# everpeace/kube-throttler

Hardware: AMD Instinct MI355X
Metric: pod_throttle_decisions_per_sec (higher is better)
Workload: dtype int64; 1 GPU; configs[2]: 1M pods x 1k Throttle+ClusterThrottle, D=8; pods_total=1000000, pods_per_gpu=1000000, throttles=1000, dims=8, labels_per_pod=8, namespaces=64, step=reconcile(aggregate+allreduce+finalize,apply)+check(all pods), streams=one, kernel_variant=indexed, parallelism=pods row-sharded x1, throttles replicated, exchange=none

## Files before the change

### include/kt_engine.h

```cpp
#ifndef KT_ENGINE_H
#define KT_ENGINE_H

#include <stdint.h>
#include "kt_snapshot.h"

#ifdef __cplusplus
extern "C" {
#endif

#define KT_OK 0
#define KT_ERR_INVALID_ARGUMENT (-1)
#define KT_ERR_OUT_OF_RANGE (-2)
#define KT_ERR_DEVICE (-3)
#define KT_ERR_OVERFLOW_RISK (-4)
#define KT_ERR_NOT_READY (-5)
#define KT_ERR_NO_DEVICE (-6)
#define KT_ERR_UNSUPPORTED (-7)

#define KT_STATUS_NOT_AFFECTED 0
#define KT_STATUS_NOT_THROTTLED 1
#define KT_STATUS_ACTIVE 2
#define KT_STATUS_INSUFFICIENT 3
#define KT_STATUS_POD_REQUESTS_EXCEEDS_THRESHOLD 4
#define KT_STATUS_ERROR 255
// ... 1 lines not shown
#define KT_VERDICT_SUCCESS 0
#define KT_VERDICT_UNSCHEDULABLE 1
#define KT_VERDICT_ERROR 2
#define KT_SUMMARY_VERDICT(w) ((uint32_t)((w) & 3u))
#define KT_SUMMARY_EXCEEDS(w) ((uint32_t)(((w) >> 4) & 0xFFFFFu))
#define KT_SUMMARY_ACTIVE(w) ((uint32_t)(((w) >> 24) & 0xFFFFFu))
#define KT_SUMMARY_INSUFFICIENT(w) ((uint32_t)(((w) >> 44) & 0xFFFFFu))

typedef struct kt_engine kt_engine;

typedef struct kt_config {
  int32_t n_dims;
  int32_t max_labels;
  int64_t pod_capacity;
  int32_t throttle_capacity;
  int32_t namespace_capacity;
  int32_t device;
  int32_t kernel_variant;
} kt_config;
#define KT_VARIANT_INCREMENTAL 0x100

const char* kt_version(void);

int32_t kt_engine_create(const kt_config* cfg, kt_engine** out);
int32_t kt_engine_destroy(kt_engine* e);
const char* kt_last_error(kt_engine* e);

int32_t kt_upsert_namespaces(kt_engine* e, const kt_snapshot* batch, const int32_t* ns_rows);
int32_t kt_upsert_pods(kt_engine* e, const kt_snapshot* batch, const int64_t* pod_rows);
int32_t kt_upsert_throttles(kt_engine* e, const kt_snapshot* batch, const int32_t* thr_rows);
int32_t kt_delete_namespaces(kt_engine* e, int32_t n, const int32_t* ns_rows);
int32_t kt_delete_pods(kt_engine* e, int64_t n, const int64_t* pod_rows);
int32_t kt_delete_throttles(kt_engine* e, int32_t n, const int32_t* thr_rows);
int32_t kt_load_snapshot(kt_engine* e, const kt_snapshot* s);

int32_t kt_upsert_namespace(kt_engine* e, int32_t ns_row, int32_t exists, int32_t n_labels, const uint32_t* label_keys,
                            const uint32_t* label_pairs);
int32_t kt_upsert_pod(kt_engine* e, int64_t pod_row, uint32_t ns, uint32_t flags, int32_t n_labels, const uint32_t* label_keys,
                      const uint32_t* label_pairs, int32_t n_ctr, const uint8_t* ctr_init, const uint32_t* ctr_present,
                      const int64_t* ctr_req, uint32_t ovh_present, const int64_t* ovh);
int32_t kt_upsert_throttle(kt_engine* e, int32_t thr_row, uint32_t flags, uint32_t ns, const int64_t* amt_v,
                           const uint32_t* amt_present, const int64_t* amt_count, const uint8_t* amt_has_count,
                           uint32_t thrl_flag, uint32_t thrl_has, uint64_t status_msgs_fp, uint64_t spec_msgs_fp, int32_t n_ovr,
                           const int64_t* ovr_begin_s, const int32_t* ovr_begin_ns, const int64_t* ovr_end_s,
                           const int32_t* ovr_end_ns, const uint8_t* ovr_flags, const int64_t* ovr_v, const uint32_t* ovr_present,
                           const int64_t* ovr_count, const uint8_t* ovr_has_count, int32_t n_terms, const uint8_t* term_flags,
                           const uint32_t* term_preq_off, const uint32_t* term_nreq_off, uint32_t n_preq, const uint8_t* preq_op,
                           const uint32_t* preq_key, const uint32_t* preq_val_off, const uint32_t* preq_val, uint32_t n_nreq,
                           const uint8_t* nreq_op, const uint32_t* nreq_key, const uint32_t* nreq_val_off, const uint32_t* nreq_val);

int32_t kt_set_reserved(kt_engine* e, int32_t n, const int32_t* thr_rows, const kt_amounts* reserved);
typedef struct kt_status {
  kt_amounts used;
  kt_amounts calc;
  uint8_t* calc_at_nonzero;
  uint32_t* thrl_flag;
  uint32_t* thrl_has;
  uint8_t* thrl_pod;
  uint64_t* msgs_fp;
  uint8_t* error;
} kt_status;
int32_t kt_set_status(kt_engine* e, int32_t n, const int32_t* thr_rows, const kt_status* status);

#define KT_RECONCILE_APPLY 0x1u
int32_t kt_reconcile_launch(kt_engine* e, int64_t now_s, int32_t now_ns, uint32_t flags, void* stream);
int32_t kt_reconcile_rows_launch(kt_engine* e, int64_t now_s, int32_t now_ns, uint32_t flags, int32_t n,
                                 const int32_t* throttle_rows, void* stream);
int32_t kt_aggregate_launch(kt_engine* e, void* stream);
int32_t kt_partial_used_buffer(kt_engine* e, void** device_ptr, int64_t* n_int64);
int32_t kt_use_partial_buffer(kt_engine* e, void* device_ptr, int64_t n_int64);
int32_t kt_finalize_launch(kt_engine* e, int64_t now_s, int32_t now_ns, uint32_t flags, void* stream);
#define KT_COMM_ID_BYTES 128
int32_t kt_comm_unique_id(void* out_id128);
int32_t kt_comm_init(kt_engine* e, int32_t rank, int32_t world, const void* id128);
int32_t kt_comm_allreduce_partial(kt_engine* e, void* stream);
int32_t kt_set_exchange_world(kt_engine* e, int32_t world);
int32_t kt_set_wide_sums(kt_engine* e, int32_t mode);
int32_t kt_partial_words(kt_engine* e, int64_t* n_int64, int32_t* wide);
int32_t kt_partial_layout(int32_t n_dims, int32_t* stride, int32_t* off_values, int32_t* off_presence, int32_t* off_pods,
                          int32_t* off_errors);
int32_t kt_comm_destroy(kt_engine* e);

int32_t kt_reconcile_fetch(kt_engine* e, int32_t n, const kt_status* out);
int32_t kt_reconcile_fetch_used_hi(kt_engine* e, int32_t n, int64_t* out_hi, int32_t* out_any_wide);
int32_t kt_reconcile_fetch_next_override(kt_engine* e, int32_t n, int64_t* next_s, int32_t* next_ns, uint8_t* has);

#define KT_CHECK_STATUS_MATRIX 0x1u
int32_t kt_check_launch(kt_engine* e, int64_t n, const int64_t* pod_rows, int32_t on_equal, uint32_t flags,
                        void* stream);
int32_t kt_sweep_launch(kt_engine* e, int64_t now_s, int32_t now_ns, uint32_t flags, int32_t on_equal, void* stream);
int32_t kt_check_fetch(kt_engine* e, int64_t n, uint64_t* out_summary, uint8_t* out_status);
int32_t kt_check(kt_engine* e, int64_t n, const int64_t* pod_rows, int32_t on_equal, uint64_t* out_summary,
                 uint8_t* out_status);
int32_t kt_affected_pods(kt_engine* e, int64_t n, const int64_t* pod_rows, int32_t m, const int32_t* throttle_rows, uint8_t* out);
#define KT_ADMIT_COMMIT 0x1u
int32_t kt_admit_launch(kt_engine* e, int64_t n, const int64_t* pod_rows, int32_t on_equal, uint32_t flags,
                        void* stream);
int32_t kt_admit_gangs_launch(kt_engine* e, int64_t n, const int64_t* pod_rows, int64_t n_gangs, const int64_t* gang_off,
                              int32_t on_equal, uint32_t flags, void* stream);
int32_t kt_admit_gangs_fetch(kt_engine* e, int64_t n_gangs, uint8_t* out_admitted);
#define KT_HEADROOM_MAX_CAP 0x7FFFFFFF
int32_t kt_headroom_launch(kt_engine* e, int64_t n, const int64_t* pod_rows, int32_t on_equal, int64_t cap, void* stream);
int32_t kt_headroom_fetch(kt_engine* e, int64_t n, int64_t* out_copies, int32_t* out_limiting );
#define KT_PREEMPT_NONE (-1)
int32_t kt_preempt_launch(kt_engine* e, int64_t n, const int64_t* pod_rows, int64_t n_cand, const int64_t* cand_rows, int64_t now_s,
                          int32_t now_ns, int32_t on_equal, void* stream);
int32_t kt_preempt_fetch(kt_engine* e, int64_t n, int64_t* out_prefix, uint8_t* out_victims );
int32_t kt_preempt_reprieve_launch(kt_engine* e, int64_t n, const int64_t* pod_rows, int64_t n_cand, const int64_t* cand_rows, int64_t now_s,
                                   int32_t now_ns, int32_t on_equal, void* stream);
int32_t kt_preempt_gangs_launch(kt_engine* e, int64_t n, const int64_t* pod_rows, int64_t n_gangs, const int64_t* gang_off, int64_t n_cand,
                                const int64_t* cand_rows, int64_t now_s, int32_t now_ns, int32_t on_equal, void* stream);
int32_t kt_preempt_gangs_fetch(kt_engine* e, int64_t n_gangs, int64_t* out_prefix ,
                               uint8_t* out_victims , int64_t* out_blocker );
int32_t kt_preempt_gangs_reprieve_launch(kt_engine* e, int64_t n, const int64_t* pod_rows, int64_t n_gangs, const int64_t* gang_off, int64_t n_cand,
                                         const int64_t* cand_rows, int64_t now_s, int32_t now_ns, int32_t on_equal, void* stream);
#define KT_FORECAST_NONE (-1)
int32_t kt_forecast_launch(kt_engine* e, int64_t n, const int64_t* pod_rows, int64_t n_inst, const int64_t* inst_s, const int32_t* inst_ns,
                           int32_t on_equal, void* stream);
int32_t kt_forecast_fetch(kt_engine* e, int64_t n, int64_t* out_first, uint8_t* out_verdicts );
int32_t kt_override_instants(kt_engine* e, int64_t from_s, int32_t from_ns, int64_t until_s, int32_t until_ns, int64_t cap, int64_t* out_s,
                             int32_t* out_ns, int64_t* out_total);
int32_t kt_fetch_reserved(kt_engine* e, int32_t n, const int32_t* throttle_rows, const kt_amounts* out);
int32_t kt_throttle_rows(kt_engine* e, int32_t* out_rows);
int32_t kt_check_device_summary(kt_engine* e, void** device_ptr);

int32_t kt_fetch_pod_requests(kt_engine* e, int64_t n, const int64_t* pod_rows, int64_t* out_v, uint32_t* out_present);

#define KT_KERNEL_CHECK 0
#define KT_KERNEL_AGGREGATE 1
#define KT_KERNEL_FINALIZE 2
#define KT_KERNEL_PREPARE 3
#define KT_KERNEL_REDUCE 4
#define KT_KERNEL_COUNT 5
int32_t kt_timing_enable(kt_engine* e, int32_t on);
int32_t kt_timing_read(kt_engine* e, int32_t kernel, double* total_ms, int64_t* launches);
int32_t kt_timing_reset(kt_engine* e);
int32_t kt_synchronize(kt_engine* e, void* stream);
const char* kt_kernel_name(kt_engine* e, int32_t kernel);
#define KT_COUNTER_FEW_CHECKS 0
#define KT_COUNTER_COMPILES 1
#define KT_COUNTER_INDEX_CHUNKS 2
#define KT_COUNTER_INDEX_WORDS 3
#define KT_COUNTER_NS_WORD_VISITS 4
#define KT_COUNTER_NS_ROWS 5
#define KT_COUNTER_NS_CHUNK_VISITS 6
#define KT_COUNTER_INDEX_IMAGE_WORDS 7
#define KT_COUNTER_SLOW_THROTTLES 8
#define KT_COUNTER_PACKED_WORDS 9
#define KT_COUNTER_VIEW_BUILDS 10
#define KT_COUNTER_AGG_WORKGROUPS 11
#define KT_COUNTER_MATCH_CACHE_BUILDS 12
#define KT_COUNTER_MATCH_CACHE_SCANS 13
#define KT_COUNTER_MATCH_CACHE_PLANES 14
int64_t kt_counter(kt_engine* e, int32_t which);
int32_t kt_paged_check(kt_engine* const* pages, int32_t n_pages, int64_t n, const int64_t* pod_rows, int32_t on_equal,
                       uint64_t* out_summary, uint8_t* out_status);
int32_t kt_paged_reconcile(kt_engine* const* pages, int32_t n_pages, int64_t now_s, int32_t now_ns, uint32_t flags, int32_t n,
                           const kt_status* page_out, uint8_t* replaced_any, uint8_t* error_any);
int32_t kt_paged_admit(kt_engine* const* pages, int32_t n_pages, int64_t n, const int64_t* pod_rows, int32_t on_equal, uint32_t flags,
                       uint64_t* out_summary, uint8_t* out_status);
int32_t kt_paged_admit_gangs(kt_engine* const* pages, int32_t n_pages, int64_t n, const int64_t* pod_rows, int64_t n_gangs,
                             const int64_t* gang_off, int32_t on_equal, uint32_t flags, uint64_t* out_summary, uint8_t* out_status,
                             uint8_t* out_gang_admitted);
int32_t kt_paged_headroom(kt_engine* const* pages, int32_t n_pages, int64_t n, const int64_t* pod_rows, int32_t on_equal,
                          int64_t cap, int64_t* out_copies, int32_t* out_limiting);
#define KT_PREEMPT_REPRIEVE 0x1u
int32_t kt_paged_preempt(kt_engine* const* pages, int32_t n_pages, int64_t n, const int64_t* pod_rows, int64_t n_cand,
                         const int64_t* cand_rows, int64_t now_s, int32_t now_ns, int32_t on_equal, uint32_t flags,
                         int64_t* out_prefix , uint8_t* out_victims );

int32_t kt_debug_reload_env(kt_engine* e);

#ifdef __cplusplus
}
#endif
#endif
```

### kube_throttler_amd/csrc/kt_engine.cpp

```cpp
#include "kt_engine_impl.h"

thread_local std::string g_create_error;

static bool getenv_flag(const char* name) {
  const char* v = getenv(name);
  return v && *v && *v != '0';
}
static void load_env_switches(kt_engine* e) {
  for (int k = 0; k < kSwCount; ++k) e->sw[k] = getenv_flag(kEnvSwitchName[k]);
  const char* cap = getenv("KT_REPRIEVE_LDS_CAP");
  const long cap_n = cap ? strtol(cap, nullptr, 10) : 0;
  e->reprieve_lds_cap_limit = cap_n > 0 && cap_n <= 0x7FFFFFFFl ? (uint32_t)cap_n : 0u;
}

void recs_invalidate_and_drain(kt_engine* e) {
  {
    std::lock_guard<std::mutex> g(e->recs_mu);
    e->recs_valid = false;
  }
  if (e->few_ready) std::lock_guard<std::mutex> drain(e->small_mu);
}

hipStream_t pick_stream(kt_engine* e, void* s) {
  hipStream_t st = s ? (hipStream_t)s : e->own_stream;
// ... 330 lines not shown
  if (e->h_small) (void)hipHostFree(e->h_small);
  if (e->h_few) (void)hipHostFree(e->h_few);
  e->d_few_acc.release();
  e->d_few_ticket.release();
  for (auto& ev : e->recs_ev)
    if (ev) (void)hipEventDestroy(ev);
  if (e->admit_pages_ev) (void)hipEventDestroy(e->admit_pages_ev);
  if (e->preempt_pages_ev) (void)hipEventDestroy(e->preempt_pages_ev);
  if (e->small_stream) (void)hipStreamDestroy(e->small_stream);
  if (e->h_stage) (void)hipHostFree(e->h_stage);
  for (auto& sl : e->ev_slots) {
    if (sl.ev) (void)hipEventDestroy(sl.ev);
    if (sl.h) (void)hipHostFree(sl.h);
  }
  if (e->h_overflow) (void)hipHostFree(e->h_overflow);
  DevBuf<uint32_t>* u32s[] = {&e->d_thr_term_off, &e->d_term_thr, &e->d_term_req_off, &e->d_req_key, &e->d_req_val_off,
                              &e->d_req_val, &e->d_ns_term_ok, &e->d_thr_flags, &e->d_thrl_flag, &e->d_thrl_has,
                              &e->d_ovr_off, &e->d_out_thrl_flag, &e->d_out_thrl_has};
  for (auto* b : u32s) b->release();
  DevBuf<uint8_t>* u8s[] = {&e->d_term_flags, &e->d_req_op, &e->d_ns_valid, &e->d_ovr_flags, &e->d_out_calc_updated,
                            &e->d_out_thrl_pod, &e->d_out_error, &e->d_recs2[0], &e->d_recs2[1], &e->d_wvimg[0], &e->d_wvimg[1], &e->d_status, &e->d_stage, &e->d_ev_stage, &e->d_slab, &e->d_admit, &e->d_admit_pages, &e->d_preempt_pages, &e->d_gang_out};
  for (auto* b : u8s) b->release();
  e->d_status_fp.release(); e->d_spec_fp.release(); e->d_summary.release(); e->d_rows.release(); e->d_gang_off.release();
  e->d_headroom_copies.release(); e->d_headroom_limiting.release();
  e->d_preempt_prefix.release(); e->d_preempt_victims.release(); e->d_preempt_partial.release(); e->d_preempt_gang_off.release(); e->d_preempt_blocker.release(); e->d_reprieve_ws.release();
  e->d_forecast_first.release(); e->d_forecast_verdicts.release(); e->d_forecast_inst_s.release(); e->d_forecast_inst_ns.release();
  e->d_used_hi.release(); e->d_out_used_hi.release();
  e->d_ovr_begin_s.release(); e->d_ovr_end_s.release(); e->d_ovr_begin_ns.release(); e->d_ovr_end_ns.release();
  e->d_partial.release();
  e->d_out_next_s.release();
  e->d_agg.release();
  e->d_out_next_ns.release();
  e->d_sp.release();
  AmountDev* ams[] = {&e->d_spec, &e->d_calc, &e->d_used, &e->d_reserved, &e->d_ovr_thr, &e->d_out_used, &e->d_out_calc};
  for (auto* a : ams) a->release();
  kt::release_index(e->dindex);
  for (auto& f : e->fam)
    for (auto& pr : f.pool) {
      (void)hipEventDestroy(pr.first);
      (void)hipEventDestroy(pr.second);
    }
  if (e->own_stream) (void)hipStreamDestroy(e->own_stream);
  delete e;
  return KT_OK;
}


int32_t kt_throttle_rows(kt_engine* e, int32_t* out_rows) {
  if (!e || !out_rows) return KT_ERR_INVALID_ARGUMENT;
  LaunchLock lk(e);
  *out_rows = e->thr_rows_hi;
  return KT_OK;
}

int32_t kt_check_device_summary(kt_engine* e, void** device_ptr) {
  if (!e || !device_ptr) return KT_ERR_INVALID_ARGUMENT;
  LaunchLock lk(e);
  if (!e->check_ready) return e->fail(KT_ERR_NOT_READY, "no check launched yet");
  *device_ptr = e->d_summary.p;
  return KT_OK;
}

int32_t kt_fetch_pod_requests(kt_engine* e, int64_t n, const int64_t* pod_rows, int64_t* out_v, uint32_t* out_present) {
  if (!e || n < 0 || !out_v || !out_present) return KT_ERR_INVALID_ARGUMENT;
  LaunchLock lk(e);
  KT_HIP(e, hipSetDevice(e->device));
  if (n == 0) return KT_OK;
  if (!pod_rows && n > e->cfg.pod_capacity) return e->fail(KT_ERR_OUT_OF_RANGE, "n > pod_capacity");
  if (pod_rows)
    for (int64_t i = 0; i < n; ++i)
      if (pod_rows[i] < 0 || pod_rows[i] >= e->cfg.pod_capacity) return e->fail(KT_ERR_OUT_OF_RANGE, "pod row");
  hipStream_t s = e->own_stream;
  if (e->last_stream) KT_HIP(e, hipStreamSynchronize(e->last_stream));
  const int D = e->D;
  size_t bytes = (size_t)n * 8 * D + (size_t)n * 4 + (pod_rows ? (size_t)n * 8 : 0) + 64;
  KT_HIP(e, e->d_stage.reserve(bytes));
  int64_t* dv = (int64_t*)e->d_stage.p;
  int64_t* drows = dv + (size_t)n * D;
  uint32_t* dp = (uint32_t*)(drows + (pod_rows ? n : 0));
  if (pod_rows) KT_HIP(e, hipMemcpyAsync(drows, pod_rows, (size_t)n * 8, hipMemcpyHostToDevice, s));
  kt::launch_gather_pod_requests(e->pods, n, pod_rows ? drows : nullptr, dv, dp, s);
  KT_HIP(e, hipMemcpyAsync(out_v, dv, (size_t)n * 8 * D, hipMemcpyDeviceToHost, s));
  KT_HIP(e, hipMemcpyAsync(out_present, dp, (size_t)n * 4, hipMemcpyDeviceToHost, s));
  KT_HIP(e, hipStreamSynchronize(s));
  return KT_OK;
}

int32_t kt_timing_enable(kt_engine* e, int32_t on) {
  if (!e) return KT_ERR_INVALID_ARGUMENT;
  LaunchLock lk(e);
  e->timing = on != 0;
  return KT_OK;
}

int32_t kt_timing_reset(kt_engine* e) {
  if (!e) return KT_ERR_INVALID_ARGUMENT;
  LaunchLock lk(e);
  KT_HIP(e, hipSetDevice(e->device));
  if (e->last_stream) KT_HIP(e, hipStreamSynchronize(e->last_stream));
  for (auto& f : e->fam) f.used = 0;
  return KT_OK;
}

int32_t kt_timing_read(kt_engine* e, int32_t kernel, double* total_ms, int64_t* launches) {
  if (!e || kernel < 0 || kernel >= KT_KERNEL_COUNT || !total_ms || !launches) return KT_ERR_INVALID_ARGUMENT;
  LaunchLock lk(e);
  KT_HIP(e, hipSetDevice(e->device));
  if (e->last_stream) KT_HIP(e, hipStreamSynchronize(e->last_stream));
  double tot = 0;
  TimingFamily& f = e->fam[kernel];
  for (size_t i = 0; i < f.used; ++i) {
    float ms = 0;
    KT_HIP(e, hipEventElapsedTime(&ms, f.pool[i].first, f.pool[i].second));
    tot += ms;
  }
  *total_ms = tot;
  *launches = (int64_t)f.used;
  return KT_OK;
}

int32_t kt_synchronize(kt_engine* e, void* stream) {
  if (!e) return KT_ERR_INVALID_ARGUMENT;
  LaunchLock lk(e);
  KT_HIP(e, hipSetDevice(e->device));
  KT_HIP(e, hipStreamSynchronize(pick_stream(e, stream)));
  return KT_OK;
}

int32_t kt_debug_reload_env(kt_engine* e) {
  if (!e) return KT_ERR_INVALID_ARGUMENT;
  StateLock lk(e);
  load_env_switches(e);
  return KT_OK;
}

int64_t kt_counter(kt_engine* e, int32_t which) {
  if (!e) return -1;
  switch (which) {
    case KT_COUNTER_FEW_CHECKS: return e->few_served.load(std::memory_order_relaxed);
    case KT_COUNTER_COMPILES: return e->n_compiles.load(std::memory_order_relaxed);
    case KT_COUNTER_INDEX_CHUNKS: return e->ctr_index_chunks.load(std::memory_order_relaxed);
    case KT_COUNTER_INDEX_WORDS: return e->ctr_index_words.load(std::memory_order_relaxed);
    case KT_COUNTER_NS_ROWS: return e->ctr_ns_rows.load(std::memory_order_relaxed);
    case KT_COUNTER_NS_WORD_VISITS: return e->ctr_ns_word_visits.load(std::memory_order_relaxed);
    case KT_COUNTER_NS_CHUNK_VISITS: return e->ctr_ns_chunk_visits.load(std::memory_order_relaxed);
    case KT_COUNTER_INDEX_IMAGE_WORDS: return e->ctr_index_image_words.load(std::memory_order_relaxed);
    case KT_COUNTER_SLOW_THROTTLES: return e->ctr_slow_throttles.load(std::memory_order_relaxed);
    case KT_COUNTER_PACKED_WORDS: return e->ctr_packed_words.load(std::memory_order_relaxed);
    case KT_COUNTER_AGG_WORKGROUPS: return e->ctr_agg_workgroups.load(std::memory_order_relaxed);
    case KT_COUNTER_VIEW_BUILDS: return e->ctr_view_builds.load(std::memory_order_relaxed);
    case KT_COUNTER_MATCH_CACHE_BUILDS: return e->ctr_mc_builds.load(std::memory_order_relaxed);
    case KT_COUNTER_MATCH_CACHE_SCANS: return e->ctr_mc_scans.load(std::memory_order_relaxed);
    case KT_COUNTER_MATCH_CACHE_PLANES: return e->ctr_mc_planes.load(std::memory_order_relaxed);
    default: return -1;
  }
}

int32_t kt_partial_layout(int32_t n_dims, int32_t* stride, int32_t* off_values, int32_t* off_presence, int32_t* off_pods,
                          int32_t* off_errors) {
  if (n_dims < 1 || n_dims > KT_MAX_DIMS) return KT_ERR_INVALID_ARGUMENT;
  if (stride) *stride = kt::partial_stride(n_dims);
  if (off_values) *off_values = 0;
  if (off_presence) *off_presence = kt::partial_off_presence(n_dims);
  if (off_pods) *off_pods = kt::partial_off_pods(n_dims);
  if (off_errors) *off_errors = kt::partial_off_errors(n_dims);
  return KT_OK;
}

const char* kt_kernel_name(kt_engine* e, int32_t kernel) {
  if (!e || kernel < 0 || kernel >= KT_KERNEL_COUNT) return "";
  return e->last_kernel[kernel];
}
```

### kube_throttler_amd/csrc/kt_engine_check.cpp

```cpp
#include "kt_engine_impl.h"

static int32_t ensure_check_recs(kt_engine* e, int32_t on_equal, int DT, hipStream_t s) {
  if (e->recs_valid && e->recs_eq == (on_equal != 0) && e->recs_DT == DT) return KT_OK;
  recs_invalidate_and_drain(e);
  {
    TimedLaunch tl(e, KT_KERNEL_PREPARE, s);
    kt::launch_prepare_check(e->tt, e->thr_rows_hi, e->D, DT, on_equal != 0, e->recs_ptr(), req_bound(e), s);
  }
  if (e->few_ready) KT_HIP(e, hipEventRecord(e->recs_ev[e->recs_cur], s));
  std::lock_guard<std::mutex> g(e->recs_mu);
  e->recs_ev_pending[e->recs_cur] = e->few_ready;
  e->recs_prev_valid = false;
  ++e->recs_seq[e->recs_cur];
  e->recs_valid = true;
  e->recs_eq = on_equal != 0;
  e->recs_DT = DT;
  return KT_OK;
}

int32_t match_cache_for_scan(kt_engine* e, hipStream_t s, kt::MatchCacheArgs& mc) {
  mc = kt::MatchCacheArgs();
  if (e->sw[kSw_NO_MATCH_CACHE] || e->cfg.kernel_variant != 0 || e->incremental || e->program_dirty || e->pod_rows_hi <= 0) return KT_OK;
  if (!kt::match_cache_fits(e->dindex) || e->hindex.has_slow || e->n_overflow != 0 || e->pods.LA > 8 || !e->pods.latom) return KT_OK;
  if (e->mc_planes_gen != e->program_gen) {
    const kt::BmChunk& ch = e->dindex.h_chunks[0];
    const uint32_t* rng = (const uint32_t*)(e->hindex.bm_images.data() + ch.img_off + ch.off_nsl_rng);
    uint32_t longest = 0;
    for (uint32_t n = 0; n < e->hindex.n_ns; ++n) longest = std::max(longest, rng[2 * n + 1] - rng[2 * n]);
    e->mc_planes = longest, e->mc_planes_gen = e->program_gen;
    e->ctr_mc_planes.store((int64_t)longest, std::memory_order_relaxed);
  }
  const uint32_t planes = e->mc_planes;
  if (!kt::check_replays_match_cache(e->pods, e->sp, e->dindex, planes, e->n_overflow != 0, e->sw[kSw_CHECK_ONE_PER_CU])) return KT_OK;
  const uint64_t stride = (uint64_t)e->cfg.pod_capacity;
  if (!e->mc_valid || e->mc_gen != e->program_gen) {
    if (e->d_mc.cap < (size_t)planes * stride) {
      if (e->last_stream) KT_HIP(e, hipStreamSynchronize(e->last_stream));
      KT_HIP(e, e->d_mc.reserve((size_t)planes * stride));
    }
    order_behind_ingest(e, s);
    if (!kt::launch_build_match_cache(e->pods, e->pod_rows_hi, nullptr, e->dindex, e->d_mc.p, stride, planes, s)) return KT_OK;
    KT_HIP(e, hipGetLastError());
    e->mc_valid = true, e->mc_gen = e->program_gen;
    e->mc_pending.clear();
    e->ctr_mc_builds.fetch_add(1, std::memory_order_relaxed);
  } else if (!e->mc_pending.empty()) {
    const size_t n = e->mc_pending.size();
    if (!e->h_mc_rows) {
      KT_HIP(e, hipHostMalloc((void**)&e->h_mc_rows, (size_t)kPatchBatchMax * 8, hipHostMallocDefault));
      KT_HIP(e, hipEventCreateWithFlags(&e->mc_rows_ev, hipEventDisableTiming));
    } else if (e->mc_rows_ev_used) {
      KT_HIP(e, hipEventSynchronize(e->mc_rows_ev));
    }
    memcpy(e->h_mc_rows, e->mc_pending.data(), n * 8);
    order_behind_ingest(e, s);
    if (!kt::launch_build_match_cache(e->pods, (int64_t)n, e->h_mc_rows, e->dindex, e->d_mc.p, stride, planes, s)) {
      e->mc_valid = false;
      e->mc_pending.clear();
      return KT_OK;
    }
    KT_HIP(e, hipGetLastError());
    KT_HIP(e, hipEventRecord(e->mc_rows_ev, s));
    e->mc_rows_ev_used = true;
    e->mc_pending.clear();
  }
  mc.mw = e->d_mc.p, mc.stride = stride, mc.planes = planes;
  return KT_OK;
}

static int32_t check_launch_locked(kt_engine* e, int64_t n, const int64_t* pod_rows, int32_t on_equal, uint32_t flags,
                                   hipStream_t s, bool allow_small = true) {
  e->headroom_ready = false;
  e->preempt_ready = false;
  e->forecast_ready = false;
  if (pod_rows) {
    for (int64_t i = 0; i < n; ++i)
      if (pod_rows[i] < 0 || pod_rows[i] >= e->cfg.pod_capacity)
        return e->fail(KT_ERR_OUT_OF_RANGE, "pod row %lld", (long long)pod_rows[i]);
  } else if (n > e->cfg.pod_capacity) {
    return e->fail(KT_ERR_OUT_OF_RANGE, "n=%lld > pod_capacity", (long long)n);
  }
  int32_t rc = ensure_ready(e, s);
  if (rc != KT_OK) return rc;
  const bool want_status = (flags & KT_CHECK_STATUS_MATRIX) != 0;
  const size_t T = (size_t)e->thr_rows_hi;
  if (e->d_summary.cap < (size_t)n + 1 || (want_status && e->d_status.cap < (size_t)n * T + 64) ||
      (pod_rows && e->d_rows.cap < (size_t)n + 1)) {
    if (e->last_stream) KT_HIP(e, hipStreamSynchronize(e->last_stream));
    KT_HIP(e, e->d_summary.reserve((size_t)n + 1));
    if (want_status) KT_HIP(e, e->d_status.reserve((size_t)n * T + 64));
    if (pod_rows) KT_HIP(e, e->d_rows.reserve((size_t)n + 1));
  }
  const bool small = allow_small && e->cfg.kernel_variant != 1 && n > 0 && n <= kt::kCheckSmallMax;
  kt::CheckSmall sm{};
  if (small) {
    if (!e->h_small) {
      KT_HIP(e, hipHostMalloc((void**)&e->h_small, (size_t)kt::kCheckSmallMax * 8, hipHostMallocMapped));
      KT_HIP(e, e->d_ticket.reserve(16));
      KT_HIP(e, hipMemsetAsync(e->d_ticket.p, 0, 16 * 4, s));
    }
    sm.ticket = e->d_ticket.p;
    sm.host_summary = e->h_small;
    if (pod_rows && n <= 8) {
      sm.n_inline = (uint32_t)n;
      for (int64_t k = 0; k < 8; ++k) sm.inline_rows[k] = pod_rows[k < n ? k : n - 1];
    }
  }
  if (pod_rows && n && !sm.n_inline) {
    KT_HIP(e, hipMemcpyAsync(e->d_rows.p, pod_rows, (size_t)n * 8, hipMemcpyHostToDevice, s));
    KT_HIP(e, hipStreamSynchronize(s));
  }
  const int DT = e->cfg.kernel_variant == 1 ? kt::dt_bucket(e->D) : kt::dt_bucket_ix(e->D);
  if ((rc = ensure_check_recs(e, on_equal, DT, s)) != KT_OK) return rc;
  kt::MatchCacheArgs mc;
  if (e->cfg.kernel_variant != 1 && !pod_rows && !small && !want_status && n > 0 && n <= e->cfg.pod_capacity && e->dindex.n_chunks == 1 &&
      !e->sw[kSw_FORCE_NS_ORDER] && !e->sw[kSw_CHECK_ONE_PER_CU]) {
    if ((rc = match_cache_for_scan(e, s, mc)) != KT_OK) return rc;
  }
  {
    TimedLaunch tl(e, KT_KERNEL_CHECK, s);
    if (e->cfg.kernel_variant == 1)
      kt::launch_check_dense(e->pods, n, pod_rows ? e->d_rows.p : nullptr, e->sp, e->uses_keys, e->recs_ptr(),
                             e->d_summary.p, want_status ? e->d_status.p : nullptr, s),
          e->last_kernel[KT_KERNEL_CHECK] = "kt_check_dense";
    else {
      const bool by_ns = !pod_rows && !small && n == e->pod_rows_hi && (e->dindex.n_chunks > 1 || e->sw[kSw_FORCE_NS_ORDER]) && !e->sw[kSw_NO_NS_ORDER];
      if (by_ns && (rc = settle_view_patches(e, s)) != KT_OK) return rc;
      ScanView& av = e->views.all_rows;
      if (by_ns && (!av.valid || (int64_t)av.n != e->pod_rows_hi)) {
        const ViewSpec spec{false, true, kt::check_sweep_blocks, e->pod_rows_hi, false};
        KT_HIP(e, e->d_carry.reserve((size_t)e->pod_rows_hi + 1));
        if ((rc = list_view_rows(e, av, spec, s)) != KT_OK) return rc;
        if ((rc = copy_view_records(e, av, spec, 0, s)) != KT_OK) return rc;
        av.valid = true;
      }
      kt::CheckByNs view{av.meta.p, av.latom.p, e->d_carry.p};
      if (by_ns && av.range_G) view.wg_range = av.range.p, view.wg_range_G = av.range_G;
      if (by_ns && !want_status && e->dindex.n_slow == 0 && e->n_overflow == 0 && e->dindex.n_chunks > 1 && !e->sw[kSw_NO_VERDICT_IMAGES]) {
        const int b = e->recs_cur;
        if (e->wvimg_seq[b] != e->recs_seq[b] || e->wvimg_gen[b] != e->program_gen || e->wvimg_DT[b] != DT) {
          KT_HIP(e, e->d_wvimg[b].reserve(kt::verdict_images_bytes(e->dindex.bm_words, e->D)));
          TimedLaunch tl2(e, KT_KERNEL_PREPARE, s);
          kt::launch_build_verdict_images(e->dindex, e->dindex.bm_words, e->recs_ptr(), e->thr_rows_hi, e->D, e->d_wvimg[b].p, s);
          e->wvimg_seq[b] = e->recs_seq[b], e->wvimg_gen[b] = e->program_gen, e->wvimg_DT[b] = DT;
        }
        view.wv_img = e->d_wvimg[b].p, view.wv_total_words = e->dindex.bm_words;
      }
      const char* k = kt::launch_check_indexed(e->pods, n, by_ns ? av.rows.p : pod_rows ? e->d_rows.p : nullptr, e->sp, e->d_sp.p, e->dindex,
                                               e->recs_ptr(), e->d_summary.p, want_status ? e->d_status.p : nullptr, s,
                                               small ? &sm : nullptr, e->n_overflow != 0, by_ns ? &view : nullptr, e->sw[kSw_CHECK_ONE_PER_CU],
                                               mc.mw ? &mc : nullptr);
      if (mc.used) e->ctr_mc_scans.fetch_add(1, std::memory_order_relaxed);
      if (!k) return e->fail(KT_ERR_UNSUPPORTED, "%d throttle rows exceed the indexed check kernel's LDS budget (use kernel_variant 1)", e->thr_rows_hi);
      e->last_kernel[KT_KERNEL_CHECK] = k;
    }
  }
  KT_HIP(e, hipGetLastError());
  e->check_n = n;
  e->check_in_h_small = small;
  e->check_T = e->thr_rows_hi;
  e->check_has_status = want_status;
  e->check_ready = true;
  e->last_stream = s;
  return KT_OK;
}

int32_t kt_check_launch(kt_engine* e, int64_t n, const int64_t* pod_rows, int32_t on_equal, uint32_t flags, void* stream) {
  if (!e || n < 0) return KT_ERR_INVALID_ARGUMENT;
  LaunchLock lk(e);
  KT_HIP(e, hipSetDevice(e->device));
  return check_launch_locked(e, n, pod_rows, on_equal, flags, pick_stream(e, stream));
}

int32_t kt_sweep_launch(kt_engine* e, int64_t now_s, int32_t now_ns, uint32_t flags, int32_t on_equal, void* stream) {
  if (!e) return KT_ERR_INVALID_ARGUMENT;
  LaunchLock lk(e);
  KT_HIP(e, hipSetDevice(e->device));
  hipStream_t s = pick_stream(e, stream);
  int32_t rc = ensure_ready(e, s);
  if (rc != KT_OK) return rc;
  const int64_t n = e->pod_rows_hi;
  auto one_after_the_other = [&]() -> int32_t {
    int32_t r = check_launch_locked(e, n, nullptr, on_equal, 0u, s);
    if (r != KT_OK) return r;
    if ((r = aggregate_locked(e, s, true)) != KT_OK) return r;
    return finalize_locked(e, now_s, now_ns, flags, s, !e->incremental);
  };
  bool fused = e->cfg.kernel_variant != 1 && !e->incremental && e->dindex.n_chunks == 1 && e->dindex.n_slow == 0 && !e->hindex.has_slow && !e->dindex.has_long &&
               e->n_overflow == 0 && e->thr_rows_hi > 0 && n > 0 && kt::dt_bucket_ix(e->D) == 8 && !e->sw[kSw_NO_SWEEP] &&
               !e->sw[kSw_NO_FUSED] && !e->sw[kSw_NO_PACK];
  if (!fused) return one_after_the_other();
  if ((rc = request_sums_in_range(e, s)) != KT_OK) return rc;
  if (e->wide) return one_after_the_other();
  const int nb = kt::aggregate_blocks(n);
  kt::PackPlan plan = kt::make_pack_plan(e->D, e->max_abs, e->or_abs, e->neg_seen, kt::aggregate_slab_pods(n, nb), true, 4);
  if (!plan.nw || plan.rec_bytes > kt::agg_rec_bytes(e->D, false)) return one_after_the_other();
  const size_t words = (size_t)e->thr_rows_hi * kt::partial_stride(e->D);
  if (e->ext_partial && (int64_t)words > e->ext_partial_words)
    return e->fail(KT_ERR_OUT_OF_RANGE, "caller partial buffer holds %lld words, %lld needed", (long long)e->ext_partial_words, (long long)words);
  if (e->d_summary.cap < (size_t)n + 1) {
    if (e->last_stream) KT_HIP(e, hipStreamSynchronize(e->last_stream));
    KT_HIP(e, e->d_summary.reserve((size_t)n + 1));
  }
  const int DT = kt::dt_bucket_ix(e->D);
  if ((rc = ensure_check_recs(e, on_equal, DT, s)) != KT_OK) return rc;
  e->fused_pending = false;
  e->agg_wide = false;
  if (words && e->clean_partial != (const void*)e->partial()) KT_HIP(e, hipMemsetAsync(e->partial(), 0, words * 8, s));
  e->clean_partial = nullptr;
  kt::AggScan sc;
// ... 947 lines not shown
```

### kube_throttler_amd/csrc/kt_engine_impl.h

```cpp
#pragma once
#include <hip/hip_runtime.h>
#include <dlfcn.h>

#include <algorithm>
#include <cstdarg>
#include <cstdio>
#include <cstring>
#include <memory>
#include <atomic>
#include <chrono>
#include <mutex>
#include <shared_mutex>
#include <string>
#include <unordered_set>
#include <vector>

#include "../../include/kt_engine.h"
#include "kt_index.h"
#include "kt_launch.h"


#define KT_INTERNAL __attribute__((visibility("hidden")))

namespace kte {


struct Req {
  uint8_t op;
  uint32_t key;
  std::vector<uint32_t> vals;
};
struct Term {
  uint8_t flags = 0;
  std::vector<Req> preq, nreq;
};
struct HostAmount {
  int64_t v[KT_MAX_DIMS] = {0};
  int64_t v_hi[KT_MAX_DIMS] = {0};
  uint32_t present = 0;
  int64_t count = 0;
  uint8_t has_count = 0;
};
struct Override {
  int64_t begin_s, end_s;
  int32_t begin_ns, end_ns;
  uint8_t flags;
  HostAmount thr;
};
struct HostThrottle {
  uint32_t flags = 0;
  uint32_t ns = 0;
  HostAmount spec, calc, used, reserved;
  uint32_t thrl_flag = 0, thrl_has = 0;
  uint64_t status_fp = 0, spec_fp = 0;
  std::vector<Override> ovr;
  std::vector<Term> terms;
  std::vector<uint32_t> adm;
  uint64_t adm_gen = 0;
  uint32_t adm_ns = 0;
};
static bool same_reqs(const std::vector<Req>& a, const std::vector<Req>& b) {
  if (a.size() != b.size()) return false;
  for (size_t i = 0; i < a.size(); ++i)
    if (a[i].op != b[i].op || a[i].key != b[i].key || a[i].vals != b[i].vals) return false;
  return true;
}
static bool same_selector(const HostThrottle& a, const HostThrottle& b) {
  const uint32_t sel = KT_THR_VALID | KT_THR_RESPONSIBLE | KT_THR_CLUSTER;
  if ((a.flags & sel) != (b.flags & sel) || a.ns != b.ns || a.terms.size() != b.terms.size()) return false;
  for (size_t k = 0; k < a.terms.size(); ++k)
    if (a.terms[k].flags != b.terms[k].flags || !same_reqs(a.terms[k].preq, b.terms[k].preq) || !same_reqs(a.terms[k].nreq, b.terms[k].nreq))
      return false;
  return true;
}
struct HostNamespace {
  bool valid = false;
  std::vector<std::pair<uint32_t, uint32_t>> labels;
};

template <class T>
struct DevBuf {
  T* p = nullptr;
  size_t cap = 0;
  hipError_t reserve(size_t n) {
    if (n <= cap && p) return hipSuccess;
    if (p) (void)hipFree(p);
    p = nullptr;
    cap = 0;
    size_t want = std::max<size_t>(n, 16);
    hipError_t e = kt::kt_alloc_device((void**)&p, want * sizeof(T));
    if (e == hipSuccess) cap = want;
    return e;
  }
  void release() {
    if (p) (void)hipFree(p);
    p = nullptr;
    cap = 0;
  }
};

struct AmountDev {
  DevBuf<int64_t> v;
  DevBuf<uint32_t> present;
  DevBuf<int64_t> count;
  DevBuf<uint8_t> has_count;
  hipError_t reserve(size_t n, int D) {
    hipError_t e;
    if ((e = v.reserve(n * D)) != hipSuccess) return e;
    if ((e = present.reserve(n)) != hipSuccess) return e;
    if ((e = count.reserve(n)) != hipSuccess) return e;
    return has_count.reserve(n);
  }
  kt::AmountTab tab() const { return kt::AmountTab{v.p, present.p, count.p, has_count.p}; }
  void release() { v.release(); present.release(); count.release(); has_count.release(); }
};

struct ScanView {
  DevBuf<int64_t> rows;
  DevBuf<unsigned long long> d_n;
  unsigned long long n = 0;
  DevBuf<uint64_t> meta;
  DevBuf<uint16_t> latom;
  DevBuf<int64_t> req;
  DevBuf<uint64_t> pk;
  kt::PackPlan pack;
  DevBuf<int32_t> pos;
  DevBuf<uint32_t> range;
  int range_G = 0;
  int64_t cap = 0;
  int64_t extra = 0;
  bool by_ns = false;
  bool valid = false;
  void release() { rows.release(); d_n.release(); meta.release(); latom.release(); req.release(); pk.release(); pos.release(); range.release(); }
};
struct ViewSpec {
  bool countable_only;
  bool by_ns;
  int (*grid)(int64_t);
  int64_t rows_cap;
  bool requests;
};
struct ScanViews {
  ScanView countable;
  ScanView all_rows;
  DevBuf<unsigned long long> d_ns_cursor;
  std::vector<unsigned long long> h_ns_end;
  std::vector<uint32_t> h_range;
  DevBuf<uint32_t> d_dirty;
  bool check_dirty = false;
  void invalidate() { countable.valid = false, all_rows.valid = false; }
  void release() { countable.release(); all_rows.release(); d_ns_cursor.release(); d_dirty.release(); }
};

struct AmountHostFlat {
  std::vector<int64_t> v;
  std::vector<uint32_t> present;
  std::vector<int64_t> count;
  std::vector<uint8_t> has_count;
  void resize(size_t n, int D) {
    v.assign(n * D, 0);
    present.assign(n, 0);
    count.assign(n, 0);
    has_count.assign(n, 0);
  }
  void set(size_t i, int D, const HostAmount& a) {
    for (int d = 0; d < D; ++d) v[i * D + d] = (a.present >> d) & 1u ? a.v[d] : 0;
    present[i] = a.present;
    count[i] = a.has_count ? a.count : 0;
    has_count[i] = a.has_count;
  }
  void get(size_t i, int D, HostAmount& a) const {
    for (int d = 0; d < D; ++d) a.v[d] = v[i * D + d];
    a.present = present[i];
    a.count = count[i];
    a.has_count = has_count[i];
  }
};

struct TimingFamily {
  std::vector<std::pair<hipEvent_t, hipEvent_t>> pool;
  size_t used = 0;
};

}
using namespace kte;

extern thread_local std::string g_create_error;


enum EnvSwitch { kSw_FEED_NO_STAGE, kSw_FORCE_NS_ORDER, kSw_INGEST_EVENT_WAIT, kSw_NO_FEED_FEW, kSw_NO_FEED_FUSION, kSw_NO_FUSED, kSw_NO_NS_ORDER, kSw_NO_PACK, kSw_NO_SCAN_VIEW, kSw_NO_SWEEP, kSw_NO_VERDICT_IMAGES, kSw_NO_WG_RANGES, kSw_SYNC_INGEST, kSw_INGEST_TRUST_FENCE, kSw_NO_VIEW_PATCH, kSw_CHECK_ONE_PER_CU, kSw_AGG_SMALL_WINDOW, kSw_AGG_ONE_PER_CU, kSw_NO_MATCH_CACHE, kSwCount };
static const char* const kEnvSwitchName[kSwCount] = {"KT_FEED_NO_STAGE", "KT_FORCE_NS_ORDER", "KT_INGEST_EVENT_WAIT", "KT_NO_FEED_FEW", "KT_NO_FEED_FUSION", "KT_NO_FUSED", "KT_NO_NS_ORDER", "KT_NO_PACK", "KT_NO_SCAN_VIEW", "KT_NO_SWEEP", "KT_NO_VERDICT_IMAGES", "KT_NO_WG_RANGES", "KT_SYNC_INGEST", "KT_INGEST_TRUST_FENCE", "KT_NO_VIEW_PATCH", "KT_CHECK_ONE_PER_CU", "KT_AGG_SMALL_WINDOW", "KT_AGG_ONE_PER_CU", "KT_NO_MATCH_CACHE"};
struct kt_engine {
  bool sw[kSwCount] = {};
  uint32_t reprieve_lds_cap_limit = 0;
  kt_config cfg{};
  std::shared_mutex mu;
  std::mutex small_mu;
  std::mutex ingest_mu;
  std::mutex op_mu;
  std::mutex recs_mu;
  std::mutex err_mu;
  std::string err;
  int device = 0;
  hipStream_t own_stream = nullptr;
  int D = 0, L = 0;

  kt::PodTable pods{};
  int64_t pod_rows_hi = 0;
  unsigned __int128 max_abs[KT_MAX_DIMS] = {0};
  uint64_t or_abs[KT_MAX_DIMS] = {0};
  ScanViews views;
  bool cut_plain = false;
  void* cur_launch_lock = nullptr;
  std::atomic<int64_t> ctr_index_chunks{0}, ctr_index_words{0}, ctr_index_image_words{0}, ctr_ns_rows{0}, ctr_ns_word_visits{0}, ctr_ns_chunk_visits{0}, ctr_slow_throttles{0}, ctr_packed_words{0}, ctr_agg_workgroups{0}, ctr_view_builds{0}, ctr_mc_builds{0}, ctr_mc_scans{0}, ctr_mc_planes{0};
  DevBuf<uint16_t> d_latom;
  DevBuf<uint64_t> d_mc;
  int64_t* h_mc_rows = nullptr;
  hipEvent_t mc_rows_ev = nullptr;
  bool mc_rows_ev_used = false;
  std::vector<int64_t> mc_pending;
  bool mc_valid = false;
  uint64_t mc_gen = ~0ull;
  uint64_t mc_planes_gen = ~0ull;
  uint32_t mc_planes = 0;
  DevBuf<unsigned long long> d_overflow;
  unsigned long long n_overflow = 0;
  static constexpr int kEvSlots = 8;
  static constexpr size_t kEvSlotBytes = 64 * 1024;
  struct EvSlot {
    uint8_t* h = nullptr;
    hipEvent_t ev = nullptr;
    bool used = false;
  } ev_slots[kEvSlots];
  int ev_next = 0;
  std::atomic<bool> ingest_pending{false};
  hipEvent_t ingest_ev = nullptr;
  std::atomic<hipEvent_t> ingest_unretired{nullptr};
  hipStream_t ingest_stream = nullptr;
  unsigned long long* h_overflow = nullptr;
  bool overflow_in_flight = false;
  unsigned long long ingest_seq = 0;
  unsigned long long ingest_spin_seq = 0;
  bool req_sums_valid = true;
  unsigned __int128 req_sum_bound[KT_MAX_DIMS] = {0};
  DevBuf<unsigned long long> d_req_sums;
  DevBuf<uint8_t> d_row_mask;
  DevBuf<uint32_t> d_slab_tag;
  uint32_t slab_epoch = 0;
  bool neg_seen = false;

  std::vector<HostNamespace> ns;
  uint64_t ns_gen = 1;
  int32_t ns_rows_hi = 0;
  int64_t pod_ns_hi = 0;
  size_t ns_compiled = 0;
  std::vector<HostThrottle> thr;
  int32_t thr_rows_hi = 0;
  bool program_dirty = true;
  bool spec_dirty = false;
  bool status_host_dirty = true;
  bool reserved_dev_newer = false;
  bool incremental = false;
  bool agg_valid = false;
  DevBuf<unsigned long long> d_agg;
  bool recs_valid = false;
  bool recs_eq = false;
  int recs_DT = 0;
  bool status_dev_newer = false;

  DevBuf<uint32_t> d_thr_term_off, d_term_thr, d_term_req_off, d_req_key, d_req_val_off, d_req_val, d_ns_term_ok;
  DevBuf<uint8_t> d_term_flags, d_req_op, d_ns_valid;
  kt::SelProgram sp{};
  DevBuf<kt::SelProgram> d_sp;
  bool uses_keys = false;
  kt::HostIndex hindex;
  kt::IndexDev dindex;

  DevBuf<uint32_t> d_thr_flags, d_thrl_flag, d_thrl_has, d_ovr_off;
  DevBuf<uint64_t> d_status_fp, d_spec_fp;
  AmountDev d_spec, d_calc, d_used, d_reserved, d_ovr_thr;
  DevBuf<int64_t> d_ovr_begin_s, d_ovr_end_s;
  DevBuf<int32_t> d_ovr_begin_ns, d_ovr_end_ns;
  DevBuf<uint8_t> d_ovr_flags;
  kt::ThrTables tt{};

  DevBuf<unsigned long long> d_partial;
  DevBuf<uint8_t> d_admit;
  DevBuf<uint8_t> d_admit_pages;
  std::vector<kt::AdmitPage> h_admit_pages;
  hipEvent_t admit_pages_ev = nullptr;
  DevBuf<int64_t> d_gang_off;
  DevBuf<uint8_t> d_gang_out;
  std::vector<int64_t> h_gang_off;
  bool gang_ready = false, gang_on_device = false;
  int64_t gang_n = 0;
  DevBuf<int64_t> d_headroom_copies;
  DevBuf<int32_t> d_headroom_limiting;
  bool headroom_ready = false;
  int64_t headroom_n = 0;
  DevBuf<int64_t> d_preempt_prefix;
  DevBuf<uint8_t> d_preempt_victims;
  DevBuf<unsigned long long> d_preempt_partial;
  DevBuf<unsigned char> d_reprieve_ws;
  bool preempt_ready = false;
  int64_t preempt_n = 0, preempt_m = 0;
  DevBuf<uint8_t> d_preempt_pages;
  std::vector<kt::PreemptPage> h_preempt_pages;
  hipEvent_t preempt_pages_ev = nullptr;
  bool preempt_gangs = false;
  DevBuf<int64_t> d_preempt_gang_off, d_preempt_blocker;
  DevBuf<int64_t> d_forecast_first, d_forecast_inst_s;
  DevBuf<int32_t> d_forecast_inst_ns;
  DevBuf<uint8_t> d_forecast_verdicts;
  bool forecast_ready = false;
  int64_t forecast_n = 0, forecast_m = 0;
  DevBuf<uint8_t> d_slab;
  unsigned long long* ext_partial = nullptr;
  int64_t ext_partial_words = 0;
  unsigned long long* partial() { return ext_partial ? ext_partial : d_partial.p; }
  const void* clean_partial = nullptr;
  AmountDev d_out_used, d_out_calc;
  bool wide = false;
  bool agg_wide = false;
  DevBuf<int64_t> d_used_hi, d_out_used_hi;
  DevBuf<uint8_t> d_out_calc_updated, d_out_thrl_pod, d_out_error;
  DevBuf<int64_t> d_out_next_s;
  DevBuf<int32_t> d_out_next_ns;
  DevBuf<uint32_t> d_out_thrl_flag, d_out_thrl_has;
  bool reconcile_ready = false;
  bool agg_pending = false;
  bool fused_pending = false;
  int fused_nb = 0;
  uint32_t fused_epoch = 0;
  kt::PackPlan fused_pack;
  size_t agg_words = 0;
  uint64_t program_gen = 0, agg_gen = 0;
  int32_t exchange_world = 1;

  DevBuf<uint8_t> d_recs2[2];
  int recs_cur = 0;
  uint64_t recs_seq[2] = {0, 0};
  DevBuf<uint8_t> d_wvimg[2];
  uint64_t wvimg_seq[2] = {~0ull, ~0ull}, wvimg_gen[2] = {~0ull, ~0ull};
  int wvimg_DT[2] = {0, 0};
  hipEvent_t recs_ev[2] = {nullptr, nullptr};
  bool recs_ev_pending[2] = {false, false};
  int32_t wide_mode = 0;
  bool recs_prev_valid = false;
  uint8_t* recs_ptr() { return d_recs2[recs_cur].p; }
  hipStream_t small_stream = nullptr;
  DevBuf<unsigned long long> d_few_acc;
  DevBuf<uint32_t> d_few_ticket;
  uint64_t* h_few = nullptr;
  uint64_t few_seq = 0;
  std::atomic<bool> few_ready{false};
  std::atomic<int64_t> few_served{0};
  std::atomic<int64_t> n_compiles{0};
  DevBuf<uint64_t> d_summary;
  DevBuf<uint64_t> d_carry;
  DevBuf<uint8_t> d_status;
  DevBuf<int64_t> d_rows;
  int64_t check_n = 0;
  DevBuf<uint32_t> d_ticket;
  uint64_t* h_small = nullptr;
  bool check_in_h_small = false;
  int32_t check_T = 0, reconcile_T = 0;
  bool check_has_status = false;
// ... 183 lines not shown
```

### kube_throttler_amd/csrc/kt_engine_reconcile.cpp

```cpp
#include "kt_engine_impl.h"

Rccl* rccl() {
  static Rccl r;
  static std::once_flag once;
  std::call_once(once, [] {
    for (const char* name : {"librccl.so.1", "librccl.so", "/opt/rocm/lib/librccl.so.1"}) {
      r.lib = dlopen(name, RTLD_NOW | RTLD_LOCAL);
      if (r.lib) break;
    }
    if (!r.lib) {
      r.err = std::string("cannot load librccl.so: ") + (dlerror() ? dlerror() : "?");
      return;
    }
    r.GetUniqueId = (decltype(r.GetUniqueId))dlsym(r.lib, "ncclGetUniqueId");
    r.CommInitRank = (decltype(r.CommInitRank))dlsym(r.lib, "ncclCommInitRank");
    r.AllReduce = (decltype(r.AllReduce))dlsym(r.lib, "ncclAllReduce");
    r.CommDestroy = (decltype(r.CommDestroy))dlsym(r.lib, "ncclCommDestroy");
    r.GetErrorString = (decltype(r.GetErrorString))dlsym(r.lib, "ncclGetErrorString");
    if (!r.GetUniqueId || !r.CommInitRank || !r.AllReduce || !r.CommDestroy) r.err = "librccl.so lacks the nccl* entry points";
  });
  return &r;
}
static constexpr int kNcclInt64 = 4, kNcclSum = 0;

// ... 30 lines not shown
  if (world > e->exchange_world) {
    e->exchange_world = world;
    if (world > 4) e->req_sums_valid = false;
  }
  return KT_OK;
}

int32_t kt_set_exchange_world(kt_engine* e, int32_t world) {
  if (!e || world < 1) return KT_ERR_INVALID_ARGUMENT;
  StateLock lk(e);
  if (world != e->exchange_world && (world > 4 || e->exchange_world > 4 || e->wide)) e->req_sums_valid = false;
  e->exchange_world = world;
  return KT_OK;
}

int32_t kt_set_wide_sums(kt_engine* e, int32_t mode) {
  if (!e || (mode != 0 && mode != 1)) return KT_ERR_INVALID_ARGUMENT;
  StateLock lk(e);
  if (mode == 1 && e->incremental) return e->fail(KT_ERR_UNSUPPORTED, "kt_set_wide_sums(1): an incremental engine keeps int64 partials");
  if (mode != e->wide_mode) e->req_sums_valid = false;
  e->wide_mode = mode;
  return KT_OK;
}

int32_t kt_partial_words(kt_engine* e, int64_t* n_int64, int32_t* wide) {
  if (!e || !n_int64) return KT_ERR_INVALID_ARGUMENT;
  LaunchLock lk(e);
  if (!e->agg_pending) return e->fail(KT_ERR_NOT_READY, "kt_partial_words: no partials pending (kt_aggregate_launch first)");
  *n_int64 = (int64_t)e->agg_words;
  if (wide) *wide = e->agg_wide ? 1 : 0;
  return KT_OK;
}

int32_t kt_comm_allreduce_partial(kt_engine* e, void* stream) {
  if (!e) return KT_ERR_INVALID_ARGUMENT;
  LaunchLock lk(e);
  KT_HIP(e, hipSetDevice(e->device));
  if (!e->comm) return e->fail(KT_ERR_NOT_READY, "kt_comm_allreduce_partial before kt_comm_init");
  hipStream_t s = pick_stream(e, stream);
  if (!e->agg_pending) return e->fail(KT_ERR_NOT_READY, "kt_comm_allreduce_partial: no partials pending (kt_aggregate_launch first)");
  KT_CHECK_PARTIALS_CURRENT(e, "kt_comm_allreduce_partial");
  const size_t words = e->agg_words;
  if (!words) return KT_OK;
  if (!e->partial()) return e->fail(KT_ERR_NOT_READY, "no partial buffer yet: kt_aggregate_launch first");
  if (e->ext_partial && (int64_t)words > e->ext_partial_words)
    return e->fail(KT_ERR_OUT_OF_RANGE, "caller partial buffer holds %lld words, %lld needed", (long long)e->ext_partial_words,
                   (long long)words);
  Rccl* r = rccl();
  const int rc = r->AllReduce(e->partial(), e->partial(), words, kNcclInt64, kNcclSum, e->comm, s);
  if (rc != 0) return e->fail(KT_ERR_DEVICE, "ncclAllReduce: %s", r->GetErrorString ? r->GetErrorString(rc) : "error");
  e->last_stream = s;
  return KT_OK;
}

int32_t kt_comm_destroy(kt_engine* e) {
  if (!e) return KT_ERR_INVALID_ARGUMENT;
  StateLock lk(e);
  KT_HIP(e, hipSetDevice(e->device));
  if (!e->comm) return KT_OK;
  if (e->last_stream) KT_HIP(e, hipStreamSynchronize(e->last_stream));
  (void)rccl()->CommDestroy(e->comm);
  e->comm = nullptr;
  e->comm_world = 1, e->comm_rank = 0;
  return KT_OK;
}



int32_t slab_tags(kt_engine* e, kt::AggScan& sc, hipStream_t s) {
  const size_t need = (size_t)e->dindex.n_chunks * kt::kSlabTagStride + 1;
  if (e->d_slab_tag.cap < need) {
    if (e->last_stream) KT_HIP(e, hipStreamSynchronize(e->last_stream));
    KT_HIP(e, e->d_slab_tag.reserve(need));
    KT_HIP(e, hipMemsetAsync(e->d_slab_tag.p, 0, e->d_slab_tag.cap * 4, s));
    e->slab_epoch = 0;
  }
  if (++e->slab_epoch == 0u) {
    KT_HIP(e, hipMemsetAsync(e->d_slab_tag.p, 0, e->d_slab_tag.cap * 4, s));
    e->slab_epoch = 1;
  }
  sc.slab_tag = e->d_slab_tag.p, sc.epoch = e->slab_epoch;
  return KT_OK;
}

int32_t request_sums_in_range(kt_engine* e, hipStream_t s) {
  if (e->req_sums_valid && !(e->wide_mode == 1 && !e->wide)) return KT_OK;
  KT_HIP(e, e->d_req_sums.reserve(32));
  kt::launch_sum_abs_requests(e->pods, e->pod_rows_hi, e->d_req_sums.p, s);
  KT_HIP(e, hipGetLastError());
  unsigned long long h[32];
  KT_HIP(e, hipMemcpyAsync(h, e->d_req_sums.p, sizeof(h), hipMemcpyDeviceToHost, s));
  KT_HIP(e, hipStreamSynchronize(s));
  bool wide = false;
  for (int d = 0; d < e->D; ++d) {
    const unsigned __int128 total = (unsigned __int128)h[2 * d] + ((unsigned __int128)h[2 * d + 1] << 32);
    e->req_sum_bound[d] = total;
    if (total > rank_sum_bound(e->exchange_world)) {
      if (e->incremental)
        return e->fail(KT_ERR_OVERFLOW_RISK,
                       "dimension %d: the requests of the pods held here add up beyond 2^60 at this scale (the reference would "
                       "promote to big decimals); an incremental engine needs a coarser scale for it", d);
      if ((unsigned __int128)e->pod_rows_hi * (unsigned __int128)e->exchange_world > ((unsigned __int128)1 << 30))
        return e->fail(KT_ERR_OVERFLOW_RISK, "dimension %d: wide sums hold for up to 2^30 pods over all ranks", d);
      if (e->exchange_world > 1 && e->wide_mode != 1)
        return e->fail(KT_ERR_OVERFLOW_RISK,
                       "dimension %d: the requests of this rank's pods add up beyond the exact range of one int64 block; with %d ranks "
                       "the two-block form must be agreed: call kt_set_wide_sums(e, 1) on every rank", d, e->exchange_world);
      wide = true;
    }
  }
  if (e->wide_mode == 1 && !wide) {
    if (e->incremental) return e->fail(KT_ERR_UNSUPPORTED, "kt_set_wide_sums(1): an incremental engine keeps int64 partials");
    if ((unsigned __int128)e->pod_rows_hi * (unsigned __int128)e->exchange_world > ((unsigned __int128)1 << 30))
      return e->fail(KT_ERR_OVERFLOW_RISK, "wide sums hold for up to 2^30 pods over all ranks");
    wide = true;
  }
  if (wide != e->wide) e->views.countable.valid = false;
  e->wide = wide;
  e->req_sums_valid = true;
  return KT_OK;
}

static void upgrade_launch_lock(kt_engine* e) {
  if (e->cur_launch_lock) ((LaunchLock*)e->cur_launch_lock)->upgrade();
}

int32_t aggregate_locked(kt_engine* e, hipStream_t s, bool allow_fused) {
  e->fused_pending = false;
  int32_t rc = ensure_ready(e, s);
  if (rc != KT_OK) return rc;
  if ((rc = request_sums_in_range(e, s)) != KT_OK) return rc;
  const size_t block_words = (size_t)e->thr_rows_hi * kt::partial_stride(e->D);
  const size_t words = block_words * (e->wide ? 2 : 1);
  e->agg_wide = e->wide;
  if (e->ext_partial && (int64_t)words > e->ext_partial_words)
    return e->fail(KT_ERR_OUT_OF_RANGE, "caller partial buffer holds %lld words, %lld needed",
                   (long long)e->ext_partial_words, (long long)words);
  if (e->incremental && e->agg_valid) {
    if (words) KT_HIP(e, hipMemcpyAsync(e->partial(), e->d_agg.p, words * 8, hipMemcpyDeviceToDevice, s));
    e->last_kernel[KT_KERNEL_AGGREGATE] = "(incremental: no scan)";
    e->last_stream = s;
    e->agg_pending = true, e->agg_words = words, e->agg_gen = e->program_gen;
    return KT_OK;
  }
  const bool by_ns = (e->dindex.n_chunks > 1 || e->sw[kSw_FORCE_NS_ORDER]) && !e->sw[kSw_NO_NS_ORDER];
  if ((rc = settle_view_patches(e, s)) != KT_OK) return rc;
  ScanView& cv = e->views.countable;
  if (cv.valid && cv.extra && !(!e->sw[kSw_NO_SCAN_VIEW] && (by_ns || e->dindex.n_chunks == 1))) cv.valid = false;
  const bool two_view = !e->sw[kSw_NO_SCAN_VIEW] && !e->sw[kSw_NO_PACK] && e->cfg.kernel_variant != 1 && !by_ns && !e->incremental && !e->wide &&
                        e->dindex.n_chunks == 1;
  const kt::AggTwoLaunch two_launch{!e->sw[kSw_AGG_ONE_PER_CU], e->sw[kSw_AGG_SMALL_WINDOW], e->n_overflow != 0, e->pods.LA};
  if (cv.valid && cv.pack.headroom >= (uint32_t)kt::kPackHeadroomBitsTwo && !(two_view && kt::aggregate_two_per_cu_fits(e->dindex, cv.pack, two_launch)))
    cv.valid = false;
  if (e->cfg.kernel_variant != 1 && (!cv.valid || cv.by_ns != by_ns)) {
    if (e->last_stream && e->last_stream != s) KT_HIP(e, hipStreamSynchronize(e->last_stream));
    const ViewSpec spec{true, by_ns, kt::aggregate_blocks, e->cfg.pod_capacity, true};
    if ((rc = list_view_rows(e, cv, spec, s)) != KT_OK) return rc;
    const int64_t headroom = std::min<int64_t>(std::max<int64_t>(65536, (int64_t)cv.n / 16), e->cfg.pod_capacity - (int64_t)cv.n);
    const bool view_scan = !e->sw[kSw_NO_SCAN_VIEW] && (cv.by_ns || e->dindex.n_chunks == 1);
    cv.pack = kt::PackPlan();
    if (view_scan && !e->incremental && !e->wide && !e->sw[kSw_NO_PACK] && !e->dindex.has_long) {
      const int64_t cap = (int64_t)cv.n + headroom;
      uint64_t slab_pods = kt::aggregate_slab_pods(cap, kt::aggregate_blocks(cap));
      if (cv.range_G) slab_pods = std::max<uint64_t>(slab_pods, (uint64_t)kt::wg_range_cap((int64_t)cv.n, cv.range_G) + 64u);
      cv.pack = kt::make_pack_plan(e->D, e->max_abs, e->or_abs, e->neg_seen, slab_pods, true, kt::pack_max_words(e->D));
      if (cv.pack.nw && cv.pack.rec_bytes > e->dindex.cut_thr_bytes) cv.pack = kt::PackPlan();
      if (two_view && cv.pack.nw) {
        const uint64_t slab_pods2 = kt::aggregate_slab_pods(cap, kt::aggregate_blocks(cap, kt::kAggWorkgroupsTwo));
        const kt::PackPlan two = kt::make_pack_plan(e->D, e->max_abs, e->or_abs, e->neg_seen, slab_pods2, false, 3,
                                                    kt::kPackHeadroomBitsTwo);
        if (two.nw && kt::aggregate_two_per_cu_fits(e->dindex, two, two_launch)) cv.pack = two;
      }
    }
    if (!cv.pack.nw && kt::agg_rec_bytes(e->D, e->incremental) > e->dindex.cut_thr_bytes) {
      upgrade_launch_lock(e);
      e->cut_plain = true, e->program_dirty = true;
      return aggregate_locked(e, s, allow_fused);
    }
    if (!e->sw[kSw_NO_SCAN_VIEW] && (rc = copy_view_records(e, cv, spec, headroom, s)) != KT_OK) return rc;
    cv.valid = true;
  }
  if (words && e->clean_partial != (const void*)e->partial()) KT_HIP(e, hipMemsetAsync(e->partial(), 0, words * 8, s));
  e->clean_partial = nullptr;
  {
    TimedLaunch tl(e, KT_KERNEL_AGGREGATE, s);
    std::unique_ptr<TimedLaunch> tr;
    const bool defer = allow_fused && !e->incremental && !e->wide && e->dindex.n_chunks == 1 && !e->sw[kSw_NO_FUSED];
    auto after_scan = [&]() {
      tl.stop_now();
      if (!(defer && cv.pack.nw)) tr.reset(new TimedLaunch(e, KT_KERNEL_REDUCE, s));
    };
    const int n_pass = e->wide ? 2 : 1;
    for (int pass = 0; pass < n_pass; ++pass) {
      const int limb = e->wide ? pass + 1 : 0;
      unsigned long long* target = e->partial() + (size_t)pass * block_words;
      if (e->cfg.kernel_variant == 1) {
        kt::launch_aggregate_dense(e->pods, e->pod_rows_hi, e->sp, e->uses_keys, target, s, limb);
        e->last_kernel[KT_KERNEL_AGGREGATE] = "kt_aggregate_dense";
      } else {
        kt::AggScan sc;
        sc.n = (int64_t)cv.n, sc.rows = cv.rows.p, sc.counts = e->incremental, sc.nonneg = !e->neg_seen;
        sc.overflow_pods = two_launch.overflow_pods;
        sc.small_window = two_launch.small_window;
        sc.one_per_cu = !two_launch.enabled;
        sc.limb = limb;
        sc.by_ns = !e->sw[kSw_NO_SCAN_VIEW] && (cv.by_ns || e->dindex.n_chunks == 1);
        if (sc.by_ns) sc.n += cv.extra;
        if (sc.by_ns) sc.v_meta = cv.meta.p, sc.v_latom = cv.latom.p, sc.v_req = cv.pack.nw ? nullptr : cv.req.p;
        if (sc.by_ns && cv.pack.nw) sc.pk = &cv.pack, sc.v_pk = cv.pk.p;
        if (sc.by_ns && cv.by_ns && cv.range_G) sc.wg_range = cv.range.p, sc.wg_range_G = cv.range_G;
        if ((rc = slab_tags(e, sc, s)) != KT_OK) return rc;
        sc.defer_reduce = defer && sc.pk != nullptr;
        const char* k = kt::launch_aggregate_indexed(e->pods, sc, e->sp, e->d_sp.p, e->dindex, target, e->d_slab.p, s,
                                                     pass == 0 ? std::function<void()>(after_scan) : std::function<void()>());
        if (!k && sc.refused) return e->fail(KT_ERR_OUT_OF_RANGE, "aggregate launch refused: %s", sc.refused);
        if (!k) return e->fail(KT_ERR_UNSUPPORTED, "a chunk of the selector index exceeds the aggregate kernel's LDS budget (use kernel_variant 1)");
        e->last_kernel[KT_KERNEL_AGGREGATE] = k;
        e->ctr_agg_workgroups.store((int64_t)sc.launched_blocks, std::memory_order_relaxed);
        e->ctr_packed_words.store(sc.launched_packed ? (int64_t)cv.pack.nw : 0, std::memory_order_relaxed);
        if (sc.defer_reduce && sc.launched_packed) e->fused_pending = true, e->fused_nb = sc.launched_blocks, e->fused_epoch = sc.epoch, e->fused_pack = cv.pack;
        e->last_kernel[KT_KERNEL_REDUCE] = e->fused_pending ? "(in kt_reduce_finalize_packed)" : sc.launched_packed ? "kt_reduce_packed_slabs" : "kt_reduce_bitmap_slabs";
      }
    }
  }
  KT_HIP(e, hipGetLastError());
  if (e->incremental) {
    KT_HIP(e, e->d_agg.reserve(words + 1));
    if (words) KT_HIP(e, hipMemcpyAsync(e->d_agg.p, e->partial(), words * 8, hipMemcpyDeviceToDevice, s));
    e->agg_valid = true;
  }
  e->last_stream = s;
  e->agg_pending = true, e->agg_words = words, e->agg_gen = e->program_gen;
  return KT_OK;
}

int32_t delta_scan(kt_engine* e, int64_t n, const int64_t* rows_dev, int64_t row0, int sign, hipStream_t s) {
  if (!e->incremental || !e->agg_valid || n <= 0 || e->thr_rows_hi == 0) return KT_OK;
  kt::AggScan sc;
  sc.n = n, sc.rows = rows_dev, sc.row0 = row0, sc.counts = true, sc.sign = sign, sc.overflow_pods = e->n_overflow != 0;
  sc.small_window = e->sw[kSw_AGG_SMALL_WINDOW];
  int32_t rc = slab_tags(e, sc, s);
  if (rc != KT_OK) return rc;
  const char* k = kt::launch_aggregate_indexed(e->pods, sc, e->sp, e->d_sp.p, e->dindex, e->d_agg.p, e->d_slab.p, s, nullptr);
  if (!k && sc.refused) return e->fail(KT_ERR_OUT_OF_RANGE, "aggregate launch refused: %s", sc.refused);
  if (!k) return e->fail(KT_ERR_UNSUPPORTED, "a chunk of the selector index exceeds the aggregate kernel's LDS budget");
  KT_HIP(e, hipGetLastError());
  return KT_OK;
}

int32_t finalize_locked(kt_engine* e, int64_t now_s, int32_t now_ns, uint32_t flags, hipStream_t s, bool consume,
                               const uint8_t* row_mask) {
  KT_CHECK_PARTIALS_CURRENT(e, "kt_finalize_launch");
  int32_t rc = ensure_ready(e, s);
  if (rc != KT_OK) return rc;
  if (!e->agg_pending) e->agg_wide = e->wide;
  e->agg_pending = false;
  kt::ReconcileOut out{e->d_out_used.tab(), e->d_out_calc.tab(), e->d_out_used_hi.p, e->d_out_calc_updated.p, e->d_out_thrl_flag.p,
                       e->d_out_thrl_has.p, e->d_out_thrl_pod.p, e->d_out_error.p, e->d_out_next_s.p, e->d_out_next_ns.p};
  const bool apply = (flags & KT_RECONCILE_APPLY) != 0;
  const int rec_DT = e->cfg.kernel_variant == 1 ? kt::dt_bucket(e->D) : kt::dt_bucket_ix(e->D);
  bool keep_prev;
  int wbuf;
  {
    std::lock_guard<std::mutex> g(e->recs_mu);
    keep_prev = apply && e->recs_valid && e->recs_DT == rec_DT && e->few_ready;
    wbuf = keep_prev ? 1 - e->recs_cur : e->recs_cur;
  }
  if (apply && !keep_prev) recs_invalidate_and_drain(e);
  if (apply && keep_prev) {
    {
      std::lock_guard<std::mutex> g(e->recs_mu);
      e->recs_prev_valid = false;
    }
    if (e->few_ready) std::lock_guard<std::mutex> drain(e->small_mu);
  }
  {
    TimedLaunch tl(e, KT_KERNEL_FINALIZE, s);
    if (e->fused_pending) {
      kt::launch_reduce_finalize_packed(e->tt, e->sp, e->D, e->dindex, e->fused_pack, e->d_slab.p, e->fused_nb, e->d_slab_tag.p, e->fused_epoch, e->partial(),
                                        consume, now_s, now_ns, apply, out, apply ? e->d_recs2[wbuf].p : nullptr, rec_DT, e->recs_eq, req_bound(e), s,
                                        row_mask, e->dindex.n_slow != 0 || e->n_overflow != 0);
      e->last_kernel[KT_KERNEL_FINALIZE] = "kt_reduce_finalize_packed";
    } else {
      kt::launch_finalize(e->tt, e->sp, e->D, e->partial(), consume, now_s, now_ns, apply, out, apply ? e->d_recs2[wbuf].p : nullptr, rec_DT,
                          e->recs_eq, req_bound(e), s, row_mask,
                          e->agg_wide ? e->partial() + (size_t)e->thr_rows_hi * kt::partial_stride(e->D) : nullptr);
      e->last_kernel[KT_KERNEL_FINALIZE] = "kt_finalize";
    }
    e->fused_pending = false;
  }
  if (apply) {
    if (e->few_ready) KT_HIP(e, hipEventRecord(e->recs_ev[wbuf], s));
    std::lock_guard<std::mutex> g(e->recs_mu);
    e->recs_ev_pending[wbuf] = e->few_ready;
    e->recs_prev_valid = keep_prev;
    e->recs_cur = wbuf;
    ++e->recs_seq[wbuf];
    e->recs_valid = true;
    e->recs_DT = rec_DT;
  }
  e->clean_partial = consume ? (const void*)e->partial() : nullptr;
  KT_HIP(e, hipGetLastError());
  if (apply) e->status_dev_newer = true;
  e->reconcile_ready = true;
  e->reconcile_T = e->thr_rows_hi;
  e->last_stream = s;
  return KT_OK;
}

int32_t preempt_reconcile_locked(kt_engine* e, int64_t now_s, int32_t now_ns, hipStream_t s) {
  int32_t rc = request_sums_in_range(e, s);
  if (rc != KT_OK) return rc;
  if (e->wide) return e->fail(KT_ERR_UNSUPPORTED, "preempt: `used` is wider than int64 (kt_preempt reads int64 sums)");
  const size_t words = (size_t)e->thr_rows_hi * kt::partial_stride(e->D);
  if (e->d_preempt_partial.cap < words + 1) {
    if (e->last_stream) KT_HIP(e, hipStreamSynchronize(e->last_stream));
    KT_HIP(e, e->d_preempt_partial.reserve(words + 1));
  }
  e->reconcile_ready = false;
  if (!words) return KT_OK;
  KT_HIP(e, hipMemsetAsync(e->d_preempt_partial.p, 0, words * 8, s));
  kt::launch_aggregate_dense(e->pods, e->pod_rows_hi, e->sp, e->uses_keys, e->d_preempt_partial.p, s, 0);
  kt::ReconcileOut out{e->d_out_used.tab(), e->d_out_calc.tab(), e->d_out_used_hi.p, e->d_out_calc_updated.p, e->d_out_thrl_flag.p,
                       e->d_out_thrl_has.p, e->d_out_thrl_pod.p, e->d_out_error.p, e->d_out_next_s.p, e->d_out_next_ns.p};
  kt::launch_finalize(e->tt, e->sp, e->D, e->d_preempt_partial.p, false, now_s, now_ns, false, out, nullptr, 0, false,
                      req_bound(e), s);
  KT_HIP(e, hipGetLastError());
  e->last_stream = s;
  return KT_OK;
}

int32_t kt_aggregate_launch(kt_engine* e, void* stream) {
  if (!e) return KT_ERR_INVALID_ARGUMENT;
  LaunchLock lk(e);
  KT_HIP(e, hipSetDevice(e->device));
  return aggregate_locked(e, pick_stream(e, stream));
}

int32_t kt_partial_used_buffer(kt_engine* e, void** device_ptr, int64_t* n_int64) {
  if (!e || !device_ptr || !n_int64) return KT_ERR_INVALID_ARGUMENT;
  LaunchLock lk(e);
  KT_HIP(e, hipSetDevice(e->device));
  int32_t rc = ensure_ready(e, e->own_stream);
  if (rc != KT_OK) return rc;
  *device_ptr = e->partial();
  *n_int64 = e->agg_pending ? (int64_t)e->agg_words : (int64_t)e->thr_rows_hi * kt::partial_stride(e->D) * ((e->wide || e->wide_mode == 1) ? 2 : 1);
  return KT_OK;
}

int32_t kt_use_partial_buffer(kt_engine* e, void* device_ptr, int64_t n_int64) {
  if (!e || (device_ptr && n_int64 <= 0)) return KT_ERR_INVALID_ARGUMENT;
  StateLock lk(e);
  KT_HIP(e, hipSetDevice(e->device));
  if (e->last_stream) KT_HIP(e, hipStreamSynchronize(e->last_stream));
  e->ext_partial = (unsigned long long*)device_ptr;
  e->ext_partial_words = device_ptr ? n_int64 : 0;
  e->clean_partial = nullptr;
  return KT_OK;
}

int32_t kt_finalize_launch(kt_engine* e, int64_t now_s, int32_t now_ns, uint32_t flags, void* stream) {
  if (!e) return KT_ERR_INVALID_ARGUMENT;
  LaunchLock lk(e);
  KT_HIP(e, hipSetDevice(e->device));
  e->fused_pending = false;
  return finalize_locked(e, now_s, now_ns, flags, pick_stream(e, stream));
}
// ... 107 lines not shown
```

### kube_throttler_amd/csrc/kt_engine_views.cpp

```cpp
#include "kt_engine_impl.h"

int32_t list_view_rows(kt_engine* e, ScanView& v, const ViewSpec& spec, hipStream_t s) {
  ScanViews& vs = e->views;
  const uint32_t n_ns = (uint32_t)e->sp.n_ns;
  e->ctr_view_builds.fetch_add(1, std::memory_order_relaxed);
  v.valid = false;
  v.by_ns = spec.by_ns;
  KT_HIP(e, v.rows.reserve((size_t)spec.rows_cap + 1));
  KT_HIP(e, v.d_n.reserve(1));
  if (spec.by_ns) {
    KT_HIP(e, vs.d_ns_cursor.reserve((size_t)n_ns + 1));
    kt::launch_order_rows_by_ns(e->pods, e->pod_rows_hi, spec.countable_only, n_ns, vs.d_ns_cursor.p, v.rows.p, v.d_n.p, s);
  } else {
    KT_HIP(e, hipMemsetAsync(v.d_n.p, 0, 8, s));
    kt::launch_compact_countable(e->pods, e->pod_rows_hi, v.rows.p, v.d_n.p, s);
  }
  KT_HIP(e, hipGetLastError());
  const bool plan_ranges = spec.by_ns && !e->sw[kSw_NO_WG_RANGES];
  if (spec.countable_only) KT_HIP(e, hipMemcpyAsync(&v.n, v.d_n.p, 8, hipMemcpyDeviceToHost, s));
  else v.n = (unsigned long long)e->pod_rows_hi;
  if (plan_ranges) {
    vs.h_ns_end.resize((size_t)n_ns + 1);
    KT_HIP(e, hipMemcpyAsync(vs.h_ns_end.data(), vs.d_ns_cursor.p, (size_t)n_ns * 8, hipMemcpyDeviceToHost, s));
  }
  if (spec.countable_only || plan_ranges) KT_HIP(e, hipStreamSynchronize(s));
  v.range_G = 0;
  if (plan_ranges && v.n > 0) {
    v.range_G = spec.grid((int64_t)v.n);
    KT_HIP(e, v.range.reserve((size_t)v.range_G + 2));
    vs.h_range.resize((size_t)v.range_G + 2);
    kt::plan_wg_ranges(vs.h_ns_end.data(), n_ns, (int64_t)v.n, v.range_G, vs.h_range.data());
    KT_HIP(e, hipMemcpyAsync(v.range.p, vs.h_range.data(), vs.h_range.size() * 4, hipMemcpyHostToDevice, s));
    KT_HIP(e, hipStreamSynchronize(s));
  }
  return KT_OK;
}

int32_t copy_view_records(kt_engine* e, ScanView& v, const ViewSpec& spec, int64_t headroom, hipStream_t s) {
  ScanViews& vs = e->views;
  v.cap = (int64_t)v.n + headroom;
  v.extra = 0;
  const size_t nc = (size_t)v.cap + 1, np = (size_t)spec.rows_cap + 1;
  KT_HIP(e, v.meta.reserve(nc));
  KT_HIP(e, v.latom.reserve(nc * (size_t)e->pods.LA));
  if (spec.requests) KT_HIP(e, v.pack.nw ? v.pk.reserve(nc * (size_t)v.pack.stride) : v.req.reserve(nc * (size_t)e->pods.DS));
  KT_HIP(e, v.pos.reserve(np));
  KT_HIP(e, vs.d_dirty.reserve(4));
  KT_HIP(e, hipMemsetAsync(v.pos.p, 0xFF, np * 4, s));
  if (spec.countable_only) {
    KT_HIP(e, hipMemsetAsync(v.meta.p + v.n, 0, (size_t)(headroom + 1) * 8, s));
    KT_HIP(e, hipMemsetAsync(v.rows.p + v.n, 0, (size_t)(headroom + 1) * 8, s));
  }
  if (!vs.check_dirty) KT_HIP(e, hipMemsetAsync(vs.d_dirty.p, 0, 4, s));
  kt::launch_build_scan_view(e->pods, (int64_t)v.n, v.rows.p, v.meta.p, v.latom.p, spec.requests && !v.pack.nw ? v.req.p : nullptr, s,
                             v.pack.nw ? &v.pack : nullptr, v.pk.p, v.pos.p);
  KT_HIP(e, hipGetLastError());
  return KT_OK;
}

bool views_patchable(const kt_engine* e, int64_t n, const unsigned __int128* batch_max, const uint64_t* batch_or, bool batch_neg) {
  const ScanView& c = e->views.countable;
  if (e->incremental || e->cfg.kernel_variant != 0 || e->program_dirty || n > kPatchBatchMax) return false;
  if (!c.valid && !e->views.all_rows.valid) return false;
  if (e->sw[kSw_NO_VIEW_PATCH]) return false;
  if (c.valid) {
    if (c.meta.p == nullptr || c.pos.p == nullptr) return false;
    if (c.extra + n > c.cap - (int64_t)c.n) return false;
    if (c.pack.nw) {
      if (batch_neg) return false;
      for (int d = 0; d < e->D; ++d) {
        if (batch_max[d] > e->max_abs[d]) return false;
        if (c.pack.shift[d] && (batch_or[d] & ((1ull << c.pack.shift[d]) - 1ull))) return false;
      }
    }
  }
  return true;
}
kt::ViewPatch view_patch_of(kt_engine* e, int64_t n) {
  ScanView& c = e->views.countable;
  const ScanView& a = e->views.all_rows;
  kt::ViewPatch v{};
  if (c.valid) {
    v.vc_meta = c.meta.p, v.vc_latom = c.latom.p, v.vc_req = c.pack.nw ? nullptr : c.req.p, v.vc_pk = c.pack.nw ? c.pk.p : nullptr;
    v.vc_rows = c.rows.p, v.pos_c = c.pos.p, v.n_c = c.d_n.p, v.cap_c = c.cap;
    v.by_ns = c.by_ns ? 1u : 0u;
    v.pk = c.pack;
    if (!c.by_ns) c.extra += n;
  }
  if (a.valid) v.va_meta = a.meta.p, v.va_latom = a.latom.p, v.pos_a = a.pos.p, v.rows_a = (int64_t)a.n;
  v.dirty = e->views.d_dirty.p;
  if ((c.valid && c.by_ns) || a.valid) e->views.check_dirty = true;
  return v;
}
int32_t patch_views(kt_engine* e, int64_t n, const int64_t* rows_dev, int64_t row0, hipStream_t s) {
  const kt::ViewPatch v = view_patch_of(e, n);
  kt::launch_patch_scan_views(e->pods, n, rows_dev, row0, v, s);
  KT_HIP(e, hipGetLastError());
  return KT_OK;
}
int32_t settle_view_patches(kt_engine* e, hipStream_t s) {
  ScanViews& vs = e->views;
  if (!vs.check_dirty) return KT_OK;
  uint32_t dirty = 0;
  KT_HIP(e, hipMemcpyAsync(&dirty, vs.d_dirty.p, 4, hipMemcpyDeviceToHost, s));
  KT_HIP(e, hipStreamSynchronize(s));
  if (dirty) {
    vs.invalidate();
    KT_HIP(e, hipMemsetAsync(vs.d_dirty.p, 0, 4, s));
  }
  vs.check_dirty = false;
  return KT_OK;
}
```

### kube_throttler_amd/csrc/kt_index.h

```cpp
#pragma once
#include <hip/hip_runtime.h>
#include <stdint.h>

#include <algorithm>
#include <functional>
#include <vector>

#include "kt_device.h"

namespace kt {

constexpr uint32_t kKeyAtom = 0x80000000u;
constexpr uint32_t kMaxIndexedTerms = 512;
constexpr uint32_t kCheckWordLds = 64u * 8u + 560u;

constexpr uint32_t kTermAdj = 0x80000000u;
constexpr uint32_t kTermReal = 0x40000000u;
constexpr uint32_t kTermRowMask = 0x000FFFFFu;
constexpr uint16_t kRankAdj = 0x8000u;

struct ThrInfo {
  bool live;
  bool cluster;
  uint32_t ns;
// ... 38 lines not shown
struct AtomId {
  uint32_t atom, id;
  uint32_t home;
};
constexpr int kAtomHomeShift = 48;
constexpr uint32_t kAtomIdMask = 0xFFFFu;

struct HostIndex {
  std::vector<uint32_t> slow_thr;
  uint32_t bm_words = 0;
  uint32_t bm_rows = 0;
  bool has_veto = false;
  uint32_t max_need = 0;
  uint32_t n_pair_keys = 0, n_key_atoms = 0;
  uint32_t n_keys = 0;
  bool has_slow = false;
  bool has_long = false;
  uint32_t la = 8;
  bool rich = false;
  std::vector<AtomId> atoms;
  std::vector<uint32_t> atom_key;
  std::vector<uint64_t> atom_table;
  std::vector<BmChunk> bm_chunks;
  std::vector<unsigned char> bm_images;
  std::vector<uint32_t> bm_rank_t;
  std::vector<uint32_t> thr_ngrp;
  std::vector<uint32_t> nogroup;
  std::vector<uint32_t> bm_chunk_ns;
  uint32_t ns_words = 0;
  uint32_t bm_max_lds = 0, bm_max_thr = 0, bm_max_words = 0;
  uint64_t bm_slab_bytes = 0;
  uint32_t cut_chk_budget = 0;
  uint32_t cut_thr_bytes = 0;
  bool agg_windowed = false;
  bool cut_grouped = false;
  uint32_t img_words = 0;
  int64_t ns_word_visits = 0;
  int64_t ns_chunk_visits = 0;
  uint32_t n_ns = 0;
  std::vector<uint64_t> full_any, full_veto, full_nsrows;
  std::vector<WordHdr> full_hdr;
  std::vector<uint32_t> full_term_t, full_term_g, full_term_rank;
  std::vector<uint8_t> full_real;
};

__host__ __device__ inline uint32_t agg_rec_bytes(int D, bool counts) {
  return (uint32_t)(((size_t)D * 8 + (counts ? (size_t)D * 4 + 4 : 8) + 15) & ~(size_t)15);
}

struct PackPlan {
  uint32_t nw = 0;
  uint32_t stride = 0;
  uint32_t rec_bytes = 0;
  uint8_t word[16] = {0}, pos[16] = {0}, width[16] = {0}, shift[16] = {0};
  uint8_t cnt_width = 0;
  uint64_t even[8] = {0, 0, 0, 0, 0, 0, 0, 0};
  uint8_t top_pos[8] = {0, 0, 0, 0, 0, 0, 0, 0};
  uint32_t desc[16] = {0};
  uint32_t cnt_desc = 0;
  uint32_t headroom = 0;
};
constexpr int kPackHeadroomBits = 8;
constexpr int kPackHeadroomBitsTwo = 9;
constexpr uint32_t kPackMaxWords = 8;
__host__ __device__ inline uint32_t pack_max_words(int D) { return D <= 8 ? 4u : kPackMaxWords; }
__host__ __device__ inline uint32_t packed_rec_max(int D) { return (pack_max_words(D) + 1u) * 8u; }
constexpr int kPackClasses = 3;
__host__ __device__ inline uint32_t pack_desc(uint32_t word, uint32_t cls, uint32_t pos, uint32_t wext, uint32_t shift) {
  return (word * 4u + cls) | pos << 8 | wext << 16 | shift << 24;
}
PackPlan make_pack_plan(int D, const unsigned __int128* max_abs, const uint64_t* or_abs, bool neg_seen, uint64_t n_slab_pods, bool pad_odd,
                        uint32_t max_words = kPackMaxWords, int headroom_bits = kPackHeadroomBits);

struct ViewPatch {
  uint64_t* vc_meta;
  uint16_t* vc_latom;
  int64_t* vc_req;
  uint64_t* vc_pk;
  int64_t* vc_rows;
  int32_t* pos_c;
  unsigned long long* n_c;
  int64_t cap_c;
  uint64_t* va_meta;
  uint16_t* va_latom;
  int32_t* pos_a;
  int64_t rows_a;
  uint32_t by_ns;
  uint32_t* dirty;
  PackPlan pk;
};

__host__ __device__ inline uint32_t atom_slot(uint32_t atom, uint32_t mask) { return ((atom * 0x9E3779B1u) >> 7) & mask; }

struct IndexDev {
  uint32_t* slow_thr = nullptr;
  uint32_t n_slow = 0;
  unsigned char* bm_blob = nullptr;
  BmChunk* bm_chunks = nullptr;
  uint32_t* bm_rank_t = nullptr;
  uint32_t* thr_ngrp = nullptr;
  uint32_t* nogroup = nullptr;
  uint32_t* grp_arrive = nullptr;
  uint32_t n_nogroup = 0;
  size_t cap_thr_ngrp = 0, cap_nogroup = 0, cap_grp_arrive = 0;
  uint32_t* bm_chunk_ns = nullptr;
  uint32_t ns_words = 0;
  uint64_t* atom_table = nullptr;
  uint32_t atom_mask = 0;
  std::vector<BmChunk> h_chunks;
  uint32_t n_chunks = 0, bm_max_lds = 0, bm_max_thr = 0, bm_max_words = 0, bm_rows = 0;
  uint64_t bm_slab_bytes = 0;
  uint32_t has_veto = 0, max_need = 0, n_atoms = 0, has_key_atoms = 0, la = 8;
  uint32_t bm_words = 0;
  uint32_t cut_thr_bytes = 0;
  bool has_long = false;
  bool rich = false;
  size_t cap_bm_blob = 0, cap_bm_chunks = 0, cap_bm_rank_t = 0, cap_bm_chunk_ns = 0, cap_atom_table = 0, cap_slow = 0;
};

void build_index(HostIndex& out, const std::vector<uint32_t>& thr_term_off, const std::vector<uint32_t>& term_thr,
                 const std::vector<uint8_t>& term_flags, const std::vector<uint32_t>& term_req_off,
                 const std::vector<uint8_t>& req_op, const std::vector<uint32_t>& req_key,
                 const std::vector<uint32_t>& req_val_off, const std::vector<uint32_t>& req_val,
                 const std::function<ThrInfo(uint32_t)>& thr_info, uint32_t n_ns,
                 const std::vector<uint32_t>& ns_term_ok, uint32_t gw, uint32_t agg_budget, uint32_t chk_budget, uint32_t thr_bytes,
                 int max_labels, const std::vector<uint32_t>* adm_in = nullptr, uint32_t chk_budget_full = 0,
                 uint32_t chk_word = kCheckWordLds, const HostIndex* atoms_from = nullptr, uint32_t thr_bytes_packed = 0);
void transpose_term_ns_bits(const std::vector<uint32_t>& in, size_t G, uint32_t nsw, uint32_t n_ns, uint32_t gw, std::vector<uint32_t>& out);
void parallel_for(size_t n, size_t min_per_part, const std::function<void(size_t, size_t, size_t)>& f, size_t* parts_out);
void cut_chunks(HostIndex& out, uint32_t agg_budget, uint32_t chk_budget, uint32_t thr_bytes, uint32_t chk_word = kCheckWordLds,
                uint32_t thr_bytes_packed = 0);
void index_group_counts(HostIndex& h, uint32_t T);
hipError_t upload_index(const HostIndex& h, IndexDev& d, hipStream_t s);
void release_index(IndexDev& d);

inline uint32_t atom_slots(uint32_t n_keys, int L) {
  const uint32_t ub = std::min<uint32_t>((uint32_t)L, n_keys);
  return ub <= 8 ? 8u : ub <= 16 ? 16u : 32u;
}

struct PodTable;
struct SelProgram;
uint32_t aggregate_fixed_lds();
uint32_t check_fixed_lds();
uint32_t check_word_lds(int D);
constexpr int kMatchPlanes = 8;
constexpr int kMatchReplay = 4;
struct MatchCacheArgs {
  const uint64_t* mw = nullptr;
  uint64_t stride = 0;
  uint32_t planes = 0;
  mutable bool used = false;
};
struct AggScan {
  int64_t n = 0;
  const int64_t* rows = nullptr;
  int64_t row0 = 0;
  bool counts = false;
  int sign = 1;
  bool nonneg = false;
  bool overflow_pods = false;
  bool by_ns = false;
  const uint64_t* v_meta = nullptr;
  const uint16_t* v_latom = nullptr;
  const int64_t* v_req = nullptr;
  uint32_t* slab_tag = nullptr;
  uint32_t epoch = 0;
  const uint32_t* wg_range = nullptr;
  int wg_range_G = 0;
  const PackPlan* pk = nullptr;
  const uint64_t* v_pk = nullptr;
  int limb = 0;
  bool small_window = false;
  bool defer_reduce = false;
  bool one_per_cu = false;
  mutable int launched_blocks = 0;
  mutable bool launched_packed = false;
  mutable const char* refused = nullptr;
};
constexpr int kAggWorkgroups = 256, kAggWorkgroupsTwo = 512;
constexpr uint32_t kSlabTagStride = kAggWorkgroupsTwo;
inline uint64_t agg_slab_area_bytes(uint32_t n_thr, uint32_t thr_bytes) {
  return (uint64_t)kAggWorkgroups * (((uint64_t)n_thr * thr_bytes + 15) & ~15ull) + 8192ull;
}
int aggregate_blocks(int64_t n_rows);
int aggregate_blocks(int64_t n_rows, int max_wg);
uint64_t aggregate_slab_pods(int64_t n_rows, int blocks);
struct AggTwoLaunch {
  bool enabled;
  bool small_window;
  bool overflow_pods;
  int pod_LA;
};
bool aggregate_two_per_cu_fits(const IndexDev& ix, const PackPlan& pk, const AggTwoLaunch& launch);
const char* launch_aggregate_indexed(const PodTable& pods, const AggScan& scan, const SelProgram& sp, const SelProgram* sp_dev,
                              const IndexDev& ix, unsigned long long* partial, void* slab, hipStream_t s,
                              const std::function<void()>& after_scan = nullptr);
struct ThrTables;
struct ReconcileOut;
struct ReqBound;
void launch_reduce_finalize_packed(const ThrTables& tt, const SelProgram& sp, int D, const IndexDev& ix, const PackPlan& pk, const void* slab,
                                   int n_slabs, const uint32_t* slab_tag, uint32_t epoch, unsigned long long* partial, bool consume, int64_t now_s,
                                   int32_t now_ns, bool apply, const ReconcileOut& out, void* recs, int rec_DT, bool rec_eq, const ReqBound& vmax,
                                   hipStream_t s, const uint8_t* row_mask, bool scan_adds_rows);
constexpr int64_t kCheckSmallMax = 256;
struct CheckSmall {
  uint32_t* ticket;
  uint64_t* host_summary;
  uint32_t n_inline;
  int64_t inline_rows[8];
};
struct CheckByNs {
  const uint64_t* v_meta;
  const uint16_t* v_latom;
  uint64_t* carry;
  const unsigned char* wv_img = nullptr;
  uint32_t wv_total_words = 0;
  const uint32_t* wg_range = nullptr;
  int wg_range_G = 0;
};
bool match_cache_fits(const IndexDev& ix);
bool check_replays_match_cache(const PodTable& pods, const SelProgram& sp, const IndexDev& ix, uint32_t planes, bool overflow_pods, bool one_per_cu);
bool launch_build_match_cache(const PodTable& pods, int64_t n, const int64_t* rows_dev, const IndexDev& ix, uint64_t* mw, uint64_t stride,
                              uint32_t planes, hipStream_t s);
int check_sweep_blocks(int64_t n);
size_t verdict_images_bytes(uint32_t total_words, int D);
void launch_build_verdict_images(const IndexDev& ix, uint32_t total_words, const void* recs, int T, int D, void* out, hipStream_t s);
const char* launch_check_indexed(const PodTable& pods, int64_t n, const int64_t* rows_dev, const SelProgram& sp,
                          const SelProgram* sp_dev, const IndexDev& ix, const void* recs, uint64_t* summary,
                          uint8_t* status, hipStream_t s, const CheckSmall* small = nullptr, bool overflow_pods = false,
                          const CheckByNs* by_ns = nullptr, bool one_per_cu = false, const MatchCacheArgs* mc = nullptr);
const char* launch_sweep_indexed(const PodTable& pods, int64_t n, const SelProgram& sp, const SelProgram* sp_dev, const IndexDev& ix,
                                 const void* recs, uint64_t* summary, const PackPlan& pk, void* slab, uint32_t* slab_tag, uint32_t epoch,
                                 int* launched_blocks, hipStream_t s);
bool launch_check_few(const PodTable& pods, int n, const int64_t* rows_host, const SelProgram& sp, const IndexDev& ix, const void* recs,
                      unsigned long long* acc, uint32_t* ticket, uint64_t* host_summary, uint64_t* host_seq, uint64_t seq, hipStream_t s);
void launch_translate_pods(const PodTable& pods, int64_t n, const int64_t* rows_dev, int64_t row0, const IndexDev& ix,
                           unsigned long long* n_overflow, hipStream_t s);

}
```

### kube_throttler_amd/csrc/kt_kernels_aggregate.hip

```cpp
#include <cstdio>
#include <type_traits>

#include "kt_scan.h"

namespace kt {

__host__ __device__ inline uint32_t agg_tab_bytes(uint32_t n_thr, int D, bool counts) { return n_thr * agg_rec_bytes(D, counts); }

template <int DT, bool PK>
constexpr int pk_words() { return PK ? (DT > 8 ? 8 : 4) : 1; }
template <int DT, int LA, bool PK>
struct TileRecAgg {
  uint32_t p;
  uint64_t meta;
  u32x4 raw[LA / 8];
  int64_t v[PK ? 1 : DT];
  unsigned long long pw[pk_words<DT, PK>()];
};

struct BmAggArgs {
  const uint64_t* meta;
  const uint16_t* latom;
  const int64_t* req;
  const uint32_t* lpair;
// ... 218 lines not shown
#pragma unroll
          for (int d = 0; d < DT; ++d) v[d] = limb_of(cur.v[d], a.limb);
        } else {
#pragma unroll
          for (int k = 0; k < NW; ++k) pw[k] = cur.pw[k];
        }
        const uint32_t zero_keys = present & ~(uint32_t)(meta >> kMetaNzShift) & 0xFFFFu;
        uint32_t ro[LA];
        atom_row_offsets<LA>(raw, ro);

        const bool overflow = a.has_overflow && countable && (meta & kMetaOverflow) != 0;
        const bool scan_counted = counted && !overflow;
        if (ci == first_ci && r0 == 0u && (a.n_slow || a.has_overflow))
          agg_walk_without_rank(a.sp, a.slow_thr, a.n_slow, a.T, a.lpair, a.lkey, a.LS, a.req, D, DS, a.partial, a.sign, a.limb, p, ns, countable,
                                counted, overflow, present);

        uint32_t last_r = 0xFFFFFFFFu;
        const uint32_t pk_nw = __builtin_amdgcn_readfirstlane(a.pk.nw);
        auto add_words = [&](lds_u64wp tv) {
          if constexpr (NW > 4) {
#pragma unroll
            for (int k = 0; k < 5; ++k) lds_add64(tv + k, pw[k]);
            if (pk_nw > 5u) lds_add64(tv + 5, pw[5]);
            if (pk_nw > 6u) lds_add64(tv + 6, pw[6]);
            if (pk_nw > 7u) lds_add64(tv + 7, pw[7]);
          } else {
            lds_add64(tv, pw[0]);
            if (pk_nw > 1u) lds_add64(tv + 1, pw[1]);
            if (pk_nw > 2u) lds_add64(tv + 2, pw[2]);
            if (pk_nw > 3u) lds_add64(tv + 3, pw[3]);
          }
        };
        auto add_match = [&](bool has, uint32_t tr) {
              const uint32_t r = tr & 0x7FFFu;
              const bool ok = has && !((tr & kRankAdj) && r == last_r);
              if (ok) last_r = r;
              if (ok && (!WIN || r - r0 < nrec)) {
                KT_LDS unsigned char* rp = tab + __umul24(WIN ? r - r0 : r, rec);
                lds_u64wp tv = (lds_u64wp)rp;
                if constexpr (PK) {
                  add_words(tv);
                  if (zero_keys) (void)__hip_atomic_fetch_or((lds_u32wp)(rp + a.pk.nw * 8u), zero_keys, __ATOMIC_RELAXED, __HIP_MEMORY_SCOPE_WORKGROUP);
                  return;
                }
                lds_u32wp tu = (lds_u32wp)(rp + (uint32_t)D * 8);
#pragma unroll
                for (int d = 0; d < DT; ++d)
                  if (v[d] != 0) lds_add64(tv + d, (unsigned long long)v[d]);
                if (counts) {
#pragma unroll
                  for (int d = 0; d < DT; ++d)
                    if ((present >> d) & 1u) lds_add(tu + d, 1u);
                  lds_add(tu + D, 1u);
                } else {
                  if (need_pres) (void)__hip_atomic_fetch_or(tu, present, __ATOMIC_RELAXED, __HIP_MEMORY_SCOPE_WORKGROUP);
                  lds_add(tu + 1, 1u);
                }
              }
        };
        auto confirm_slow = [&](uint32_t c) {
          return term_match_mem(*a.sp, bm.term_g[c], a.lpair + (uint64_t)p * (uint32_t)a.LS, a.lkey + (uint64_t)p * (uint32_t)a.LS, a.LS);
        };
        if constexpr (kFoldQueue) {
          constexpr int kWq = 4;
          uint64_t qx[kWq];
          typedef typename std::conditional<(kWq > 3), uint64_t, uint32_t>::type qw_t;
          static_assert(kWq * 10 <= 64, "ten bits per queued word number");
          qw_t qw = 0;
          uint32_t qn = 0u;
#pragma unroll
          for (int k = 0; k < kWq; ++k) qx[k] = 0ull;
          auto add_rank = [&](bool has, uint32_t r) {
            if (has && (!WIN || r - r0 < nrec)) {
              KT_LDS unsigned char* rp = tab + __umul24(WIN ? r - r0 : r, rec);
              lds_u64wp tv = (lds_u64wp)rp;
              add_words(tv);
              if (zero_keys) (void)__hip_atomic_fetch_or((lds_u32wp)(rp + a.pk.nw * 8u), zero_keys, __ATOMIC_RELAXED, __HIP_MEMORY_SCOPE_WORKGROUP);
            }
          };
          auto flush = [&]() {
            while (__ballot(qn != 0u) != 0ull) {
              const bool has = qn != 0u;
              const uint32_t cw = ((uint32_t)qw & 1023u) * 64u;
              const uint32_t c = cw + (uint32_t)__ffsll((unsigned long long)qx[0]) - 1u;
              qx[0] &= qx[0] - 1ull;
              const uint32_t r = trank[has ? c : 0u] & 0x7FFFu;
              if (has && qx[0] == 0ull) {
#pragma unroll
                for (int k = 0; k + 1 < kWq; ++k) qx[k] = qx[k + 1];
                qx[kWq - 1] = 0ull;
                qw >>= 10;
                qn -= 1u;
              }
              add_rank(has, r);
            }
          };
          const bool seg_on = ch.has_adj != 0u;
          KT_LDS const u64x2* segp = (KT_LDS const u64x2*)(lds + a.off_seg);
          scan_tile<LA, VETO, NEED, VETO>(
              bm, scan_counted, ns, ro, [&](bool, uint32_t) {}, confirm_slow,
              [&](uint32_t w, uint64_t x, const u64x2& seg) -> uint64_t {
                if (seg_on) {
                  const uint64_t v = x | seg.y;
                  x = andn_64(x, v - seg.x);
                }
                if (__ballot(x != 0ull && qn >= (uint32_t)kWq) != 0ull) flush();
                if (x != 0ull) {
#pragma unroll
                  for (int k = kWq - 1; k > 0; --k) qx[k] = qx[k - 1];
                  qx[0] = x;
                  qw = (qw_t)(qw << 10) | (qw_t)w;
                  qn += 1u;
                }
                return 0ull;
              },
              [&](uint32_t w) -> u64x2 { return seg_on ? segp[w] : u64x2{0ull, 0ull}; });
          flush();
        } else if constexpr (PK) {
          scan_tile<LA, VETO, NEED, VETO>(
              bm, scan_counted, ns, ro, [&](bool, uint32_t) {}, confirm_slow,
              [&](uint32_t w, uint64_t x, int) -> uint64_t {
                uint64_t xf = x;
                while (__ballot(xf != 0ull) != 0ull) {
                  const bool h1 = xf != 0ull;
                  const uint32_t c1 = h1 ? w * 64u + (uint32_t)__ffsll((unsigned long long)xf) - 1u : 0u;
                  xf &= xf - 1ull;
                  const bool h2 = xf != 0ull;
                  const uint32_t c2 = h2 ? w * 64u + (uint32_t)__ffsll((unsigned long long)xf) - 1u : 0u;
                  xf &= xf - 1ull;
                  const uint32_t tr1 = trank[c1], tr2 = trank[c2];
                  add_match(h1, tr1);
                  add_match(h2, tr2);
                }
                return 0ull;
              });
        } else {
          scan_tile<LA, VETO, NEED, VETO>(
              bm, scan_counted, ns, ro, [&](bool has, uint32_t c) { add_match(has, trank[c]); }, confirm_slow);
        }
      }
      __syncthreads();
      u32x4* dst = (u32x4*)(a.slab + (size_t)ch.slab_off * 16 + (size_t)blockIdx.x * slab_pitch + (size_t)r0 * rec);
      lds_u4p src = (lds_u4p)(lds + a.off_tab);
      for (uint32_t i = threadIdx.x; i < tab_bytes / 16; i += kBlockIx) dst[i] = src[i];
    }
    if (threadIdx.x == 0) a.slab_tag[ci * kSlabTagStride + blockIdx.x] = a.epoch;
  }
}

struct BmAggOneArgs {
  const uint64_t* v_meta;
  const uint16_t* v_latom;
  const uint64_t* v_pk;
  unsigned char* slab;
  BmIndexArgs ix;
  BmChunk ch;
  uint32_t n_rows, tpb;
  uint32_t off_rank, off_tab, off_seg;
  uint32_t tab_bytes;
  uint32_t pk_nw, pk_stride, pk_rec, skew;
};
__device__ __forceinline__ uint32_t agg_one_rec_off(uint32_t r, uint32_t rec, uint32_t skew) { return __umul24(r, rec) + (skew ? (r >> 3) << 3 : 0u); }

template <bool VETO, int NEED>
__global__ __launch_bounds__(kBlockIx, 8) void kt_aggregate_bitmap_one(const BmAggOneArgs a) {
  constexpr int LA = 8, NW = 3, kWq = VETO ? 3 : 4;
  KT_LDS unsigned char* lds = (KT_LDS unsigned char*)kt_smem;
  const uint32_t lane = threadIdx.x & (kWave - 1);
  const uint32_t wave = __builtin_amdgcn_readfirstlane(threadIdx.x / kWave);
  const uint32_t n_rows = a.n_rows;
  const uint32_t n_wtiles = (n_rows + kWave - 1u) / kWave;
  const uint32_t t_lo = min(blockIdx.x * a.tpb, n_wtiles), t_hi = min(t_lo + a.tpb, n_wtiles);
  const BmChunk& ch = a.ch;
  const uint32_t rec = a.pk_rec, skew = a.skew, pk_nw = a.pk_nw;
  KT_LDS const uint16_t* trank = (KT_LDS const uint16_t*)(lds + a.off_rank);
  KT_LDS unsigned char* tab = lds + a.off_tab;
  struct Rec {
    uint64_t meta;
    u32x4 raw;
    unsigned long long pw[NW];
  };
  auto fetch_tile = [&](uint32_t wt) {
    Rec r;
    const uint32_t ic = min(wt * kWave + lane, n_rows - 1u);
    r.meta = a.v_meta[ic];
    r.raw = *(const u32x4*)(a.v_latom + (uint64_t)ic * LA);
    const u64x2* q = (const u64x2*)(a.v_pk + (uint64_t)ic * a.pk_stride);
    const u64x2 q0 = q[0];
    r.pw[0] = q0.x, r.pw[1] = q0.y, r.pw[2] = 0ull;
    if (a.pk_stride > 2u) r.pw[2] = q[1].x;
    return r;
  };
  for (uint32_t i = threadIdx.x; i < a.tab_bytes / 4; i += kBlockIx) ((lds_u32wp)tab)[i] = 0u;
  {
    const StageSeg segs[2] = {chunk_image_segment(a.ix, ch),
                              StageSeg{a.off_rank, (const u32x4*)(a.ix.blob + ch.img_off + ch.off_term_rank), ch.n_words * 8u}};
    lds_stage_segments<2, 4>(lds, segs);
  }
  if (ch.has_adj) {
    const uint16_t* g_rank = (const uint16_t*)(a.ix.blob + ch.img_off + ch.off_term_rank);
    for (uint32_t w = wave; w < ch.n_words; w += (uint32_t)(kBlockIx / kWave)) {
      const uint32_t tr = g_rank[w * 64u + lane];
      const uint32_t tp = (uint32_t)__shfl_up((int)tr, 1), tn = (uint32_t)__shfl_down((int)tr, 1);
      const bool adj = (tr & kRankAdj) != 0u;
      const bool same_prev = lane > 0u && adj && tp == tr, same_next = lane < 63u && adj && tn == tr;
      const uint64_t m_lo = __ballot(!same_prev), m_hi = __ballot(!same_next);
      if (lane < 2u) ((lds_u64wp)(lds + a.off_seg))[w * 2u + lane] = lane == 0u ? m_lo : m_hi;
    }
  }
  const BmView bm = open_chunk<VETO>(lds, a.ix, ch);
  __syncthreads();
  const bool seg_on = ch.has_adj != 0u;
  KT_LDS const u64x2* segp = (KT_LDS const u64x2*)(lds + a.off_seg);
  for (uint32_t wt = t_lo + wave; wt < t_hi; wt += (uint32_t)(kBlockIx / kWave)) {
    const Rec cur = fetch_tile(wt);
    const bool in = wt * kWave + lane < n_rows;
    const uint64_t meta = cur.meta;
    const uint32_t st = (uint32_t)(meta >> kMetaStateShift) & 0xFu;
    const bool counted = in && (st & (kPodValid | kPodSchedMatch | kPodScheduled | kPodFinished)) == (kPodValid | kPodSchedMatch | kPodScheduled);
    if (__ballot(counted) == 0ull) continue;
    const uint32_t ns = counted ? (uint32_t)(meta & kMetaNsMask) : 0u;
    const uint32_t present = (uint32_t)(meta >> kMetaPresentShift) & 0xFFFFu;
    const uint32_t zero_keys = present & ~(uint32_t)(meta >> kMetaNzShift) & 0xFFFFu;
    unsigned long long pw[NW];
#pragma unroll
    for (int k = 0; k < NW; ++k) pw[k] = cur.pw[k];
    const u32x4 raw[1] = {cur.raw};
    uint32_t ro[LA];
    atom_row_offsets<LA>(raw, ro);
    uint64_t qx[kWq];
    typedef typename std::conditional<(kWq > 3), uint64_t, uint32_t>::type qw_t;
    qw_t qw = 0;
    uint32_t qn = 0u;
#pragma unroll
    for (int k = 0; k < kWq; ++k) qx[k] = 0ull;
    auto flush = [&]() {
      while (__ballot(qn != 0u) != 0ull) {
        const bool has = qn != 0u;
        const uint32_t cw = ((uint32_t)qw & 1023u) * 64u;
        const uint32_t c = cw + (uint32_t)__ffsll((unsigned long long)qx[0]) - 1u;
        qx[0] &= qx[0] - 1ull;
        const uint32_t r = trank[has ? c : 0u] & 0x7FFFu;
        if (has && qx[0] == 0ull) {
#pragma unroll
          for (int k = 0; k + 1 < kWq; ++k) qx[k] = qx[k + 1];
          qx[kWq - 1] = 0ull;
          qw >>= 10;
          qn -= 1u;
        }
        if (has) {
          KT_LDS unsigned char* rp = tab + agg_one_rec_off(r, rec, skew);
          lds_u64wp tv = (lds_u64wp)rp;
          lds_add64(tv, pw[0]);
          if (pk_nw > 1u) lds_add64(tv + 1, pw[1]);
          if (pk_nw > 2u) lds_add64(tv + 2, pw[2]);
          if (zero_keys) (void)__hip_atomic_fetch_or((lds_u32wp)(rp + pk_nw * 8u), zero_keys, __ATOMIC_RELAXED, __HIP_MEMORY_SCOPE_WORKGROUP);
        }
      }
    };
    scan_tile<LA, VETO, NEED, false>(
        bm, counted, ns, ro, [&](bool, uint32_t) {}, [&](uint32_t) { return true; },
        [&](uint32_t w, uint64_t x, const u64x2& seg) -> uint64_t {
          if (seg_on) {
            const uint64_t v = x | seg.y;
            x = andn_64(x, v - seg.x);
          }
          if (__ballot(x != 0ull && qn >= (uint32_t)kWq) != 0ull) flush();
          if (x != 0ull) {
#pragma unroll
            for (int k = kWq - 1; k > 0; --k) qx[k] = qx[k - 1];
            qx[0] = x;
            qw = (qw_t)(qw << 10) | (qw_t)w;
            qn += 1u;
          }
          return 0ull;
        },
        [&](uint32_t w) -> u64x2 { return seg_on ? segp[w] : u64x2{0ull, 0ull}; });
    flush();
  }
  __syncthreads();
  const uint32_t slab_pitch = (ch.n_thr * rec + 15u) & ~15u;
  u32x4* dst = (u32x4*)(a.slab + (size_t)blockIdx.x * slab_pitch);
  for (uint32_t i = threadIdx.x; i < slab_pitch / 16u; i += kBlockIx) {
    KT_LDS const u32x2* src = (KT_LDS const u32x2*)(tab + i * 16u + (skew ? (i >> 4) << 3 : 0u));
    const u32x2 lo = src[0], hi = src[1];
    dst[i] = u32x4{lo.x, lo.y, hi.x, hi.y};
  }
}

static BmAggOneArgs make_bm_agg_one_args(const IndexDev& ix, const PackPlan& pk, uint32_t* total) {
  BmAggOneArgs a{};
  uint32_t o = 0;
  auto take = [&](uint32_t bytes) { uint32_t r = o; o += (bytes + 15u) & ~15u; return r; };
  a.pk_nw = pk.nw, a.pk_stride = pk.stride, a.pk_rec = pk.rec_bytes, a.skew = pk.rec_bytes == 32u ? 1u : 0u;
  a.off_rank = take(ix.bm_max_words * 64u * 2u);
  a.tab_bytes = (ix.bm_max_thr * pk.rec_bytes + (a.skew ? ((ix.bm_max_thr + 7u) >> 3) * 8u : 0u) + 15u) & ~15u;
  a.off_tab = take(a.tab_bytes);
  a.off_seg = take(ix.bm_max_words * 16u);
  plan_bitmap_index(ix, a.ix, take);
  *total = o;
  return a;
}

bool aggregate_two_per_cu_fits(const IndexDev& ix, const PackPlan& pk, const AggTwoLaunch& launch) {
  if (!launch.enabled || launch.small_window || launch.overflow_pods || launch.pod_LA > 8) return false;
  if (ix.n_chunks != 1 || ix.h_chunks.size() != 1 || ix.n_slow != 0 || ix.has_long || ix.la > 8u || ix.max_need > 3u) return false;
  if (!pk.nw || pk.nw > 3u || pk.rec_bytes > 32u || pk.headroom < (uint32_t)kPackHeadroomBitsTwo) return false;
  const BmChunk& ch = ix.h_chunks[0];
  if (ch.has_slow || ch.n_thr == 0u) return false;
  uint32_t total = 0;
  (void)make_bm_agg_one_args(ix, pk, &total);
  if (2u * total > (uint32_t)kMaxLds) return false;
  const uint64_t pitch = ((uint64_t)ch.n_thr * pk.rec_bytes + 15u) & ~15ull;
  return (uint64_t)kAggWorkgroupsTwo * pitch <= agg_slab_area_bytes(ch.n_thr, ix.cut_thr_bytes);
}

constexpr int kSlabSplits = 4;
__global__ __launch_bounds__(256) void kt_reduce_bitmap_slabs(const unsigned char* slab, const BmChunk* chunks,
                                                              const uint32_t* rank_t, int n_slabs, int D, int counts, int sign,
                                                              const uint32_t* slab_tag, uint32_t epoch, unsigned long long* partial) {
  constexpr int G = 4;
  __shared__ unsigned long long part[G][64][4];
  const BmChunk ch = chunks[blockIdx.y];
  const uint32_t rec = agg_rec_bytes(D, counts != 0), ppr = rec / 16u;
  const uint32_t n_pieces = ch.n_thr * ppr;
  if (blockIdx.x * 64u >= n_pieces) return;
  const size_t pitch = (size_t)ch.n_thr * rec;
  const uint32_t wl = threadIdx.x & 63u, g = threadIdx.x >> 6;
  const uint32_t pi = blockIdx.x * 64u + wl;
  const bool in = pi < n_pieces;
  const uint32_t r = in ? pi / ppr : 0u, q = in ? pi - r * ppr : 0u;
  const uint32_t dw0 = q * 4u, n_val = 2u * (uint32_t)D, n_u32 = counts ? (uint32_t)D + 1u : 2u;
  uint32_t kind[4];
#pragma unroll
  for (int k = 0; k < 4; ++k) {
    const uint32_t dw = dw0 + k;
    kind[k] = dw < n_val ? 0u : dw < n_val + n_u32 ? ((!counts && dw == n_val) ? 2u : 1u) : 3u;
  }
  unsigned long long acc[4] = {0, 0, 0, 0};
  const unsigned char* base = slab + (size_t)ch.slab_off * 16 + (size_t)(in ? pi : 0u) * 16;
  const int step = G * kSlabSplits;
  const uint32_t* tag = slab_tag + blockIdx.y * kSlabTagStride;
#pragma unroll 8
  for (int b = (int)(blockIdx.z * G + g); b < n_slabs; b += step) {
    if (tag[b] != epoch) continue;
    const u32x4 x = *(const u32x4*)(base + (size_t)b * pitch);
    const uint32_t w[4] = {x.x, x.y, x.z, x.w};
#pragma unroll
    for (int h = 0; h < 2; ++h) {
      if (kind[2 * h] == 0u) {
        acc[2 * h] += (unsigned long long)w[2 * h] | (unsigned long long)w[2 * h + 1] << 32;
      } else {
        acc[2 * h] = kind[2 * h] == 2u ? (acc[2 * h] | w[2 * h]) : acc[2 * h] + w[2 * h];
        acc[2 * h + 1] = kind[2 * h + 1] == 2u ? (acc[2 * h + 1] | w[2 * h + 1]) : acc[2 * h + 1] + w[2 * h + 1];
      }
    }
  }
#pragma unroll
  for (int k = 0; k < 4; ++k) part[g][wl][k] = acc[k];
  __syncthreads();
  if (g == 0 && in) {
    const int stride = partial_stride(D);
    unsigned long long* prow = partial + (size_t)rank_t[ch.rank0 + r] * stride;
#pragma unroll
    for (int k = 0; k < 4; ++k) {
      if (kind[k] == 3u || (kind[k] == 0u && (k & 1))) continue;
      unsigned long long sum = 0;
#pragma unroll
      for (int gg = 0; gg < G; ++gg) sum = kind[k] == 2u ? (sum | part[gg][wl][k]) : sum + part[gg][wl][k];
      if (sum == 0ull) continue;
      const uint32_t dw = dw0 + k;
      if (kind[k] == 0u) {
        atomicAdd(prow + dw / 2u, (unsigned long long)((long long)sign * (long long)sum));
      } else if (kind[k] == 2u) {
        for (int d = 0; d < D; ++d)
          if ((sum >> d) & 1ull) atomicAdd(prow + partial_off_presence(D) + d, 1ull);
      } else {
        const uint32_t u = dw - n_val;
        const int j = counts ? (u < (uint32_t)D ? partial_off_presence(D) + (int)u : partial_off_pods(D)) : partial_off_pods(D);
        atomicAdd(prow + j, (unsigned long long)((long long)sign * (long long)sum));
      }
    }
  }
}

template <int NL>
__global__ __launch_bounds__(kRecBlock) void kt_reduce_packed_slabs(const unsigned char* slab, const BmChunk* chunks, const uint32_t* rank_t,
                                                                   int n_slabs, int D, const PackPlan pk, const uint32_t* slab_tag, uint32_t epoch,
                                                                   int check_tags, unsigned long long* partial) {
  __shared__ RecSumsLds lds;
  const BmChunk ch = chunks[blockIdx.y];
  const uint32_t units = pk.rec_bytes >> 3, rb = RecSlabLoads<NL>::kTileUnits / units;
  const uint32_t rec0 = blockIdx.x * rb;
  if (rec0 >= ch.n_thr) return;
  const uint32_t nrec = min(rb, ch.n_thr - rec0);
  const uint32_t x = threadIdx.x, g = x >> 4, d = x & 15u;
  const size_t pitch = ((size_t)ch.n_thr * pk.rec_bytes + 15u) & ~(size_t)15u;
  RecSlabLoads<NL> sl;
  record_slabs_live(n_slabs, slab_tag + blockIdx.y * kSlabTagStride, epoch, check_tags, sl);
  uint32_t t = 0;
  if (g < nrec) t = rank_t[ch.rank0 + rec0 + g];
  record_slabs_issue(slab + (size_t)ch.slab_off * 16 + (size_t)rec0 * pk.rec_bytes, pitch, nrec * units, sl);
  block_record_sums(sl, pk, lds);
  if (g >= nrec) return;
  const uint32_t ub = g * units;
  const unsigned long long pods = packed_pods(lds, ub, pk);
  if (pods == 0ull) return;
  unsigned long long* prow = partial + (size_t)t * partial_stride(D);
  if (d == 0u) atomicAdd(prow + partial_off_pods(D), pods);
  if (d < (uint32_t)D) {
    const unsigned long long mine = packed_field(lds, ub, packed_desc_of(pk, (int)d, D));
    if (mine) atomicAdd(prow + d, mine);
    if ((packed_zero_keys(lds, ub, pk) >> d) & 1u) atomicAdd(prow + partial_off_presence(D) + d, 1ull);
  }
}

#define KT_AGG_BM_LAUNCH(DT_, LA_, VETO_, NEED_, PK_, WIN_)                                                    \
  {                                                                                                           \
    auto kfn = kt_aggregate_bitmap<DT_, LA_, VETO_, NEED_, PK_, WIN_>;                                        \
    (void)hipFuncSetAttribute((const void*)kfn, hipFuncAttributeMaxDynamicSharedMemorySize, (int)lds_bm);     \
    hipLaunchKernelGGL(kfn, g_, b_, lds_bm, s, bm_args);                                                      \
  }
#define KT_AGG_BM_CASE(DT_, LA_, VETO_, NEED_)                                                                \
  {                                                                                                           \
    if (!packed && !windowed) KT_AGG_BM_LAUNCH(DT_, LA_, VETO_, NEED_, false, false)                          \
    else if (!packed) KT_AGG_BM_LAUNCH(DT_, LA_, VETO_, NEED_, false, true)                                   \
    else if (!windowed && !wide_pk) KT_AGG_BM_LAUNCH(8, LA_, VETO_, NEED_, true, false)                      \
    else if (!wide_pk) KT_AGG_BM_LAUNCH(8, LA_, VETO_, NEED_, true, true)                                     \
    else if (!windowed) KT_AGG_BM_LAUNCH(16, LA_, VETO_, NEED_, true, false)                                  \
    else KT_AGG_BM_LAUNCH(16, LA_, VETO_, NEED_, true, true)                                                  \
  }

static_assert(kAggWorkgroups == kCUs && kAggWorkgroupsTwo == 2 * kCUs, "one or two workgroups per CU");
static_assert(kAggWorkgroups <= 16 * kRecWaves && kAggWorkgroupsTwo <= 32 * kRecWaves, "the packed reductions take 16 or 32 slabs per wave");
static_assert(kAggWorkgroups <= 1 << kPackHeadroomBits && kAggWorkgroupsTwo <= 1 << kPackHeadroomBitsTwo, "headroom of the packed fields");
int aggregate_blocks(int64_t n_rows, int max_wg) {
  int64_t b = (n_rows + kBlockIx - 1) / kBlockIx;
  return (int)(b < 1 ? 1 : b > max_wg ? max_wg : b);
}
int aggregate_blocks(int64_t n_rows) { return aggregate_blocks(n_rows, kAggWorkgroups); }
uint64_t aggregate_slab_pods(int64_t n_rows, int blocks) {
  const int64_t tiles = (n_rows + kWave - 1) / kWave;
  const int64_t per_wg = (tiles + blocks - 1) / blocks + (kBlockIx / kWave);
  return (uint64_t)per_wg * kWave;
}

const char* launch_aggregate_indexed(const PodTable& pods, const AggScan& sc, const SelProgram& sp, const SelProgram* sp_dev,
                              const IndexDev& ix, unsigned long long* partial, void* slab_, hipStream_t s,
                              const std::function<void()>& after_scan) {
  const int64_t n_rows = sc.n;
  if (n_rows <= 0 || sp.T <= 0) return "";
  const int DT = dt_bucket_ix(pods.D), LA = pods.LA;
  unsigned char* slab = (unsigned char*)slab_;
  uint32_t bm_total = 0;
  BmAggArgs bm_args = make_bm_agg_args(pods, sc, sp, sp_dev, ix, partial, slab, &bm_total);
  if (bm_total > (uint32_t)kMaxLds) return nullptr;
  const bool packed = bm_args.v_pk != nullptr && bm_args.ix.by_ns && !sc.counts && sc.sign == 1 && sc.nonneg &&
                      bm_args.pk.rec_bytes <= ix.cut_thr_bytes && !ix.has_long;
  if (bm_args.v_pk != nullptr && !packed) return nullptr;
  if (!packed && agg_rec_bytes(pods.D, sc.counts) > ix.cut_thr_bytes) return nullptr;
  const bool two_per_cu = packed && aggregate_two_per_cu_fits(ix, bm_args.pk, AggTwoLaunch{!sc.one_per_cu, sc.small_window, sc.overflow_pods, LA});
  if (packed && bm_args.pk.headroom >= (uint32_t)kPackHeadroomBitsTwo && !two_per_cu) {
    sc.refused = "the packed words were planned for two workgroups per CU and this launch cannot run that form";
    return nullptr;
  }
  int nb = aggregate_blocks(n_rows, two_per_cu ? kAggWorkgroupsTwo : kAggWorkgroups);
  if (two_per_cu) bm_args.wg_range = nullptr;
  if (bm_args.ix.by_ns && bm_args.wg_range) {
    if (ix.n_chunks == 1) bm_args.wg_range = nullptr;
  }
  if (bm_args.ix.by_ns && !bm_args.wg_range) {
    const int64_t tiles = (n_rows + kWave - 1) / kWave, tpb = (tiles + nb - 1) / nb;
    nb = (int)((tiles + tpb - 1) / tpb);
  }
  {
    const uint32_t rec_bytes = packed ? bm_args.pk.rec_bytes : agg_rec_bytes(pods.D, sc.counts);
    for (const BmChunk& ch : ix.h_chunks)
      if ((uint64_t)nb * (((uint64_t)ch.n_thr * rec_bytes + 15u) & ~15ull) > agg_slab_area_bytes(ch.n_thr, ix.cut_thr_bytes)) {
        sc.refused = "the slabs of the launch's workgroups do not fit the chunk's slab area";
        return nullptr;
      }
  }
  dim3 g_(nb), b_(kBlockIx);
  const size_t lds_bm = bm_total;
  if (two_per_cu) {
    uint32_t one_total = 0;
    BmAggOneArgs oa = make_bm_agg_one_args(ix, bm_args.pk, &one_total);
    const BmChunk& ch = ix.h_chunks[0];
    oa.v_meta = sc.v_meta, oa.v_latom = sc.v_latom, oa.v_pk = sc.v_pk, oa.ch = ch;
    oa.slab = slab + (size_t)ch.slab_off * 16;
    oa.n_rows = (uint32_t)n_rows;
    oa.tpb = (uint32_t)((((n_rows + kWave - 1) / kWave) + nb - 1) / nb);
    static const bool dbg_one = getenv("KT_DEBUG_LDS") != nullptr;
    if (dbg_one)
      fprintf(stderr, "kt_aggregate_bitmap_one: lds=%u (2 per CU) workgroups=%d tiles per workgroup=%u nw=%u rec=%u skew=%u\n", one_total, nb, oa.tpb,
              oa.pk_nw, oa.pk_rec, oa.skew);
#define KT_AGG_ONE_LAUNCH(VETO_, NEED_)                                                                          \
  {                                                                                                             \
    auto kfn = kt_aggregate_bitmap_one<VETO_, NEED_>;                                                           \
    (void)hipFuncSetAttribute((const void*)kfn, hipFuncAttributeMaxDynamicSharedMemorySize, (int)one_total);    \
    hipLaunchKernelGGL(kfn, g_, b_, one_total, s, oa);                                                          \
  }
#ifdef KT_FAST_BUILD
    KT_AGG_ONE_LAUNCH(false, 2)
#else
    if (!ix.rich) KT_AGG_ONE_LAUNCH(false, 2) else KT_AGG_ONE_LAUNCH(true, 3)
#endif
#undef KT_AGG_ONE_LAUNCH
  } else {
  const bool windowed = bm_args.win_recs != 0u;
  const bool wide_pk = packed && bm_args.pk.nw > 4u;
  static const bool dbg_lds = getenv("KT_DEBUG_LDS") != nullptr;
  if (dbg_lds)
    fprintf(stderr, "kt_aggregate_bitmap: lds=%u chunks=%u largest LDS part=%u max thr=%u T=%d packed=%d nw=%u rec=%u\n", bm_total, ix.n_chunks,
            ix.bm_max_lds, ix.bm_max_thr, sp.T, packed ? 1 : 0, bm_args.pk.nw, bm_args.pk.rec_bytes);
#ifdef KT_FAST_BUILD
  KT_AGG_BM_CASE(8, 8, false, 2)
#else
  if (!ix.rich) { if (DT <= 8) KT_AGG_BM_CASE(8, 8, false, 2) else KT_AGG_BM_CASE(16, 8, false, 2) }
  else if (ix.max_need > 3u) {
    if (LA <= 8) { if (DT <= 8) KT_AGG_BM_CASE(8, 8, true, 5) else KT_AGG_BM_CASE(16, 8, true, 5) }
    else if (LA <= 16) { if (DT <= 8) KT_AGG_BM_CASE(8, 16, true, 5) else KT_AGG_BM_CASE(16, 16, true, 5) }
    else { if (DT <= 8) KT_AGG_BM_CASE(8, 32, true, 5) else KT_AGG_BM_CASE(16, 32, true, 5) }
  }
  else if (LA <= 8) { if (DT <= 8) KT_AGG_BM_CASE(8, 8, true, 3) else KT_AGG_BM_CASE(16, 8, true, 3) }
  else if (LA <= 16) { if (DT <= 8) KT_AGG_BM_CASE(8, 16, true, 3) else KT_AGG_BM_CASE(16, 16, true, 3) }
  else { if (DT <= 8) KT_AGG_BM_CASE(8, 32, true, 3) else KT_AGG_BM_CASE(16, 32, true, 3) }
#endif
  }
  if (after_scan) after_scan();
  sc.launched_blocks = nb, sc.launched_packed = packed;
  if (packed && sc.defer_reduce) {
  } else if (packed) {
    const uint32_t rb_ = (uint32_t)(nb > 16 * kRecWaves ? kRecTileUnits / 2 : kRecTileUnits) / (bm_args.pk.rec_bytes >> 3);
    if (ix.bm_max_thr > 0 && nb > 16 * kRecWaves)
      hipLaunchKernelGGL(kt_reduce_packed_slabs<32>, dim3((ix.bm_max_thr + rb_ - 1u) / rb_, ix.n_chunks), dim3(kRecBlock), 0, s, slab,
                         ix.bm_chunks, ix.bm_rank_t, nb, pods.D, bm_args.pk, sc.slab_tag, sc.epoch, ix.n_chunks > 1 ? 1 : 0, partial);
    else if (ix.bm_max_thr > 0)
      hipLaunchKernelGGL(kt_reduce_packed_slabs<16>, dim3((ix.bm_max_thr + rb_ - 1u) / rb_, ix.n_chunks), dim3(kRecBlock), 0, s, slab,
                         ix.bm_chunks, ix.bm_rank_t, nb, pods.D, bm_args.pk, sc.slab_tag, sc.epoch, ix.n_chunks > 1 ? 1 : 0, partial);
  } else {
    const uint32_t max_pieces = ix.bm_max_thr * (agg_rec_bytes(pods.D, sc.counts) / 16u);
    if (max_pieces > 0)
      hipLaunchKernelGGL(kt_reduce_bitmap_slabs, dim3((max_pieces + 63) / 64, ix.n_chunks, kSlabSplits), dim3(256), 0, s, slab,
                         ix.bm_chunks, ix.bm_rank_t, nb, pods.D, sc.counts ? 1 : 0, sc.sign, sc.slab_tag, sc.epoch, partial);
  }
  return packed ? (ix.n_chunks == 1 ? "kt_aggregate_bitmap_packed" : "kt_aggregate_bitmap_packed_chunked")
                : (ix.n_chunks == 1 ? "kt_aggregate_bitmap" : "kt_aggregate_bitmap_chunked");
}

}
```

### kube_throttler_amd/csrc/kt_kernels_match.hip

```cpp
#include "kt_scan.h"

namespace kt {

struct MatchBuildArgs {
  const uint64_t* meta;
  const uint16_t* latom;
  const int64_t* rows;
  uint64_t* mw;
  uint64_t stride;
  uint32_t planes;
  uint32_t n;
  uint32_t cap;
  BmIndexArgs ix;
  BmChunk ch;
};

template <bool VETO, int NEED>
__global__ __launch_bounds__(kBlockIx) void kt_build_match_cache(const MatchBuildArgs a) {
  constexpr int LA = 8;
  KT_LDS unsigned char* lds = (KT_LDS unsigned char*)kt_smem;
  const uint32_t lane = threadIdx.x & (kWave - 1);
  const uint32_t wave = __builtin_amdgcn_readfirstlane(threadIdx.x / kWave);
  const BmChunk& ch = a.ch;
  {
    const StageSeg segs[1] = {chunk_image_segment(a.ix, ch)};
    lds_stage_segments<1, 4>(lds, segs);
  }
  const BmView bm = open_chunk<VETO>(lds, a.ix, ch);
  __syncthreads();
  const uint32_t n = a.n, planes = a.planes;
  const uint32_t n_wtiles = (n + kWave - 1u) / kWave;
  const uint32_t wstep = gridDim.x * (uint32_t)(kBlockIx / kWave);
  for (uint32_t wt = blockIdx.x * (uint32_t)(kBlockIx / kWave) + wave; wt < n_wtiles; wt += wstep) {
    const uint32_t i = wt * kWave + lane;
    const uint32_t ic = min(i, n - 1u);
    const uint32_t p = a.rows ? (uint32_t)a.rows[ic] : ic;
    const bool in = i < n && p < a.cap;
    const uint32_t pc = min(p, a.cap - 1u);
    const uint64_t meta = a.meta[pc];
    u32x4 raw[1];
    load_atoms<LA>(a.latom, (int64_t)pc, raw);
    const bool on = in && ((meta >> kMetaStateShift) & kPodValid) != 0;
    const uint32_t ns = on ? (uint32_t)(meta & kMetaNsMask) : 0u;
    uint32_t ro[LA];
    atom_row_offsets<LA>(raw, ro);
    uint64_t* q = a.mw + pc;
    uint32_t round = 0u;
    scan_tile<LA, VETO, NEED, false>(
        bm, on, ns, ro, [&](bool, uint32_t) {}, [&](uint32_t) { return true; },
        [&](uint32_t, uint64_t xx, int) -> uint64_t {
          if (in && round < planes) q[(uint64_t)round * a.stride] = xx;
          round += 1u;
          return 0ull;
        });
    for (; round < planes; ++round)
      if (in) q[(uint64_t)round * a.stride] = 0ull;
  }
}

bool match_cache_fits(const IndexDev& ix) {
  if (ix.n_chunks != 1 || ix.h_chunks.size() != 1 || ix.n_slow != 0 || ix.has_long || ix.la > 8u || ix.max_need > 3u) return false;
  const BmChunk& ch = ix.h_chunks[0];
  return !ch.has_slow && ch.n_words != 0u && ix.bm_max_lds <= (uint32_t)kMaxLds;
}

bool launch_build_match_cache(const PodTable& pods, int64_t n, const int64_t* rows_dev, const IndexDev& ix, uint64_t* mw, uint64_t stride,
                              uint32_t planes, hipStream_t s) {
  if (n <= 0) return true;
  if (!match_cache_fits(ix) || pods.LA > 8 || !mw || planes == 0u || planes > (uint32_t)kMatchPlanes || stride == 0u || n > (int64_t)stride)
    return false;
  MatchBuildArgs a{};
  a.meta = pods.meta, a.latom = pods.latom, a.rows = rows_dev, a.mw = mw, a.stride = stride, a.planes = planes;
  a.n = (uint32_t)n, a.cap = (uint32_t)std::min<uint64_t>(stride, 0x80000000ull);
  uint32_t o = 0;
  auto take = [&](uint32_t bytes) { uint32_t r = o; o += (bytes + 15u) & ~15u; return r; };
  plan_bitmap_index(ix, a.ix, take);
  a.ch = ix.h_chunks[0];
  const uint32_t lds_bytes = o;
  const int64_t tiles = (n + kWave - 1) / kWave, per_wg = kBlockIx / kWave;
  const int64_t nb = std::min<int64_t>((tiles + per_wg - 1) / per_wg, 2 * kCUs);
  dim3 g_((unsigned)nb), b_(kBlockIx);
#define KT_MATCH_LAUNCH(VETO_, NEED_)                                                                           \
  {                                                                                                             \
    auto kfn = kt_build_match_cache<VETO_, NEED_>;                                                              \
    (void)hipFuncSetAttribute((const void*)kfn, hipFuncAttributeMaxDynamicSharedMemorySize, (int)lds_bytes);    \
    hipLaunchKernelGGL(kfn, g_, b_, lds_bytes, s, a);                                                           \
  }
#ifdef KT_FAST_BUILD
  KT_MATCH_LAUNCH(false, 2)
#else
  if (!ix.rich) KT_MATCH_LAUNCH(false, 2) else KT_MATCH_LAUNCH(true, 3)
#endif
#undef KT_MATCH_LAUNCH
  return true;
}

}
```

### kube_throttler_amd/engine.py

```python
from __future__ import annotations

import ctypes as C
import os
import subprocess

import numpy as np

from . import snapshot as S

_HERE = os.path.dirname(os.path.abspath(__file__))
_CSRC = os.path.join(_HERE, "csrc")
LIB_PATH = os.path.join(_CSRC, "libkt_engine.so")
if os.environ.get("KT_ENGINE_LIB"):
    LIB_PATH = os.path.abspath(os.environ["KT_ENGINE_LIB"])
_LIB = None

KT_OK = 0
ERR_NAMES = {-1: "KT_ERR_INVALID_ARGUMENT", -2: "KT_ERR_OUT_OF_RANGE", -3: "KT_ERR_DEVICE", -4: "KT_ERR_OVERFLOW_RISK",
             -5: "KT_ERR_NOT_READY", -6: "KT_ERR_NO_DEVICE", -7: "KT_ERR_UNSUPPORTED"}
RECONCILE_APPLY = 0x1
ADMIT_COMMIT = 0x1
VARIANT_INCREMENTAL = 0x100
CHECK_STATUS_MATRIX = 0x1
KERNEL_CHECK, KERNEL_AGGREGATE, KERNEL_FINALIZE, KERNEL_PREPARE, KERNEL_REDUCE = 0, 1, 2, 3, 4
VARIANT_INDEXED, VARIANT_DENSE = 0, 1

EXPORTS = [
    "kt_version", "kt_engine_create", "kt_engine_destroy", "kt_last_error", "kt_upsert_namespaces", "kt_upsert_pods",
    "kt_upsert_throttles", "kt_delete_namespaces", "kt_delete_pods", "kt_delete_throttles", "kt_load_snapshot",
    "kt_set_reserved", "kt_set_status", "kt_reconcile_launch", "kt_aggregate_launch", "kt_partial_used_buffer",
    "kt_use_partial_buffer", "kt_finalize_launch", "kt_reconcile_fetch", "kt_check_launch", "kt_check_fetch", "kt_throttle_rows", "kt_sweep_launch",
    "kt_check_device_summary", "kt_fetch_pod_requests", "kt_timing_enable", "kt_timing_read", "kt_timing_reset",
    "kt_synchronize", "kt_kernel_name", "kt_admit_launch", "kt_fetch_reserved", "kt_reconcile_fetch_next_override",
    "kt_check", "kt_upsert_namespace", "kt_upsert_pod", "kt_upsert_throttle", "kt_comm_unique_id", "kt_comm_init",
    "kt_comm_allreduce_partial", "kt_comm_destroy", "kt_reconcile_rows_launch", "kt_set_exchange_world", "kt_counter", "kt_reconcile_fetch_used_hi",
    "kt_set_wide_sums", "kt_partial_words", "kt_partial_layout", "kt_debug_reload_env", "kt_affected_pods", "kt_paged_check", "kt_paged_reconcile",
    "kt_paged_admit", "kt_admit_gangs_launch", "kt_admit_gangs_fetch", "kt_paged_admit_gangs",
    "kt_headroom_launch", "kt_headroom_fetch", "kt_paged_headroom", "kt_preempt_launch", "kt_preempt_fetch",
    "kt_preempt_reprieve_launch", "kt_preempt_gangs_launch", "kt_preempt_gangs_reprieve_launch", "kt_preempt_gangs_fetch", "kt_forecast_launch", "kt_forecast_fetch", "kt_override_instants",
    "kt_paged_preempt",
]
HEADROOM_MAX_CAP = 0x7FFFFFFF
PREEMPT_NONE = -1
PREEMPT_REPRIEVE = 0x1
FORECAST_NONE = -1
COUNTER_FEW_CHECKS, COUNTER_COMPILES, COUNTER_INDEX_CHUNKS, COUNTER_INDEX_WORDS, COUNTER_NS_WORD_VISITS, COUNTER_NS_ROWS = range(6)
COUNTER_NS_CHUNK_VISITS, COUNTER_INDEX_IMAGE_WORDS, COUNTER_SLOW_THROTTLES, COUNTER_PACKED_WORDS = 6, 7, 8, 9
COUNTER_AGG_WORKGROUPS = 11
COUNTER_VIEW_BUILDS = 10
COUNTER_MATCH_CACHE_BUILDS, COUNTER_MATCH_CACHE_SCANS, COUNTER_MATCH_CACHE_PLANES = 12, 13, 14


def partial_layout(n_dims: int) -> dict:
    v = [C.c_int32() for _ in range(5)]
    rc = lib().kt_partial_layout(int(n_dims), *[C.byref(x) for x in v])
    if rc != KT_OK:
        raise EngineError(rc, f"kt_partial_layout({n_dims})")
    return dict(zip(("stride", "values", "presence", "pods", "errors"), (int(x.value) for x in v)))


def version() -> str:
    return lib().kt_version().decode()


def paged_check(engines, n, rows=None, on_equal=False):
    hs = (C.c_void_p * len(engines))(*[e._h for e in engines])
    T = engines[0].throttle_rows()
    rows_a = None if rows is None else np.ascontiguousarray(rows, dtype=np.int64)
    if rows_a is None:
        rows_a = np.arange(n, dtype=np.int64)
    status = np.zeros((max(n, 1), max(T, 1)), np.uint8)
    summary = np.zeros(max(n, 1), np.uint64)
    rc = lib().kt_paged_check(hs, len(engines), n, rows_a.ctypes.data, int(on_equal), summary.ctypes.data, status.ctypes.data)
    if rc != KT_OK:
        raise EngineError(rc, "kt_paged_check: " + "; ".join(lib().kt_last_error(e._h).decode() for e in engines))
    return status[:n, :T], summary[:n]


def paged_admit(engines, rows, on_equal=False, commit=False):
    hs = (C.c_void_p * len(engines))(*[e._h for e in engines])
    T = engines[0].throttle_rows()
    rows_a = np.ascontiguousarray(rows, dtype=np.int64)
    n = len(rows_a)
    status = np.zeros((max(n, 1), max(T, 1)), np.uint8)
    summary = np.zeros(max(n, 1), np.uint64)
    rc = lib().kt_paged_admit(hs, len(engines), n, rows_a.ctypes.data if n else None, int(on_equal),
                              ADMIT_COMMIT if commit else 0, summary.ctypes.data, status.ctypes.data)
    if rc != KT_OK:
        raise EngineError(rc, "kt_paged_admit: " + "; ".join(lib().kt_last_error(e._h).decode() for e in engines))
    return status[:n, :T], summary[:n]


def _gang_offsets(gang_off):
    g = np.ascontiguousarray(gang_off, dtype=np.int64)
    if g.ndim != 1 or len(g) < 1:
        raise ValueError("gang_off: [n_gangs + 1] offsets, starting at 0 and ending at the queue length")
    return g


def paged_admit_gangs(engines, rows, gang_off, on_equal=False, commit=False):
    hs = (C.c_void_p * len(engines))(*[e._h for e in engines])
    T = engines[0].throttle_rows()
    rows_a = np.ascontiguousarray(rows, dtype=np.int64)
    g = _gang_offsets(gang_off)
    n, ng = len(rows_a), len(g) - 1
    status = np.zeros((max(n, 1), max(T, 1)), np.uint8)
    summary = np.zeros(max(n, 1), np.uint64)
    admitted = np.zeros(max(ng, 1), np.uint8)
    rc = lib().kt_paged_admit_gangs(hs, len(engines), n, rows_a.ctypes.data if n else None, ng, g.ctypes.data, int(on_equal),
                                    ADMIT_COMMIT if commit else 0, summary.ctypes.data, status.ctypes.data, admitted.ctypes.data)
    if rc != KT_OK:
        raise EngineError(rc, "kt_paged_admit_gangs: " + "; ".join(lib().kt_last_error(e._h).decode() for e in engines))
    return status[:n, :T], summary[:n], admitted[:ng]


def paged_headroom(engines, rows, cap, on_equal=False):
    hs = (C.c_void_p * len(engines))(*[e._h for e in engines])
    rows_a = np.ascontiguousarray(rows, dtype=np.int64)
    n = len(rows_a)
    copies = np.zeros(max(n, 1), np.int64)
    limiting = np.zeros(max(n, 1), np.int32)
    rc = lib().kt_paged_headroom(hs, len(engines), n, rows_a.ctypes.data if n else None, int(on_equal), int(cap),
                                 copies.ctypes.data, limiting.ctypes.data)
    if rc != KT_OK:
        raise EngineError(rc, "kt_paged_headroom: " + "; ".join(lib().kt_last_error(e._h).decode() for e in engines))
    return copies[:n], limiting[:n]


def paged_preempt(engines, pod_rows, cand_rows, now, on_equal=False, reprieve=False, want_victims=True):
    hs = (C.c_void_p * len(engines))(*[e._h for e in engines])
    a = np.ascontiguousarray(pod_rows, dtype=np.int64)
    c = np.ascontiguousarray(cand_rows, dtype=np.int64)
    n, m = len(a), len(c)
    prefix = np.zeros(max(n, 1), np.int64)
    flat = np.zeros(max(n * m, 1), np.uint8) if want_victims else None
    rc = lib().kt_paged_preempt(hs, len(engines), n, a.ctypes.data if n else None, m, c.ctypes.data if m else None, int(now[0]), int(now[1]),
                                int(on_equal), PREEMPT_REPRIEVE if reprieve else 0, prefix.ctypes.data,
                                None if flat is None else flat.ctypes.data)
    if rc != KT_OK:
        raise EngineError(rc, "kt_paged_preempt: " + "; ".join(lib().kt_last_error(e._h).decode() for e in engines))
    return prefix[:n], (None if flat is None else flat[:n * m].reshape(n, m))


def paged_reconcile(engines, now, apply=True):
    hs = (C.c_void_p * len(engines))(*[e._h for e in engines])
    T = engines[0].throttle_rows()
    results = [ReconcileResult(T, e.D) for e in engines]
    structs = (KtStatus * len(engines))(*[r.as_struct() for r in results])
    replaced, err = np.zeros(max(T, 1), np.uint8), np.zeros(max(T, 1), np.uint8)
    rc = lib().kt_paged_reconcile(hs, len(engines), int(now[0]), int(now[1]), RECONCILE_APPLY if apply else 0, T, structs,
                                  replaced.ctypes.data, err.ctypes.data)
    if rc != KT_OK:
        raise EngineError(rc, "kt_paged_reconcile: " + "; ".join(lib().kt_last_error(e._h).decode() for e in engines))
    return results, replaced[:T], err[:T]


class EngineError(RuntimeError):
    def __init__(self, code, msg):
        super().__init__(f"{ERR_NAMES.get(code, code)}: {msg}")
        self.code = code


class KtConfig(C.Structure):
    _fields_ = [("n_dims", C.c_int32), ("max_labels", C.c_int32), ("pod_capacity", C.c_int64),
                ("throttle_capacity", C.c_int32), ("namespace_capacity", C.c_int32), ("device", C.c_int32),
                ("kernel_variant", C.c_int32)]


class KtStatus(C.Structure):
    _fields_ = [("used", S.KtAmounts), ("calc", S.KtAmounts), ("calc_at_nonzero", C.POINTER(C.c_uint8)),
                ("thrl_flag", C.POINTER(C.c_uint32)), ("thrl_has", C.POINTER(C.c_uint32)),
                ("thrl_pod", C.POINTER(C.c_uint8)), ("msgs_fp", C.POINTER(C.c_uint64)),
                ("error", C.POINTER(C.c_uint8))]


def build(force: bool = False) -> str:
    args = ["make", "-C", _CSRC, "-j8"]
    if force:
        args.append("-B")
    subprocess.check_call(args, stdout=subprocess.DEVNULL)
    return LIB_PATH


def lib():
    global _LIB
    if _LIB is None:
        if not os.path.exists(LIB_PATH):
            raise EngineError(-6, f"{LIB_PATH} is missing: build it with kube_throttler_amd.engine.build() "
                                  "(there is no CPU fallback)")
        L = C.CDLL(LIB_PATH)
        L.kt_version.restype = C.c_char_p
        L.kt_last_error.restype = C.c_char_p
        L.kt_last_error.argtypes = [C.c_void_p]
        L.kt_kernel_name.restype = C.c_char_p
        L.kt_kernel_name.argtypes = [C.c_void_p, C.c_int32]
        L.kt_engine_create.argtypes = [C.POINTER(KtConfig), C.POINTER(C.c_void_p)]
        L.kt_engine_destroy.argtypes = [C.c_void_p]
        for name in ("kt_upsert_namespaces", "kt_upsert_pods", "kt_upsert_throttles"):
            getattr(L, name).argtypes = [C.c_void_p, C.POINTER(S.KtSnapshot), C.c_void_p]
        L.kt_delete_namespaces.argtypes = [C.c_void_p, C.c_int32, C.c_void_p]
        L.kt_delete_pods.argtypes = [C.c_void_p, C.c_int64, C.c_void_p]
        L.kt_delete_throttles.argtypes = [C.c_void_p, C.c_int32, C.c_void_p]
        L.kt_load_snapshot.argtypes = [C.c_void_p, C.POINTER(S.KtSnapshot)]
# ... 109 lines not shown
        try:
            self.close()
        except Exception:
            pass

    def _ck(self, rc):
        if rc != KT_OK:
            raise EngineError(rc, lib().kt_last_error(self._h).decode())

    def load_snapshot(self, snap: S.Snapshot):
        st = snap.as_struct()
        self._ck(lib().kt_load_snapshot(self._h, C.byref(st)))

    @staticmethod
    def _rows(rows, dtype):
        if rows is None:
            return None, None
        a = np.ascontiguousarray(rows, dtype=dtype)
        return a, a.ctypes.data

    def upsert_namespaces(self, batch: S.Snapshot, rows=None):
        st = batch.as_struct()
        a, p = self._rows(rows, np.int32)
        self._ck(lib().kt_upsert_namespaces(self._h, C.byref(st), p))

    def upsert_pods(self, batch: S.Snapshot, rows=None):
        st = batch.as_struct()
        a, p = self._rows(rows, np.int64)
        self._ck(lib().kt_upsert_pods(self._h, C.byref(st), p))

    def upsert_throttles(self, batch: S.Snapshot, rows=None):
        st = batch.as_struct()
        a, p = self._rows(rows, np.int32)
        self._ck(lib().kt_upsert_throttles(self._h, C.byref(st), p))

    def delete_pods(self, rows):
        a, p = self._rows(rows, np.int64)
        self._ck(lib().kt_delete_pods(self._h, len(a), p))

    def delete_throttles(self, rows):
        a, p = self._rows(rows, np.int32)
        self._ck(lib().kt_delete_throttles(self._h, len(a), p))

    def delete_namespaces(self, rows):
        a, p = self._rows(rows, np.int32)
        self._ck(lib().kt_delete_namespaces(self._h, len(a), p))

    def set_reserved(self, rows, amounts: S.Amounts):
        a, p = self._rows(rows, np.int32)
        st = amounts.as_struct()
        self._ck(lib().kt_set_reserved(self._h, len(a), p, C.byref(st)))

    def set_status(self, rows, used: S.Amounts, calc: S.Amounts, calc_at_nonzero, thrl_flag, thrl_has, thrl_pod,
                   msgs_fp=None):
        a, p = self._rows(rows, np.int32)
        n = len(a)
        keep = [np.ascontiguousarray(calc_at_nonzero, np.uint8), np.ascontiguousarray(thrl_flag, np.uint32),
                np.ascontiguousarray(thrl_has, np.uint32), np.ascontiguousarray(thrl_pod, np.uint8),
                np.ascontiguousarray(msgs_fp if msgs_fp is not None else np.zeros(n), np.uint64)]
        st = KtStatus(used.as_struct(), calc.as_struct(), keep[0].ctypes.data_as(C.POINTER(C.c_uint8)),
                      keep[1].ctypes.data_as(C.POINTER(C.c_uint32)), keep[2].ctypes.data_as(C.POINTER(C.c_uint32)),
                      keep[3].ctypes.data_as(C.POINTER(C.c_uint8)), keep[4].ctypes.data_as(C.POINTER(C.c_uint64)), None)
        self._ck(lib().kt_set_status(self._h, n, p, C.byref(st)))

    def reconcile_launch(self, now, apply=True, stream=None):
        self._ck(lib().kt_reconcile_launch(self._h, int(now[0]), int(now[1]), RECONCILE_APPLY if apply else 0, stream))

    def reconcile_rows(self, now, rows, apply=True) -> "ReconcileResult":
        rows = np.ascontiguousarray(rows, dtype=np.int32)
        self._ck(lib().kt_reconcile_rows_launch(self._h, int(now[0]), int(now[1]), RECONCILE_APPLY if apply else 0,
                                                len(rows), rows.ctypes.data_as(C.c_void_p), None))
        return self.reconcile_fetch()

    def aggregate_launch(self, stream=None):
        self._ck(lib().kt_aggregate_launch(self._h, stream))

    def partial_used_buffer(self):
        ptr, n = C.c_void_p(), C.c_int64()
        self._ck(lib().kt_partial_used_buffer(self._h, C.byref(ptr), C.byref(n)))
        return ptr.value, n.value

    def use_partial_buffer(self, device_ptr, n_int64):
        self._ck(lib().kt_use_partial_buffer(self._h, device_ptr, n_int64))

    @staticmethod
    def comm_unique_id() -> bytes:
        buf = C.create_string_buffer(128)
        rc = lib().kt_comm_unique_id(buf)
        if rc != 0:
            raise EngineError(rc, lib().kt_last_error(None).decode())
        return buf.raw

    def comm_init(self, rank: int, world: int, unique_id: bytes):
        self._ck(lib().kt_comm_init(self._h, rank, world, C.create_string_buffer(unique_id, 128)))

    def comm_allreduce_partial(self, stream=None):
        self._ck(lib().kt_comm_allreduce_partial(self._h, stream))

    def comm_destroy(self):
        self._ck(lib().kt_comm_destroy(self._h))

    def reconcile_fetch_used_hi(self, n=None):
        n = self.throttle_rows() if n is None else n
        hi = np.zeros((max(n, 1), self.D), np.int64)
        anyw = C.c_int32()
        self._ck(lib().kt_reconcile_fetch_used_hi(self._h, n, hi.ctypes.data_as(C.c_void_p), C.byref(anyw)))
        return hi[:n], bool(anyw.value)

    def few_checks_served(self) -> int:
        return int(lib().kt_counter(self._h, 0))

    def compiles(self) -> int:
        return int(lib().kt_counter(self._h, 1))

    def set_exchange_world(self, world: int):
        self._ck(lib().kt_set_exchange_world(self._h, world))

    def affected_pods(self, pod_rows, throttle_rows):
        pr = np.ascontiguousarray(pod_rows, dtype=np.int64)
        tr = np.ascontiguousarray(throttle_rows, dtype=np.int32)
        out = np.zeros((max(len(pr), 1), max(len(tr), 1)), np.uint8)
        self._ck(lib().kt_affected_pods(self._h, len(pr), pr.ctypes.data, len(tr), tr.ctypes.data, out.ctypes.data))
        return out[:len(pr), :len(tr)]

    def reload_env(self):
        self._ck(lib().kt_debug_reload_env(self._h))

    def index_stats(self) -> dict:
        ch, words, visits, rows, cvis, iw, slow = (int(lib().kt_counter(self._h, k)) for k in (
            COUNTER_INDEX_CHUNKS, COUNTER_INDEX_WORDS, COUNTER_NS_WORD_VISITS, COUNTER_NS_ROWS, COUNTER_NS_CHUNK_VISITS, COUNTER_INDEX_IMAGE_WORDS,
            COUNTER_SLOW_THROTTLES))
        return {"chunks": ch, "words": words, "image_words": iw, "namespace_rows": rows,
                "word_visits_per_namespace": round(visits / rows, 3) if rows > 0 else None,
                "chunks_per_namespace": round(cvis / rows, 3) if rows > 0 else None, "slow_throttles": slow}

    def packed_words(self) -> int:
        return int(lib().kt_counter(self._h, COUNTER_PACKED_WORDS))

    def aggregate_workgroups(self) -> int:
        return int(lib().kt_counter(self._h, COUNTER_AGG_WORKGROUPS))

    def view_builds(self) -> int:
        return int(lib().kt_counter(self._h, COUNTER_VIEW_BUILDS))

    def match_cache_builds(self) -> int:
        return int(lib().kt_counter(self._h, COUNTER_MATCH_CACHE_BUILDS))

    def match_cache_planes(self) -> int:
        return int(lib().kt_counter(self._h, COUNTER_MATCH_CACHE_PLANES))

    def match_cache_scans(self) -> int:
        return int(lib().kt_counter(self._h, COUNTER_MATCH_CACHE_SCANS))

    def partial_words(self) -> int:
        return self.throttle_rows() * partial_layout(self.D)["stride"]

    def set_wide_sums(self, mode: int):
        self._ck(lib().kt_set_wide_sums(self._h, mode))

    def pending_partial_words(self):
        n, w = C.c_int64(), C.c_int32()
        self._ck(lib().kt_partial_words(self._h, C.byref(n), C.byref(w)))
        return int(n.value), bool(w.value)

    def finalize_launch(self, now, apply=True, stream=None):
        self._ck(lib().kt_finalize_launch(self._h, int(now[0]), int(now[1]), RECONCILE_APPLY if apply else 0, stream))

    def throttle_rows(self) -> int:
        n = C.c_int32()
        self._ck(lib().kt_throttle_rows(self._h, C.byref(n)))
        return n.value

    def reconcile_fetch(self, n=None) -> ReconcileResult:
        n = self.throttle_rows() if n is None else n
        r = ReconcileResult(n, self.D)
        st = r.as_struct()
        self._ck(lib().kt_reconcile_fetch(self._h, n, C.byref(st)))
        return r

    def next_override(self, n=None):
        n = self.throttle_rows() if n is None else n
        sec, nsec, has = np.zeros(max(n, 1), np.int64), np.zeros(max(n, 1), np.int32), np.zeros(max(n, 1), np.uint8)
        self._ck(lib().kt_reconcile_fetch_next_override(self._h, n, sec.ctypes.data, nsec.ctypes.data, has.ctypes.data))
        return sec[:n], nsec[:n], has[:n]

    def reconcile(self, now, apply=True) -> ReconcileResult:
        self.reconcile_launch(now, apply)
        return self.reconcile_fetch()

    def check_launch(self, n, rows=None, on_equal=False, want_status=False, stream=None):
        a, p = self._rows(rows, np.int64)
        self._ck(lib().kt_check_launch(self._h, n, p, int(on_equal), CHECK_STATUS_MATRIX if want_status else 0, stream))

    def sweep_launch(self, now, apply=True, on_equal=False, stream=None):
        self._ck(lib().kt_sweep_launch(self._h, int(now[0]), int(now[1]), RECONCILE_APPLY if apply else 0, int(on_equal), stream))

    def check_fetch(self, n, want_status=False):
        T = self.throttle_rows()
        summary = np.zeros(max(n, 1), np.uint64)
        status = np.zeros((max(n, 1), max(T, 1)), np.uint8) if want_status else None
        self._ck(lib().kt_check_fetch(self._h, n, summary.ctypes.data, None if status is None else status.ctypes.data))
        return (None if status is None else status[:n, :T]), summary[:n]

    def check(self, rows=None, n=None, on_equal=False, want_status=True):
        n = len(rows) if rows is not None else n
        self.check_launch(n, rows, on_equal, want_status)
        return self.check_fetch(n, want_status)

    def check_atomic(self, rows=None, n=None, on_equal=False, want_status=True):
        a, p = self._rows(rows, np.int64)
        n = len(a) if a is not None else n
        T = self.throttle_rows()
        summary = np.zeros(max(n, 1), np.uint64)
        status = np.zeros((max(n, 1), max(T, 1)), np.uint8) if want_status else None
        self._ck(lib().kt_check(self._h, n, p, int(on_equal), summary.ctypes.data,
                                None if status is None else status.ctypes.data))
        return (None if status is None else status[:n, :T]), summary[:n]

    def checker(self, n: int, on_equal=False):
        rows = np.zeros(n, np.int64)
        summary = np.zeros(n, np.uint64)
        fn, h = lib().kt_check, self._h
        rp, sp, eq = C.c_void_p(rows.ctypes.data), C.c_void_p(summary.ctypes.data), int(on_equal)

        def call():
            rc = fn(h, n, rp, eq, sp, None)
            if rc != KT_OK:
                self._ck(rc)
        return rows, summary, call

    def admit(self, rows=None, n=None, on_equal=False, commit=False, want_status=True):
        a, p = self._rows(rows, np.int64)
        n = len(a) if a is not None else n
        self._ck(lib().kt_admit_launch(self._h, n, p, int(on_equal), ADMIT_COMMIT if commit else 0, None))
        return self.check_fetch(n, want_status)

    def admit_gangs(self, rows, gang_off, on_equal=False, commit=False, want_status=True):
        a, p = self._rows(rows, np.int64)
        g = _gang_offsets(gang_off)
        n, ng = len(a), len(g) - 1
        self._ck(lib().kt_admit_gangs_launch(self._h, n, p, ng, g.ctypes.data, int(on_equal), ADMIT_COMMIT if commit else 0, None))
        status, summary = self.check_fetch(n, want_status)
        return status, summary, self.admit_gangs_fetch(ng)

    def admit_gangs_fetch(self, n_gangs):
        admitted = np.zeros(max(n_gangs, 1), np.uint8)
        self._ck(lib().kt_admit_gangs_fetch(self._h, n_gangs, admitted.ctypes.data))
        return admitted[:n_gangs]

    def headroom_launch(self, n, rows=None, cap=1, on_equal=False, stream=None):
        a, p = self._rows(rows, np.int64)
        self._ck(lib().kt_headroom_launch(self._h, n, p, int(on_equal), int(cap), stream))

    def headroom_fetch(self, n, want_limiting=True):
        copies = np.zeros(max(n, 1), np.int64)
        limiting = np.zeros(max(n, 1), np.int32) if want_limiting else None
        self._ck(lib().kt_headroom_fetch(self._h, n, copies.ctypes.data, None if limiting is None else limiting.ctypes.data))
        return copies[:n], (None if limiting is None else limiting[:n])

    def headroom(self, rows=None, n=None, *, cap, on_equal=False):
        n = len(rows) if rows is not None else n
        self.headroom_launch(n, rows, cap, on_equal)
        return self.headroom_fetch(n)

    def preempt_launch(self, pod_rows, cand_rows, now, on_equal=False, stream=None):
        a, p = self._rows(pod_rows, np.int64)
        c, q = self._rows(cand_rows, np.int64)
        self._ck(lib().kt_preempt_launch(self._h, len(a), p if len(a) else None, len(c), q if len(c) else None, int(now[0]), int(now[1]),
                                         int(on_equal), stream))

    def preempt_reprieve_launch(self, pod_rows, cand_rows, now, on_equal=False, stream=None):
        a, p = self._rows(pod_rows, np.int64)
        c, q = self._rows(cand_rows, np.int64)
        self._ck(lib().kt_preempt_reprieve_launch(self._h, len(a), p if len(a) else None, len(c), q if len(c) else None, int(now[0]),
                                                  int(now[1]), int(on_equal), stream))

    def preempt_fetch(self, n, n_cand, want_victims=True):
        prefix = np.zeros(max(n, 1), np.int64)
        flat = np.zeros(max(n * n_cand, 1), np.uint8) if want_victims else None
        self._ck(lib().kt_preempt_fetch(self._h, n, prefix.ctypes.data, None if flat is None else flat.ctypes.data))
        return prefix[:n], (None if flat is None else flat[:n * n_cand].reshape(n, n_cand))

    def preempt(self, pod_rows, cand_rows, now, on_equal=False, want_victims=True, reprieve=False):
        (self.preempt_reprieve_launch if reprieve else self.preempt_launch)(pod_rows, cand_rows, now, on_equal)
        return self.preempt_fetch(len(pod_rows), len(cand_rows), want_victims)

    def preempt_gangs_launch(self, pod_rows, gang_off, cand_rows, now, on_equal=False, stream=None):
        a, p = self._rows(pod_rows, np.int64)
        c, q = self._rows(cand_rows, np.int64)
        g = _gang_offsets(gang_off)
        self._ck(lib().kt_preempt_gangs_launch(self._h, len(a), p if len(a) else None, len(g) - 1, g.ctypes.data, len(c), q if len(c) else None,
                                               int(now[0]), int(now[1]), int(on_equal), stream))

    def preempt_gangs_reprieve_launch(self, pod_rows, gang_off, cand_rows, now, on_equal=False, stream=None):
        a, p = self._rows(pod_rows, np.int64)
        c, q = self._rows(cand_rows, np.int64)
        g = _gang_offsets(gang_off)
        self._ck(lib().kt_preempt_gangs_reprieve_launch(self._h, len(a), p if len(a) else None, len(g) - 1, g.ctypes.data, len(c),
                                                        q if len(c) else None, int(now[0]), int(now[1]), int(on_equal), stream))

    def preempt_gangs_fetch(self, n_gangs, n_cand, want_victims=True):
        prefix = np.zeros(max(n_gangs, 1), np.int64)
        blocker = np.zeros(max(n_gangs, 1), np.int64)
        flat = np.zeros(max(n_gangs * n_cand, 1), np.uint8) if want_victims else None
        self._ck(lib().kt_preempt_gangs_fetch(self._h, n_gangs, prefix.ctypes.data, None if flat is None else flat.ctypes.data,
                                              blocker.ctypes.data))
# ... 74 lines not shown
```

Measured before the change: 21700 billion decisions/s.

## Replay cached selector match planes in the one-per-CU aggregate scan

Extends the match cache, previously used only by the check kernel, to the aggregate kernel. The per-pod match-plane words are gathered into the countable scan view's order, or written through during the cache build. A new cached instantiation of the bitmap aggregate kernel replays those words instead of loading label atoms and re-scanning the selector image, so it stages less index data into LDS. The cost is an extra view-ordered plane buffer, a gather kernel whenever the view or program changes, more invalidation state to keep consistent, and larger per-lane tile records.

```diff
diff --git a/include/kt_engine.h b/include/kt_engine.h
--- a/include/kt_engine.h
+++ b/include/kt_engine.h
@@ -177,6 +177,7 @@
 #define KT_COUNTER_MATCH_CACHE_BUILDS 12
 #define KT_COUNTER_MATCH_CACHE_SCANS 13
 #define KT_COUNTER_MATCH_CACHE_PLANES 14
+#define KT_COUNTER_MATCH_CACHE_AGG_SCANS 15
 int64_t kt_counter(kt_engine* e, int32_t which);
 int32_t kt_paged_check(kt_engine* const* pages, int32_t n_pages, int64_t n, const int64_t* pod_rows, int32_t on_equal,
                        uint64_t* out_summary, uint8_t* out_status);
diff --git a/kube_throttler_amd/csrc/kt_engine.cpp b/kube_throttler_amd/csrc/kt_engine.cpp
--- a/kube_throttler_amd/csrc/kt_engine.cpp
+++ b/kube_throttler_amd/csrc/kt_engine.cpp
@@ -506,6 +506,7 @@
     case KT_COUNTER_MATCH_CACHE_BUILDS: return e->ctr_mc_builds.load(std::memory_order_relaxed);
     case KT_COUNTER_MATCH_CACHE_SCANS: return e->ctr_mc_scans.load(std::memory_order_relaxed);
     case KT_COUNTER_MATCH_CACHE_PLANES: return e->ctr_mc_planes.load(std::memory_order_relaxed);
+    case KT_COUNTER_MATCH_CACHE_AGG_SCANS: return e->ctr_mc_agg_scans.load(std::memory_order_relaxed);
     default: return -1;
   }
 }
diff --git a/kube_throttler_amd/csrc/kt_engine_check.cpp b/kube_throttler_amd/csrc/kt_engine_check.cpp
--- a/kube_throttler_amd/csrc/kt_engine_check.cpp
+++ b/kube_throttler_amd/csrc/kt_engine_check.cpp
@@ -33,13 +33,22 @@
   const uint32_t planes = e->mc_planes;
   if (!kt::check_replays_match_cache(e->pods, e->sp, e->dindex, planes, e->n_overflow != 0, e->sw[kSw_CHECK_ONE_PER_CU])) return KT_OK;
   const uint64_t stride = (uint64_t)e->cfg.pod_capacity;
+  ScanView& cv = e->views.countable;
+  kt::MatchViewPlanes vp;
+  if (cv.valid && cv.mx_valid && cv.mx.p && cv.pos.p && cv.mx_planes == planes && e->mc_gen == e->program_gen)
+    vp.mx = cv.mx.p, vp.pos = cv.pos.p, vp.stride = (uint64_t)cv.cap + 1u;
+  else
+    cv.mx_valid = false;
   if (!e->mc_valid || e->mc_gen != e->program_gen) {
     if (e->d_mc.cap < (size_t)planes * stride) {
       if (e->last_stream) KT_HIP(e, hipStreamSynchronize(e->last_stream));
       KT_HIP(e, e->d_mc.reserve((size_t)planes * stride));
     }
     order_behind_ingest(e, s);
-    if (!kt::launch_build_match_cache(e->pods, e->pod_rows_hi, nullptr, e->dindex, e->d_mc.p, stride, planes, s)) return KT_OK;
+    if (!kt::launch_build_match_cache(e->pods, e->pod_rows_hi, nullptr, e->dindex, e->d_mc.p, stride, planes, s, &vp)) {
+      cv.mx_valid = false;
+      return KT_OK;
+    }
     KT_HIP(e, hipGetLastError());
     e->mc_valid = true, e->mc_gen = e->program_gen;
     e->mc_pending.clear();
@@ -54,8 +63,8 @@
     }
     memcpy(e->h_mc_rows, e->mc_pending.data(), n * 8);
     order_behind_ingest(e, s);
-    if (!kt::launch_build_match_cache(e->pods, (int64_t)n, e->h_mc_rows, e->dindex, e->d_mc.p, stride, planes, s)) {
-      e->mc_valid = false;
+    if (!kt::launch_build_match_cache(e->pods, (int64_t)n, e->h_mc_rows, e->dindex, e->d_mc.p, stride, planes, s, &vp)) {
+      e->mc_valid = false, cv.mx_valid = false;
       e->mc_pending.clear();
       return KT_OK;
     }
diff --git a/kube_throttler_amd/csrc/kt_engine_impl.h b/kube_throttler_amd/csrc/kt_engine_impl.h
--- a/kube_throttler_amd/csrc/kt_engine_impl.h
+++ b/kube_throttler_amd/csrc/kt_engine_impl.h
@@ -125,13 +125,16 @@
   DevBuf<uint64_t> pk;
   kt::PackPlan pack;
   DevBuf<int32_t> pos;
+  DevBuf<uint64_t> mx;
+  uint32_t mx_planes = 0;
+  bool mx_valid = false;
   DevBuf<uint32_t> range;
   int range_G = 0;
   int64_t cap = 0;
   int64_t extra = 0;
   bool by_ns = false;
   bool valid = false;
-  void release() { rows.release(); d_n.release(); meta.release(); latom.release(); req.release(); pk.release(); pos.release(); range.release(); }
+  void release() { rows.release(); d_n.release(); meta.release(); latom.release(); req.release(); pk.release(); pos.release(); range.release(); mx.release(); mx_valid = false; }
 };
 struct ViewSpec {
   bool countable_only;
@@ -188,8 +191,8 @@
 extern thread_local std::string g_create_error;
 
 
-enum EnvSwitch { kSw_FEED_NO_STAGE, kSw_FORCE_NS_ORDER, kSw_INGEST_EVENT_WAIT, kSw_NO_FEED_FEW, kSw_NO_FEED_FUSION, kSw_NO_FUSED, kSw_NO_NS_ORDER, kSw_NO_PACK, kSw_NO_SCAN_VIEW, kSw_NO_SWEEP, kSw_NO_VERDICT_IMAGES, kSw_NO_WG_RANGES, kSw_SYNC_INGEST, kSw_INGEST_TRUST_FENCE, kSw_NO_VIEW_PATCH, kSw_CHECK_ONE_PER_CU, kSw_AGG_SMALL_WINDOW, kSw_AGG_ONE_PER_CU, kSw_NO_MATCH_CACHE, kSwCount };
-static const char* const kEnvSwitchName[kSwCount] = {"KT_FEED_NO_STAGE", "KT_FORCE_NS_ORDER", "KT_INGEST_EVENT_WAIT", "KT_NO_FEED_FEW", "KT_NO_FEED_FUSION", "KT_NO_FUSED", "KT_NO_NS_ORDER", "KT_NO_PACK", "KT_NO_SCAN_VIEW", "KT_NO_SWEEP", "KT_NO_VERDICT_IMAGES", "KT_NO_WG_RANGES", "KT_SYNC_INGEST", "KT_INGEST_TRUST_FENCE", "KT_NO_VIEW_PATCH", "KT_CHECK_ONE_PER_CU", "KT_AGG_SMALL_WINDOW", "KT_AGG_ONE_PER_CU", "KT_NO_MATCH_CACHE"};
+enum EnvSwitch { kSw_FEED_NO_STAGE, kSw_FORCE_NS_ORDER, kSw_INGEST_EVENT_WAIT, kSw_NO_FEED_FEW, kSw_NO_FEED_FUSION, kSw_NO_FUSED, kSw_NO_NS_ORDER, kSw_NO_PACK, kSw_NO_SCAN_VIEW, kSw_NO_SWEEP, kSw_NO_VERDICT_IMAGES, kSw_NO_WG_RANGES, kSw_SYNC_INGEST, kSw_INGEST_TRUST_FENCE, kSw_NO_VIEW_PATCH, kSw_CHECK_ONE_PER_CU, kSw_AGG_SMALL_WINDOW, kSw_AGG_ONE_PER_CU, kSw_NO_MATCH_CACHE, kSw_NO_MATCH_CACHE_AGG, kSwCount };
+static const char* const kEnvSwitchName[kSwCount] = {"KT_FEED_NO_STAGE", "KT_FORCE_NS_ORDER", "KT_INGEST_EVENT_WAIT", "KT_NO_FEED_FEW", "KT_NO_FEED_FUSION", "KT_NO_FUSED", "KT_NO_NS_ORDER", "KT_NO_PACK", "KT_NO_SCAN_VIEW", "KT_NO_SWEEP", "KT_NO_VERDICT_IMAGES", "KT_NO_WG_RANGES", "KT_SYNC_INGEST", "KT_INGEST_TRUST_FENCE", "KT_NO_VIEW_PATCH", "KT_CHECK_ONE_PER_CU", "KT_AGG_SMALL_WINDOW", "KT_AGG_ONE_PER_CU", "KT_NO_MATCH_CACHE", "KT_NO_MATCH_CACHE_AGG"};
 struct kt_engine {
   bool sw[kSwCount] = {};
   uint32_t reprieve_lds_cap_limit = 0;
@@ -212,7 +215,7 @@
   ScanViews views;
   bool cut_plain = false;
   void* cur_launch_lock = nullptr;
-  std::atomic<int64_t> ctr_index_chunks{0}, ctr_index_words{0}, ctr_index_image_words{0}, ctr_ns_rows{0}, ctr_ns_word_visits{0}, ctr_ns_chunk_visits{0}, ctr_slow_throttles{0}, ctr_packed_words{0}, ctr_agg_workgroups{0}, ctr_view_builds{0}, ctr_mc_builds{0}, ctr_mc_scans{0}, ctr_mc_planes{0};
+  std::atomic<int64_t> ctr_index_chunks{0}, ctr_index_words{0}, ctr_index_image_words{0}, ctr_ns_rows{0}, ctr_ns_word_visits{0}, ctr_ns_chunk_visits{0}, ctr_slow_throttles{0}, ctr_packed_words{0}, ctr_agg_workgroups{0}, ctr_view_builds{0}, ctr_mc_builds{0}, ctr_mc_scans{0}, ctr_mc_planes{0}, ctr_mc_agg_scans{0};
   DevBuf<uint16_t> d_latom;
   DevBuf<uint64_t> d_mc;
   int64_t* h_mc_rows = nullptr;
diff --git a/kube_throttler_amd/csrc/kt_engine_reconcile.cpp b/kube_throttler_amd/csrc/kt_engine_reconcile.cpp
--- a/kube_throttler_amd/csrc/kt_engine_reconcile.cpp
+++ b/kube_throttler_amd/csrc/kt_engine_reconcile.cpp
@@ -206,6 +206,11 @@
   const kt::AggTwoLaunch two_launch{!e->sw[kSw_AGG_ONE_PER_CU], e->sw[kSw_AGG_SMALL_WINDOW], e->n_overflow != 0, e->pods.LA};
   if (cv.valid && cv.pack.headroom >= (uint32_t)kt::kPackHeadroomBitsTwo && !(two_view && kt::aggregate_two_per_cu_fits(e->dindex, cv.pack, two_launch)))
     cv.valid = false;
+  kt::MatchCacheArgs mc;
+  if (two_view && two_launch.enabled && !two_launch.small_window && !two_launch.overflow_pods && e->pods.LA <= 8 && !e->sw[kSw_NO_MATCH_CACHE_AGG] &&
+      !e->sw[kSw_CHECK_ONE_PER_CU]) {
+    if ((rc = match_cache_for_scan(e, s, mc)) != KT_OK) return rc;
+  }
   if (e->cfg.kernel_variant != 1 && (!cv.valid || cv.by_ns != by_ns)) {
     if (e->last_stream && e->last_stream != s) KT_HIP(e, hipStreamSynchronize(e->last_stream));
     const ViewSpec spec{true, by_ns, kt::aggregate_blocks, e->cfg.pod_capacity, true};
@@ -233,6 +238,19 @@
     }
     if (!e->sw[kSw_NO_SCAN_VIEW] && (rc = copy_view_records(e, cv, spec, headroom, s)) != KT_OK) return rc;
     cv.valid = true;
+  }
+  const bool replay = mc.mw != nullptr && mc.planes <= (uint32_t)kt::kMatchReplay && two_view && cv.valid && cv.pack.nw && cv.pk.p &&
+                      cv.pack.headroom >= (uint32_t)kt::kPackHeadroomBitsTwo && kt::aggregate_two_per_cu_fits(e->dindex, cv.pack, two_launch);
+  if (replay && !(cv.mx_valid && cv.mx_planes == mc.planes)) {
+    const size_t need = (size_t)mc.planes * ((size_t)cv.cap + 1);
+    if (cv.mx.cap < need) {
+      if (e->last_stream) KT_HIP(e, hipStreamSynchronize(e->last_stream));
+      KT_HIP(e, cv.mx.reserve(need));
+    }
+    const int64_t listed = std::min<int64_t>((int64_t)cv.n + cv.extra, cv.cap);
+    kt::launch_gather_match_planes(mc.mw, mc.stride, mc.planes, cv.rows.p, listed, cv.mx.p, (uint64_t)cv.cap + 1u, s);
+    KT_HIP(e, hipGetLastError());
+    cv.mx_planes = mc.planes, cv.mx_valid = true;
   }
   if (words && e->clean_partial != (const void*)e->partial()) KT_HIP(e, hipMemsetAsync(e->partial(), 0, words * 8, s));
   e->clean_partial = nullptr;
@@ -265,8 +283,10 @@
         if (sc.by_ns && cv.by_ns && cv.range_G) sc.wg_range = cv.range.p, sc.wg_range_G = cv.range_G;
         if ((rc = slab_tags(e, sc, s)) != KT_OK) return rc;
         sc.defer_reduce = defer && sc.pk != nullptr;
+        if (replay && sc.by_ns && sc.v_pk && limb == 0) sc.v_mx = cv.mx.p, sc.mx_stride = (uint64_t)cv.cap + 1u, sc.mx_planes = cv.mx_planes;
         const char* k = kt::launch_aggregate_indexed(e->pods, sc, e->sp, e->d_sp.p, e->dindex, target, e->d_slab.p, s,
                                                      pass == 0 ? std::function<void()>(after_scan) : std::function<void()>());
+        if (sc.replayed) e->ctr_mc_agg_scans.fetch_add(1, std::memory_order_relaxed);
         if (!k && sc.refused) return e->fail(KT_ERR_OUT_OF_RANGE, "aggregate launch refused: %s", sc.refused);
         if (!k) return e->fail(KT_ERR_UNSUPPORTED, "a chunk of the selector index exceeds the aggregate kernel's LDS budget (use kernel_variant 1)");
         e->last_kernel[KT_KERNEL_AGGREGATE] = k;
diff --git a/kube_throttler_amd/csrc/kt_engine_views.cpp b/kube_throttler_amd/csrc/kt_engine_views.cpp
--- a/kube_throttler_amd/csrc/kt_engine_views.cpp
+++ b/kube_throttler_amd/csrc/kt_engine_views.cpp
@@ -40,6 +40,7 @@
   ScanViews& vs = e->views;
   v.cap = (int64_t)v.n + headroom;
   v.extra = 0;
+  v.mx_valid = false;
   const size_t nc = (size_t)v.cap + 1, np = (size_t)spec.rows_cap + 1;
   KT_HIP(e, v.meta.reserve(nc));
   KT_HIP(e, v.latom.reserve(nc * (size_t)e->pods.LA));
diff --git a/kube_throttler_amd/csrc/kt_index.h b/kube_throttler_amd/csrc/kt_index.h
--- a/kube_throttler_amd/csrc/kt_index.h
+++ b/kube_throttler_amd/csrc/kt_index.h
@@ -214,6 +214,11 @@
   uint32_t planes = 0;
   mutable bool used = false;
 };
+struct MatchViewPlanes {
+  uint64_t* mx = nullptr;
+  const int32_t* pos = nullptr;
+  uint64_t stride = 0;
+};
 struct AggScan {
   int64_t n = 0;
   const int64_t* rows = nullptr;
@@ -236,6 +241,10 @@
   bool small_window = false;
   bool defer_reduce = false;
   bool one_per_cu = false;
+  const uint64_t* v_mx = nullptr;
+  uint64_t mx_stride = 0;
+  uint32_t mx_planes = 0;
+  mutable bool replayed = false;
   mutable int launched_blocks = 0;
   mutable bool launched_packed = false;
   mutable const char* refused = nullptr;
@@ -284,7 +293,9 @@
 bool match_cache_fits(const IndexDev& ix);
 bool check_replays_match_cache(const PodTable& pods, const SelProgram& sp, const IndexDev& ix, uint32_t planes, bool overflow_pods, bool one_per_cu);
 bool launch_build_match_cache(const PodTable& pods, int64_t n, const int64_t* rows_dev, const IndexDev& ix, uint64_t* mw, uint64_t stride,
-                              uint32_t planes, hipStream_t s);
+                              uint32_t planes, hipStream_t s, const MatchViewPlanes* view = nullptr);
+void launch_gather_match_planes(const uint64_t* mw, uint64_t stride, uint32_t planes, const int64_t* rows, int64_t n, uint64_t* mx,
+                                uint64_t mx_stride, hipStream_t s);
 int check_sweep_blocks(int64_t n);
 size_t verdict_images_bytes(uint32_t total_words, int D);
 void launch_build_verdict_images(const IndexDev& ix, uint32_t total_words, const void* recs, int T, int D, void* out, hipStream_t s);
diff --git a/kube_throttler_amd/csrc/kt_kernels_aggregate.hip b/kube_throttler_amd/csrc/kt_kernels_aggregate.hip
--- a/kube_throttler_amd/csrc/kt_kernels_aggregate.hip
+++ b/kube_throttler_amd/csrc/kt_kernels_aggregate.hip
@@ -394,6 +394,9 @@
   const uint64_t* v_meta;
   const uint16_t* v_latom;
   const uint64_t* v_pk;
+  const uint64_t* v_mx;
+  uint64_t mx_stride;
+  uint32_t mx_planes;
   unsigned char* slab;
   BmIndexArgs ix;
   BmChunk ch;
@@ -404,8 +407,9 @@
 };
 __device__ __forceinline__ uint32_t agg_one_rec_off(uint32_t r, uint32_t rec, uint32_t skew) { return __umul24(r, rec) + (skew ? (r >> 3) << 3 : 0u); }
 
-template <bool VETO, int NEED>
+template <bool VETO, int NEED, bool CACHED = false>
 __global__ __launch_bounds__(kBlockIx, 8) void kt_aggregate_bitmap_one(const BmAggOneArgs a) {
+  static_assert(!CACHED || (!VETO && NEED == 2), "the cached form is one instantiation: nothing of the scan's form is left in it");
   constexpr int LA = 8, NW = 3, kWq = VETO ? 3 : 4;
   KT_LDS unsigned char* lds = (KT_LDS unsigned char*)kt_smem;
   const uint32_t lane = threadIdx.x & (kWave - 1);
@@ -420,13 +424,21 @@
   struct Rec {
     uint64_t meta;
     u32x4 raw;
+    uint64_t mx[kMatchReplay];
     unsigned long long pw[NW];
   };
   auto fetch_tile = [&](uint32_t wt) {
-    Rec r;
+    Rec r{};
     const uint32_t ic = min(wt * kWave + lane, n_rows - 1u);
     r.meta = a.v_meta[ic];
-    r.raw = *(const u32x4*)(a.v_latom + (uint64_t)ic * LA);
+    if constexpr (CACHED) {
+      const uint64_t* q = a.v_mx + ic;
+#pragma unroll
+      for (int j = 0; j < kMatchReplay; ++j)
+        if ((uint32_t)j < a.mx_planes) r.mx[j] = q[(uint64_t)j * a.mx_stride];
+    } else {
+      r.raw = *(const u32x4*)(a.v_latom + (uint64_t)ic * LA);
+    }
     const u64x2* q = (const u64x2*)(a.v_pk + (uint64_t)ic * a.pk_stride);
     const u64x2 q0 = q[0];
     r.pw[0] = q0.x, r.pw[1] = q0.y, r.pw[2] = 0ull;
@@ -435,8 +447,10 @@
   };
   for (uint32_t i = threadIdx.x; i < a.tab_bytes / 4; i += kBlockIx) ((lds_u32wp)tab)[i] = 0u;
   {
-    const StageSeg segs[2] = {chunk_image_segment(a.ix, ch),
-                              StageSeg{a.off_rank, (const u32x4*)(a.ix.blob + ch.img_off + ch.off_term_rank), ch.n_words * 8u}};
+    const StageSeg img = CACHED ? StageSeg{a.ix.lds_img + ch.off_nsl_rng, (const u32x4*)(a.ix.blob + ch.img_off + ch.off_nsl_rng),
+                                           (ch.lds_bytes - ch.off_nsl_rng) / 16u}
+                                : chunk_image_segment(a.ix, ch);
+    const StageSeg segs[2] = {img, StageSeg{a.off_rank, (const u32x4*)(a.ix.blob + ch.img_off + ch.off_term_rank), ch.n_words * 8u}};
     lds_stage_segments<2, 4>(lds, segs);
   }
   if (ch.has_adj) {
@@ -467,9 +481,6 @@
     unsigned long long pw[NW];
 #pragma unroll
     for (int k = 0; k < NW; ++k) pw[k] = cur.pw[k];
-    const u32x4 raw[1] = {cur.raw};
-    uint32_t ro[LA];
-    atom_row_offsets<LA>(raw, ro);
     uint64_t qx[kWq];
     typedef typename std::conditional<(kWq > 3), uint64_t, uint32_t>::type qw_t;
     qw_t qw = 0;
@@ -500,24 +511,30 @@
         }
       }
     };
-    scan_tile<LA, VETO, NEED, false>(
-        bm, counted, ns, ro, [&](bool, uint32_t) {}, [&](uint32_t) { return true; },
-        [&](uint32_t w, uint64_t x, const u64x2& seg) -> uint64_t {
-          if (seg_on) {
-            const uint64_t v = x | seg.y;
-            x = andn_64(x, v - seg.x);
-          }
-          if (__ballot(x != 0ull && qn >= (uint32_t)kWq) != 0ull) flush();
-          if (x != 0ull) {
-#pragma unroll
-            for (int k = kWq - 1; k > 0; --k) qx[k] = qx[k - 1];
-            qx[0] = x;
-            qw = (qw_t)(qw << 10) | (qw_t)w;
-            qn += 1u;
-          }
-          return 0ull;
-        },
-        [&](uint32_t w) -> u64x2 { return seg_on ? segp[w] : u64x2{0ull, 0ull}; });
+    auto push_word = [&](uint32_t w, uint64_t x, const u64x2& seg) -> uint64_t {
+      if (seg_on) {
+        const uint64_t v = x | seg.y;
+        x = andn_64(x, v - seg.x);
+      }
+      if (__ballot(x != 0ull && qn >= (uint32_t)kWq) != 0ull) flush();
+      if (x != 0ull) {
+#pragma unroll
+        for (int k = kWq - 1; k > 0; --k) qx[k] = qx[k - 1];
+        qx[0] = x;
+        qw = (qw_t)(qw << 10) | (qw_t)w;
+        qn += 1u;
+      }
+      return 0ull;
+    };
+    auto run_masks = [&](uint32_t w) -> u64x2 { return seg_on ? segp[w] : u64x2{0ull, 0ull}; };
+    if constexpr (CACHED) {
+      replay_tile(bm, counted, ns, cur.mx, a.mx_planes, [&](bool, uint32_t) {}, push_word, run_masks);
+    } else {
+      const u32x4 raw[1] = {cur.raw};
+      uint32_t ro[LA];
+      atom_row_offsets<LA>(raw, ro);
+      scan_tile<LA, VETO, NEED, false>(bm, counted, ns, ro, [&](bool, uint32_t) {}, [&](uint32_t) { return true; }, push_word, run_masks);
+    }
     flush();
   }
   __syncthreads();
@@ -730,24 +747,32 @@
     BmAggOneArgs oa = make_bm_agg_one_args(ix, bm_args.pk, &one_total);
     const BmChunk& ch = ix.h_chunks[0];
     oa.v_meta = sc.v_meta, oa.v_latom = sc.v_latom, oa.v_pk = sc.v_pk, oa.ch = ch;
+    const bool cached = sc.v_mx != nullptr && sc.limb == 0 && sc.mx_planes >= 1u && sc.mx_planes <= (uint32_t)kMatchReplay &&
+                        (uint64_t)n_rows <= sc.mx_stride && match_cache_fits(ix);
+    if (cached) oa.v_mx = sc.v_mx, oa.mx_stride = sc.mx_stride, oa.mx_planes = sc.mx_planes;
     oa.slab = slab + (size_t)ch.slab_off * 16;
     oa.n_rows = (uint32_t)n_rows;
     oa.tpb = (uint32_t)((((n_rows + kWave - 1) / kWave) + nb - 1) / nb);
     static const bool dbg_one = getenv("KT_DEBUG_LDS") != nullptr;
     if (dbg_one)
-      fprintf(stderr, "kt_aggregate_bitmap_one: lds=%u (2 per CU) workgroups=%d tiles per workgroup=%u nw=%u rec=%u skew=%u\n", one_total, nb, oa.tpb,
-              oa.pk_nw, oa.pk_rec, oa.skew);
-#define KT_AGG_ONE_LAUNCH(VETO_, NEED_)                                                                          \
+      fprintf(stderr, "kt_aggregate_bitmap_one: lds=%u (2 per CU) workgroups=%d tiles per workgroup=%u nw=%u rec=%u skew=%u cached=%d\n", one_total, nb,
+              oa.tpb, oa.pk_nw, oa.pk_rec, oa.skew, cached ? 1 : 0);
+#define KT_AGG_ONE_LAUNCH(VETO_, NEED_, ...)                                                                     \
   {                                                                                                             \
-    auto kfn = kt_aggregate_bitmap_one<VETO_, NEED_>;                                                           \
+    auto kfn = kt_aggregate_bitmap_one<VETO_, NEED_, ##__VA_ARGS__>;                                            \
     (void)hipFuncSetAttribute((const void*)kfn, hipFuncAttributeMaxDynamicSharedMemorySize, (int)one_total);    \
     hipLaunchKernelGGL(kfn, g_, b_, one_total, s, oa);                                                          \
   }
+    if (cached) {
+      KT_AGG_ONE_LAUNCH(false, 2, true)
+      sc.replayed = true;
+    } else {
 #ifdef KT_FAST_BUILD
-    KT_AGG_ONE_LAUNCH(false, 2)
+      KT_AGG_ONE_LAUNCH(false, 2)
 #else
-    if (!ix.rich) KT_AGG_ONE_LAUNCH(false, 2) else KT_AGG_ONE_LAUNCH(true, 3)
+      if (!ix.rich) KT_AGG_ONE_LAUNCH(false, 2) else KT_AGG_ONE_LAUNCH(true, 3)
 #endif
+    }
 #undef KT_AGG_ONE_LAUNCH
   } else {
   const bool windowed = bm_args.win_recs != 0u;
diff --git a/kube_throttler_amd/csrc/kt_kernels_match.hip b/kube_throttler_amd/csrc/kt_kernels_match.hip
--- a/kube_throttler_amd/csrc/kt_kernels_match.hip
+++ b/kube_throttler_amd/csrc/kt_kernels_match.hip
@@ -11,6 +11,9 @@
   uint32_t planes;
   uint32_t n;
   uint32_t cap;
+  uint64_t* vx;
+  const int32_t* vpos;
+  uint64_t vstride;
   BmIndexArgs ix;
   BmChunk ch;
 };
@@ -38,6 +41,7 @@
     const bool in = i < n && p < a.cap;
     const uint32_t pc = min(p, a.cap - 1u);
     const uint64_t meta = a.meta[pc];
+    const int32_t vj = a.vx ? a.vpos[pc] : -1;
     u32x4 raw[1];
     load_atoms<LA>(a.latom, (int64_t)pc, raw);
     const bool on = in && ((meta >> kMetaStateShift) & kPodValid) != 0;
@@ -45,17 +49,42 @@
     uint32_t ro[LA];
     atom_row_offsets<LA>(raw, ro);
     uint64_t* q = a.mw + pc;
+    const bool thru = in && vj >= 0 && (uint64_t)vj < a.vstride;
+    uint64_t* qv = a.vx + (thru ? (uint32_t)vj : 0u);
     uint32_t round = 0u;
     scan_tile<LA, VETO, NEED, false>(
         bm, on, ns, ro, [&](bool, uint32_t) {}, [&](uint32_t) { return true; },
         [&](uint32_t, uint64_t xx, int) -> uint64_t {
           if (in && round < planes) q[(uint64_t)round * a.stride] = xx;
+          if (thru && round < planes) qv[(uint64_t)round * a.vstride] = xx;
           round += 1u;
           return 0ull;
         });
-    for (; round < planes; ++round)
+    for (; round < planes; ++round) {
       if (in) q[(uint64_t)round * a.stride] = 0ull;
+      if (thru) qv[(uint64_t)round * a.vstride] = 0ull;
+    }
   }
+}
+
+__global__ __launch_bounds__(256) void kt_gather_match_planes(const uint64_t* mw, uint64_t stride, uint32_t planes, const int64_t* rows, int64_t n,
+                                                             uint64_t* mx, uint64_t mx_stride) {
+  for (int64_t j = (int64_t)blockIdx.x * 256 + threadIdx.x; j < n; j += (int64_t)gridDim.x * 256) {
+    const uint64_t p = (uint64_t)rows[j];
+    if (p >= stride) continue;
+    uint64_t x[kMatchReplay];
+#pragma unroll
+    for (int k = 0; k < kMatchReplay; ++k) x[k] = (uint32_t)k < planes ? mw[(uint64_t)k * stride + p] : 0ull;
+#pragma unroll
+    for (int k = 0; k < kMatchReplay; ++k)
+      if ((uint32_t)k < planes) mx[(uint64_t)k * mx_stride + (uint64_t)j] = x[k];
+  }
+}
+void launch_gather_match_planes(const uint64_t* mw, uint64_t stride, uint32_t planes, const int64_t* rows, int64_t n, uint64_t* mx,
+                                uint64_t mx_stride, hipStream_t s) {
+  if (n <= 0 || !mw || !mx || planes == 0u || planes > (uint32_t)kMatchReplay || (uint64_t)n > mx_stride) return;
+  const int64_t nb = std::min<int64_t>((n + 255) / 256, 4096);
+  hipLaunchKernelGGL(kt_gather_match_planes, dim3((unsigned)nb), dim3(256), 0, s, mw, stride, planes, rows, n, mx, mx_stride);
 }
 
 bool match_cache_fits(const IndexDev& ix) {
@@ -65,13 +94,14 @@
 }
 
 bool launch_build_match_cache(const PodTable& pods, int64_t n, const int64_t* rows_dev, const IndexDev& ix, uint64_t* mw, uint64_t stride,
-                              uint32_t planes, hipStream_t s) {
+                              uint32_t planes, hipStream_t s, const MatchViewPlanes* view) {
   if (n <= 0) return true;
   if (!match_cache_fits(ix) || pods.LA > 8 || !mw || planes == 0u || planes > (uint32_t)kMatchPlanes || stride == 0u || n > (int64_t)stride)
     return false;
   MatchBuildArgs a{};
   a.meta = pods.meta, a.latom = pods.latom, a.rows = rows_dev, a.mw = mw, a.stride = stride, a.planes = planes;
   a.n = (uint32_t)n, a.cap = (uint32_t)std::min<uint64_t>(stride, 0x80000000ull);
+  if (view && view->mx && view->pos && view->stride) a.vx = view->mx, a.vpos = view->pos, a.vstride = view->stride;
   uint32_t o = 0;
   auto take = [&](uint32_t bytes) { uint32_t r = o; o += (bytes + 15u) & ~15u; return r; };
   plan_bitmap_index(ix, a.ix, take);
diff --git a/kube_throttler_amd/engine.py b/kube_throttler_amd/engine.py
--- a/kube_throttler_amd/engine.py
+++ b/kube_throttler_amd/engine.py
@@ -49,6 +49,7 @@
 COUNTER_AGG_WORKGROUPS = 11
 COUNTER_VIEW_BUILDS = 10
 COUNTER_MATCH_CACHE_BUILDS, COUNTER_MATCH_CACHE_SCANS, COUNTER_MATCH_CACHE_PLANES = 12, 13, 14
+COUNTER_MATCH_CACHE_AGG_SCANS = 15
 
 
 def partial_layout(n_dims: int) -> dict:
@@ -464,6 +465,9 @@
     def match_cache_scans(self) -> int:
         return int(lib().kt_counter(self._h, COUNTER_MATCH_CACHE_SCANS))
 
+    def match_cache_agg_scans(self) -> int:
+        return int(lib().kt_counter(self._h, COUNTER_MATCH_CACHE_AGG_SCANS))
+
     def partial_words(self) -> int:
         return self.throttle_rows() * partial_layout(self.D)["stride"]
 
```

After: 22920 billion decisions/s (median of 6 runs). 1.06x the previous value.
